# embedded-software-laboratory/p-dmpc

Measured on AMD Instinct MI355X. Metric: MPC steps/sec (whole node) + p50 per-step plan latency, N vehicles H=8, higher is better.
Workload: dtype f64

## Files before the change

include/pdmpc.h:

```cpp
#ifndef PDMPC_H
#define PDMPC_H

#include <stddef.h>
#include <stdint.h>

#ifdef __cplusplus
extern "C" {
#endif

#define PDMPC_HP_MAX 16
#define PDMPC_VMAX 8
#define PDMPC_JOINT_MAX 4

enum {
    PDMPC_OK = 0,
    PDMPC_EXHAUSTED = 1,
    PDMPC_ARENA_OVERFLOW = 2,
    PDMPC_ERR_INVALID = -1,
    PDMPC_ERR_NO_DEVICE = -2,
    PDMPC_ERR_HIP = -3,
    PDMPC_ERR_CAPACITY = -4,
    PDMPC_ERR_NO_MPA = -5
};

// ... 21 lines not shown
    double area[2][PDMPC_VMAX];
    double area_without_offset[2][PDMPC_VMAX];
    double area_large_offset[2][PDMPC_VMAX];
} pdmpc_maneuver;

typedef struct {
    int32_t n_trims;
    int32_t Hp;
    const uint8_t* transition;
    const int32_t* maneuver_index;
    int32_t n_maneuvers;
    const pdmpc_maneuver* maneuvers;
} pdmpc_mpa;

typedef struct {
    int32_t n_polygons;
    const int32_t* offset;
    const double* x;
    const double* y;
} pdmpc_polygon_set;

typedef struct {
    double x0, y0, yaw0;
    int32_t trim0;
    int32_t n_left;
    int32_t n_right;
    int32_t _pad;
    const double* ref_x;
    const double* ref_y;
    const double* v_ref;
    const double* left_x;
    const double* left_y;
    const double* right_x;
    const double* right_y;
    pdmpc_polygon_set obstacles;
    pdmpc_polygon_set dynamic_obstacles;
    pdmpc_polygon_set hdv_reachable_sets;
} pdmpc_vehicle_in;

typedef struct {
    int32_t status;
    int32_t n_expanded;
    int32_t n_popped;
    int32_t n_hp;
    int32_t tree_path[PDMPC_HP_MAX + 1];
    int32_t predicted_trims[PDMPC_HP_MAX];
    int32_t shape_cols[PDMPC_HP_MAX];
    int32_t _pad;
    double y_predicted[PDMPC_HP_MAX][3];
    double shapes[PDMPC_HP_MAX][2][PDMPC_VMAX];
    double path_nodes[PDMPC_HP_MAX + 1][8];
} pdmpc_vehicle_out;

typedef struct {
    int64_t n_vehicles;
    int64_t nodes_popped;
    int64_t nodes_generated;
    int64_t obstacle_columns;
    int64_t algorithmic_bytes;
    double kernel_ms;
    int64_t lds_bytes;
    int64_t lds_nodes;
    int64_t n_launches;
    int64_t queue_fallbacks;
    int64_t speculation_arrivals;
    int64_t edge_checks;
    int64_t segment_pair_tests;
    int64_t kernel;
    int64_t nodes_processed;
    int64_t rounds;
    int64_t shared_rounds;
    int64_t helper_checked;
    int64_t safe_replans;
    int64_t bad_status_plans;
} pdmpc_stats;


int pdmpc_create(const pdmpc_config* config, pdmpc_handle** out_handle);
int pdmpc_destroy(pdmpc_handle* handle);

int pdmpc_get_config(pdmpc_handle* handle, pdmpc_config* config, int32_t* mpa_uploaded);

int pdmpc_upload_mpa(pdmpc_handle* handle, const pdmpc_mpa* mpa);

int pdmpc_plan_batch(pdmpc_handle* handle, int32_t n_vehicles, const pdmpc_vehicle_in* in,
                     pdmpc_vehicle_out* out);

int pdmpc_set_arena_limit(pdmpc_handle* handle, int32_t max_nodes_limit);
int pdmpc_grow_arena(pdmpc_handle* handle, int32_t max_nodes);
int pdmpc_arena_nodes(pdmpc_handle* handle, int32_t* max_nodes, int64_t* regrows);

int pdmpc_plan_step(pdmpc_handle* handle, int32_t n_vehicles, const pdmpc_vehicle_in* in, const int32_t* pred_offset,
                    const int32_t* pred_index, const pdmpc_polygon_set* fallback_shapes, pdmpc_vehicle_out* out);

int pdmpc_plan_step_literal(pdmpc_handle* handle, int32_t n_vehicles, const pdmpc_vehicle_in* in, const int32_t* pred_offset, const int32_t* pred_index,
                            const pdmpc_polygon_set* fallback_shapes, pdmpc_vehicle_out* out);

int pdmpc_pack_batch(pdmpc_handle* handle, int32_t n_vehicles, const pdmpc_vehicle_in* in);
int pdmpc_plan_step_lean(pdmpc_handle* handle, int32_t n_vehicles, const pdmpc_vehicle_in* in, const int32_t* pred_offset, const int32_t* pred_index,
                         const pdmpc_polygon_set* fallback_shapes, int32_t* status, double* final_cost);
int pdmpc_fetch_records_at(pdmpc_handle* handle, int32_t count, const int32_t* vehicles, pdmpc_vehicle_out* out);
typedef struct {
    int32_t n_cells;
    int32_t n_graphs;
    int32_t n_picks;
    int32_t _pad;
    const int32_t* cell_offset;
    const int32_t* cell_slot;
    const int32_t* graph_offset;
    const int32_t* pick_graph;
    const int32_t* pick_offset;
    const int32_t* pick_slot;
} pdmpc_choice;
int pdmpc_choose_host(int32_t n, const int32_t* status, const double* final_cost, const pdmpc_choice* choice, int32_t* chosen, double* cell_cost);
int pdmpc_choose_resident(pdmpc_handle* handle, int32_t n, const pdmpc_choice* choice, int32_t* chosen, double* cell_cost, pdmpc_vehicle_out* picks);
int pdmpc_plan_step_chosen(pdmpc_handle* handle, int32_t n_vehicles, const pdmpc_vehicle_in* in, const int32_t* pred_offset, const int32_t* pred_index,
                           const pdmpc_polygon_set* fallback_shapes, const pdmpc_choice* choice, int32_t* chosen, double* cell_cost, pdmpc_vehicle_out* picks);
int pdmpc_choice_kernel_ms(pdmpc_handle* handle, double* ms);
int pdmpc_last_call_timing(pdmpc_handle* handle, double* us3);
int pdmpc_launch_packed(pdmpc_handle* handle);
int pdmpc_launch_range(pdmpc_handle* handle, int32_t first, int32_t count);
int pdmpc_fetch_results(pdmpc_handle* handle, int32_t n_vehicles, pdmpc_vehicle_out* out);
int pdmpc_synchronize(pdmpc_handle* handle);
int pdmpc_set_safe_launch(pdmpc_handle* handle, int32_t on);
int pdmpc_set_device_share(pdmpc_handle* handle, int32_t n_handles);
int pdmpc_begin_step(pdmpc_handle* handle);
int pdmpc_select_bank(pdmpc_handle* handle, int32_t bank);
int pdmpc_reset_stats(pdmpc_handle* handle);

int pdmpc_set_step_weights(pdmpc_handle* handle, int32_t n_vehicles, const double* weights);
int pdmpc_pack_step(pdmpc_handle* handle, int32_t n_vehicles, const pdmpc_vehicle_in* in,
                    const int32_t* pred_offset, const int32_t* pred_index,
                    const pdmpc_polygon_set* fallback_shapes);

int pdmpc_result_device_buffer(pdmpc_handle* handle, void** dev_ptr, size_t* nbytes);
int pdmpc_import_results(pdmpc_handle* handle, int32_t first, int32_t n, const void* dev_records);
int pdmpc_export_results(pdmpc_handle* handle, int32_t first, int32_t n, void* dev_records);

int pdmpc_export_results_async(pdmpc_handle* handle, int32_t first, int32_t n, void* dev_records);
int pdmpc_stream(pdmpc_handle* handle, void** hip_stream);

int pdmpc_get_last_stats(pdmpc_handle* handle, pdmpc_stats* stats);

int pdmpc_debug_pop_trace(pdmpc_handle* handle, int32_t vehicle, int32_t capacity, int32_t* ids, int32_t* n);
int pdmpc_debug_tree(pdmpc_handle* handle, int32_t vehicle, int32_t capacity, double* x, double* y,
                     double* yaw, double* g, double* h, int32_t* trim, int32_t* k, int32_t* parent,
                     int32_t* n);

int pdmpc_debug_edge_check(pdmpc_handle* handle, int32_t mode, int32_t n_cases, const int32_t* a_off, const double* a_x, const double* a_y,
                           const int32_t* b_off, const double* b_x, const double* b_y, int32_t* hit);

int pdmpc_debug_raw_tree(pdmpc_handle* handle, int32_t vehicle, int32_t capacity, double* x, double* y, double* yaw, double* g,
                         double* h, int32_t* trim, int32_t* k, int32_t* parent, double* key, uint8_t* validity, int32_t* n);

int pdmpc_debug_counters(pdmpc_handle* handle, uint64_t* out16);

int pdmpc_debug_progress(pdmpc_handle* handle, int32_t vehicle, uint32_t* words16);

int pdmpc_debug_heap_script(pdmpc_handle* handle, int32_t n, const int32_t* op, const int32_t* id, const double* key,
                            int32_t lds_entries, int32_t* popped, int32_t* n_popped, double* cycles_per_pop,
                            double* cycles_per_push);

int pdmpc_plan_batch_sampled(pdmpc_handle* handle, int32_t n_vehicles, const pdmpc_vehicle_in* in, const uint32_t* seeds,
                             pdmpc_vehicle_out* out);
int pdmpc_plan_step_sampled(pdmpc_handle* handle, int32_t n_vehicles, const pdmpc_vehicle_in* in, const int32_t* pred_offset,
                            const int32_t* pred_index, const pdmpc_polygon_set* fallback_shapes, const uint32_t* seeds,
// ... 181 lines not shown
```

p-dmpc_amd/csrc/api.cpp:

```cpp
#include <hip/hip_runtime.h>

#include <algorithm>
#include <cmath>
#include <cstdio>
#include <cstdlib>
#include <chrono>
#include <cstring>
#include <limits>
#include <map>
#include <mutex>
#include <string>
#include <utility>
#include <vector>

#include "../../include/pdmpc_geometry.h"
#include "handle.hpp"

namespace {

thread_local std::string g_err;

inline uint32_t align16(uint32_t v) { return (v + 15u) & ~15u; }

const size_t kLdsMax = 160 * 1024;

bool parse_tuning(const char* text, Tuning& T, std::string& err) {
    struct Key { const char* name; int* dst; };
    int spin = (int)T.spin_limit;
    const Key keys[] = {{"round0", &T.round0}, {"round", &T.round}, {"ramp", &T.ramp}, {"ready", &T.ready}, {"share_min", &T.share_min},
                        {"tile", &T.tile}, {"mid_min", &T.mid_min}, {"mid_fill", &T.mid_fill}, {"tentative", &T.tentative}, {"fast_arrival", &T.fast_arrival}, {"helpers_first", &T.helpers_first}, {"seat_nodes", &T.seat_nodes},
                        {"helpers", &T.helpers}, {"helpers_oversub", &T.helpers_oversub}, {"speculate", &T.speculate}, {"waves", &T.waves}, {"compact", &T.compact}, {"spin_limit", &spin},
                        {"force_tie", &T.force_tie}, {"reverse_dispatch", &T.reverse_dispatch}, {"debug_tail", &T.debug_tail}, {"debug_lds", &T.debug_lds},
                        {"debug_host", &T.debug_host}, {"debug_progress", &T.debug_progress}, {"generic", &T.generic}};
    std::string str(text ? text : "");
    size_t pos = 0;
    while (pos < str.size()) {
        size_t end = str.find(',', pos);
        if (end == std::string::npos) end = str.size();
        const std::string item = str.substr(pos, end - pos);
        pos = end + 1;
        if (item.empty()) continue;
        const size_t eq = item.find('=');
        if (eq == std::string::npos || eq == 0 || eq + 1 >= item.size()) {
            err = "PDMPC_TUNING: '" + item + "' is not key=value";
            return false;
        }
        const std::string name = item.substr(0, eq);
        char* tail = nullptr;
        const long v = strtol(item.c_str() + eq + 1, &tail, 10);
        if (!tail || *tail) {
            err = "PDMPC_TUNING: value of '" + name + "' is not an integer";
            return false;
        }
        bool found = false;
        for (const Key& k : keys)
            if (name == k.name) {
                *k.dst = (int)v;
                found = true;
            }
        if (!found) {
            err = "PDMPC_TUNING: unknown key '" + name + "'";
            return false;
        }
    }
    if (T.compact < -1 || T.compact > 1) {
        err = "PDMPC_TUNING: compact takes -1, 0 or 1";
        return false;
    }
    if (T.round0 >= 0) T.round0 = std::max(1, T.round0);
    if (T.round >= 0) T.round = std::max(1, T.round);
    if (T.ramp >= 0) T.ramp = std::max(1, T.ramp);
    T.ready = std::min(2048, std::max(256, T.ready)) & ~63;
    if (T.share_min >= 0) T.share_min = std::max(32, T.share_min);
    if (T.tile >= 0) T.tile = std::min(768, std::max(8, T.tile));
    T.mid_min = std::max(0, T.mid_min);
    T.mid_fill = std::max(256, T.mid_fill);
    if (T.waves >= 0) T.waves = std::min(PDMPC_MAX_WAVES, std::max(4, T.waves));
    T.spin_limit = (uint32_t)std::max(1024, spin);
    return true;
}
}

namespace {

std::mutex g_lds_mutex;
uint32_t g_lds_high_water[64][4][2];
const char* const kBulkKernelNames[4][2] = {{"pdmpc_bulk_kernel", "pdmpc_bulk_kernel_any"},
                                            {"pdmpc_bulk_kernel_wide", "pdmpc_bulk_kernel_wide_any"},
                                            {"pdmpc_bulk_kernel_sat", "pdmpc_bulk_kernel_sat_any"},
                                            {"pdmpc_bulk_kernel_compact", "pdmpc_bulk_kernel_compact_any"}};
template <class Layout>
uint32_t layout_mpa(const pdmpc_handle* h, uint32_t off, bool areas, Layout& L) {
    L.mask = off;
    off = align16(off + (uint32_t)h->mask_bytes);
    L.man_index = off;
    off = align16(off + (uint32_t)h->mi_bytes);
    L.pose = off;
    off = align16(off + (uint32_t)(h->n_man * sizeof(DevManPose)));
    L.area = off;
    if (areas) off = align16(off + (uint32_t)(h->n_man * 3 * PDMPC_VMAX * 16));
    return off;
}

bool layout_bulk(const pdmpc_handle* h, size_t budget, int n_waves, int areas, int soup_cap, LdsLayout& L, uint32_t& nv, uint32_t& nl, uint32_t ready_cap, bool compact) {
    const uint32_t lk_waves = compact ? PDMPC_LK_COMPACT_WAVES : PDMPC_MAX_WAVES, lk_ready = compact ? PDMPC_LK_COMPACT_READY_CAP : 2048u, lk_per = compact ? PDMPC_LK_COMPACT_BK_PER : PDMPC_BK_PER;
    if (ready_cap > lk_ready || (uint32_t)n_waves > lk_waves) return false;
    uint32_t off = layout_mpa(h, pdmpc_lk_fixed(lk_waves, lk_ready, lk_per, &L), areas, L);
    L.soup = off;
    off = align16(off + (uint32_t)std::max(soup_cap, 1) * 16);
    L.tree16 = L.bk_hist;
    const uint32_t min_nodes = 64 * (uint32_t)sizeof(NodeRec) + 1024;
    if ((size_t)off + min_nodes + 256 > budget) return false;
    const uint32_t rest = (uint32_t)(budget - off - 256);
    nv = std::min<uint32_t>(16384u, std::max<uint32_t>(compact ? 512u : 1024u, rest / 6));
    nv = std::min(nv, h->arena.max_nodes) & ~15u;
    nl = std::min((rest - nv) / (uint32_t)sizeof(NodeRec), h->arena.max_nodes);
    L.vstate = off;
    off += align16(nv);
    L.nodes = off;
    off += nl * (uint32_t)sizeof(NodeRec);
    L.total = align16(off);
    return L.total <= budget;
}

bool bulk_has_helpers(const Tuning& T, int n_cu, int n_launch) {
    if (!T.speculate || T.helpers == 0) return false;
    if (n_launch > n_cu) return T.helpers_oversub != 0;
    return n_launch <= n_cu - 2;
}

int compute_lds_bulk(const pdmpc_handle* h, int n_launch, int soup_cap, LaunchLayout& out) {
    const Tuning& T = h->tune;
    const int ready_want = bulk_has_helpers(T, h->n_cu, n_launch) ? T.ready : std::max(256, T.ready / 2);
    const int cap = h->cfg.checker == PDMPC_CHECK_SAT ? PDMPC_MAX_WAVES_SAT : PDMPC_MAX_WAVES;
    const bool want_compact = h->cfg.checker == PDMPC_CHECK_INTERX && h->n_words == 1 && (T.compact > 0 || (T.compact < 0 && n_launch > 2 * h->n_cu));
    uint32_t nv = 0, nl = 0;
    if (want_compact) {
        LdsLayout L{};
        const int waves = T.waves >= 0 ? std::min(T.waves, PDMPC_LK_COMPACT_WAVES) : PDMPC_LK_COMPACT_WAVES;
        const int ready = std::min(std::min(ready_want, 3 * PDMPC_WAVE * waves), (int)PDMPC_LK_COMPACT_READY_CAP);
        if (layout_bulk(h, kLdsMax / 2, waves, 0, soup_cap, L, nv, nl, (uint32_t)ready, true)) {
            out = {L, waves, (int)nl, (int)nv, 0, ready, true};
            return PDMPC_OK;
        }
    }
    const int waves = T.waves >= 0 ? std::min(T.waves, cap) : (n_launch > 2 * h->n_cu ? std::min(12, cap) : cap);
    for (int areas = 1; areas >= 0; --areas) {
        LdsLayout L{};
        const int ready = std::min(ready_want, 3 * PDMPC_WAVE * waves);
        if (!layout_bulk(h, kLdsMax, waves, areas, soup_cap, L, nv, nl, (uint32_t)ready, false)) continue;
        out = {L, waves, (int)nl, (int)nv, areas, ready, false};
        return PDMPC_OK;
    }
    char buf[256];
    snprintf(buf, sizeof buf, "obstacle soup (%d columns) + MPA tables do not fit into %zu B of LDS", soup_cap, kLdsMax);
    return fail(PDMPC_ERR_CAPACITY, buf);
}

int compute_lds_sampled(const pdmpc_handle* h, int soup_cap, int cand_cap, LaunchLayout& out) {
    static_assert(288u * 16u * 2u >= 624u * 4u, "the tree region holds the generator's state");
    for (int pass = 0; pass < 4; ++pass) {
        const int areas = pass == 0 || pass == 2;
        const size_t budget = pass < 2 ? kLdsMax / 2 : kLdsMax;
        LdsLayout L{};
        uint32_t off = layout_mpa(h, 0, areas, L);
        L.ref = off;
        off += 3 * PDMPC_HP_MAX * 8;
        L.shape = off;
        off += (2 * PDMPC_VMAX + 1) * 16;
        L.path = off;
        off += align16((PDMPC_HP_MAX + 2) * 4 + 2 * (PDMPC_HP_MAX + 1) * 4 + PDMPC_SH_WORDS * 4 + PDMPC_HP_MAX * 4);
        L.soup = off;
        off = align16(off + (uint32_t)std::max(soup_cap, 1) * 16);
        L.cand = off;
        off += align16((uint32_t)std::max(cand_cap, 1) * 4u);
        L.expand = off;
        off += (2 * PDMPC_HP_MAX * PDMPC_HP_MAX) * 8 + 16 * 16;
        L.tree16 = off;
        off += align16(288u * 18u * 2u);
        L.rand = off;
        off += align16((uint32_t)h->cfg.Hp * 250u * 8u);
        L.total = align16(off);
        if (L.total <= budget) {
            out = {L, 1, 0, 0, areas, h->tune.ready, false};
            return PDMPC_OK;
        }
    }
    return fail(PDMPC_ERR_CAPACITY, "obstacle soup + MPA tables do not fit into the LDS budget of the sampled optimizer");
}

int layout_joint(pdmpc_handle* h, int soup_cap, JointLds& L, uint32_t& heap_lds, int& areas_in_lds) {
    for (int pass = 0; pass < 4; ++pass) {
        const bool areas = pass == 0 || pass == 2;
        const size_t budget = pass < 2 ? 64 * 1024 : kLdsMax;
        uint32_t off = layout_mpa(h, 0, areas, L);
        L.ref = off;
        off += PDMPC_JOINT_MAX * 3 * PDMPC_HP_MAX * 8;
        L.shape = off;
        off += PDMPC_JOINT_MAX * 2 * PDMPC_VMAX * 16;
        L.ints = off;
        off = align16(off + PDMPC_JOINT_INTS * 4);
        L.succ = off;
        off = align16(off + (uint32_t)(PDMPC_JOINT_MAX * h->n_trims * 4));
        L.soup = off;
        off = align16(off + (uint32_t)std::max(soup_cap, 1) * 16);
        if (off + 256 * 12 > budget) continue;
        const uint32_t entries = std::min<uint32_t>(8192u, (uint32_t)((budget - off) / 12) & ~63u);
        L.heap_key = off;
        off += entries * 8;
        L.heap_id = off;
        off += entries * 4;
        L.total = align16(off);
        heap_lds = entries;
        areas_in_lds = areas ? 1 : 0;
        return PDMPC_OK;
    }
    return fail(PDMPC_ERR_CAPACITY, "the MPA tables and a joint problem's obstacle soups do not fit into LDS");
}
template <class Args>
void set_batch_args(const pdmpc_handle* h, const PackedStep& B, int areas_in_lds, Args& a) {
    a.succ_mask = h->d_mask.p;
    a.man_index = h->d_mi.p;
    a.man_pose = h->d_pose.p;
    a.man_area = h->d_area.p;
    a.n_trims = h->n_trims;
    a.n_words = h->n_words;
    a.n_man = h->n_man;
    a.Hp = h->cfg.Hp;
    a.areas_in_lds = areas_in_lds;
    a.dt = h->cfg.dt_seconds;
    a.veh = B.dev.veh;
    a.points = B.dev.pts;
    a.out = h->d_out.p;
    a.max_nodes = h->arena.max_nodes;
    a.tree_size = h->d_tree_size.p;
// ... 69 lines not shown
    a.bk_mid_fill = T.mid_fill;
    a.bk_tentative = T.tentative;
    a.bk_fast_arrival = T.fast_arrival;
    a.bk_seat_nodes = std::max(1, T.seat_nodes);
    a.bk_force_tie = T.force_tie;
    a.bk_post = h->d_bk_post.p;
    a.help_board = h->d_help_board.p;
    a.help_verdict = h->d_help_verdict.p;
    a.help_finished = h->d_help_finished.p;
    h->launch_serial += 1;
    if (h->launch_serial == 0) h->launch_serial = 1;
    a.launch_id = h->launch_serial;
    a.n_searches = count;
}

int prepare_boards(pdmpc_handle* h, int count, uint32_t& fin_base) {
    fin_base = 0;
    if (!h->boards_dirty) {
        fin_base = h->help_fin_total;
        h->help_fin_total += (uint32_t)count;
    } else {
        HIPCHK(hipMemsetAsync(h->d_help_board.p, 0, (size_t)h->max_vehicles * PDMPC_HB_WORDS * sizeof(unsigned long long), h->stream));
        HIPCHK(hipMemsetAsync(h->d_help_finished.p, 0, 16 * sizeof(uint32_t), h->stream));
        h->help_fin_total = (uint32_t)count;
        h->boards_dirty = false;
    }
    return PDMPC_OK;
}

int bulk_variant(const pdmpc_handle* h, const LaunchLayout& lay) {
    return lay.compact ? PDMPC_BULK_COMPACT : (h->cfg.checker == PDMPC_CHECK_SAT ? PDMPC_BULK_SAT : (h->n_words != 1 ? PDMPC_BULK_WIDE : PDMPC_BULK));
}
bool bulk_generic(const pdmpc_handle* h, const KernelArgs& a, const LaunchLayout& lay) { return h->tune.generic != 0 || !ProductSwitches::matches(a, bulk_variant(h, lay)); }

void print_bulk_layout(const pdmpc_handle* h, const KernelArgs& a, const LaunchLayout& lay) {
    const uint32_t near = (lay.compact ? PDMPC_LK_COMPACT_BK_PER : PDMPC_BK_PER) * (uint32_t)lay.n_waves * PDMPC_WAVE;
    const char* kernel = kBulkKernelNames[bulk_variant(h, lay)][bulk_generic(h, a, lay) ? 1 : 0];
    if (lay.compact)
        fprintf(stderr, "pdmpc LDS layout (compact): launch %d waves %d near %u ready %d nv %d nl %d total %u kernel %s\n", a.n_searches, lay.n_waves, near, lay.ready, lay.NV, lay.NL, lay.lds.total, kernel);
    else
        fprintf(stderr, "pdmpc LDS layout: launch %d waves %d areas %d near %u ready %d nv %d nl %d total %u kernel %s\n", a.n_searches, lay.n_waves, lay.areas_in_lds, near, lay.ready, lay.NV, lay.NL,
                lay.lds.total, kernel);
}

int dispatch(const pdmpc_handle* h, const KernelArgs& a, const LaunchLayout& lay, bool search, bool safe) {
    const int first = a.first, count = a.n_searches;
    const int variant = bulk_variant(h, lay), generic = bulk_generic(h, a, lay) ? 1 : 0;
    auto launch_search = [&](const KernelArgs* ka, int cnt) -> int {
        typedef int (*launcher_t)(const KernelArgs*, int, void*, uint32_t*);
        static const launcher_t launchers[4][2] = {{pdmpc_launch_bulk, pdmpc_launch_bulk_any},
                                                   {pdmpc_launch_bulk_wide, pdmpc_launch_bulk_wide_any},
                                                   {pdmpc_launch_bulk_sat, pdmpc_launch_bulk_sat_any},
                                                   {pdmpc_launch_bulk_compact, pdmpc_launch_bulk_compact_any}};
        std::lock_guard<std::mutex> lock(g_lds_mutex);
        return launchers[variant][generic](ka, cnt, (void*)h->stream, &g_lds_high_water[h->cfg.device & 63][variant][generic]);
    };
    auto in_slices = [&](int resident, auto&& launch) -> int {
        int lrc = 0;
        for (int done = 0; done < count && lrc == 0; done += resident) {
            KernelArgs part = a;
            part.first = first + done;
            part.n_searches = std::min(resident, count - done);
            lrc = launch(&part, part.n_searches);
        }
        return lrc;
    };
    if (!search) {
        const int resident = lay.lds.total <= kLdsMax / 2 ? 2 * h->n_cu : h->n_cu;
        return in_slices(safe ? resident : count, [&](const KernelArgs* ka, int cnt) { return pdmpc_launch_sampled(ka, cnt, (void*)h->stream); });
    }
    if (safe && count > h->n_cu) return in_slices(h->n_cu, launch_search);
    return launch_search(&a, count);
}

int launch_range(pdmpc_handle* h, int first, int count, bool safe) {
    if (!h) return fail(PDMPC_ERR_INVALID, "null handle");
    PackedStep& B = h->banks[h->bank];
    const bool search = !B.sampled;
    if (B.pack_failed) return fail(PDMPC_ERR_INVALID, "the last pack into this bank failed: nothing is packed");
    if (first < 0 || count < 0 || first + count > B.n_packed) return fail(PDMPC_ERR_INVALID, "launch range outside the packed batch");
    if (!B.perm.empty() && (first != 0 || count != B.n_packed)) return fail(PDMPC_ERR_INVALID, "range launches need a batch packed in level order (predecessors in lower slots)");
    if (count == 0) return PDMPC_OK;
    LaunchLayout lay;
    int rc = search ? compute_lds_bulk(h, count, B.soup_cap, lay) : compute_lds_sampled(h, B.soup_cap, B.cand_cap, lay);
    if (rc) return rc;
    KernelArgs a{};
    set_launch_args(h, B, lay, first, count, safe, a);
    launch_policy(h->tune, count, h->n_cu, h->device_share, safe, search, lay, B.host.veh + first, a);
    if (a.n_helpers > 0 && (rc = prepare_boards(h, count, a.help_fin_base))) return rc;
    if (search && h->tune.debug_lds) print_bulk_layout(h, a, lay);
    if ((rc = h->timer.begin(h->stream, search ? kLaunchSearch : kLaunchSampled))) return rc;
    const int lrc = dispatch(h, a, lay, search, safe);
    if (lrc != 0) {
        h->boards_dirty = true;
        char buf[256];
        snprintf(buf, sizeof buf, "kernel launch failed: %s (LDS %u B)", hipGetErrorString((hipError_t)lrc), lay.lds.total);
        return fail(PDMPC_ERR_HIP, buf);
    }
    if ((rc = h->timer.end(h->stream))) return rc;
    h->stats.lds_bytes = lay.lds.total;
    h->stats.lds_nodes = lay.NL;
    return PDMPC_OK;
}

int check_result_slots(const pdmpc_handle* h, int32_t first, int32_t n) {
    if (!h->banks[h->bank].perm.empty()) return fail(PDMPC_ERR_INVALID, "the packed batch was put into level order by the library: raw slots are not the caller's vehicles (pack it in level order to use the device-resident record path)");
    if (first < 0 || n < 0 || first + n > h->max_vehicles) return fail(PDMPC_ERR_INVALID, "slot range out of bounds");
    return PDMPC_OK;
}
}

extern "C" {

const char* pdmpc_last_error(void) { return g_err.c_str(); }
void pdmpc_set_last_error(const char* msg) { g_err = msg ? msg : ""; }
const char* pdmpc_version(void) { return "pdmpc-hip 0.1 (gfx950)"; }

int pdmpc_create(const pdmpc_config* config, pdmpc_handle** out_handle) {
    if (!config || !out_handle) return fail(PDMPC_ERR_INVALID, "null argument");
    if (config->Hp < 1 || config->Hp > PDMPC_HP_MAX) return fail(PDMPC_ERR_INVALID, "Hp must be in 1..PDMPC_HP_MAX");
    if (config->checker != PDMPC_CHECK_SAT && config->checker != PDMPC_CHECK_INTERX) return fail(PDMPC_ERR_INVALID, "unknown checker");
    int ndev = 0;
    if (hipGetDeviceCount(&ndev) != hipSuccess || ndev == 0)
        return fail(PDMPC_ERR_NO_DEVICE, "no HIP device visible: this backend has no CPU fallback");
    if (config->device < 0 || config->device >= ndev) return fail(PDMPC_ERR_NO_DEVICE, "device ordinal out of range");
    ON_DEVICE(config->device);
    hipDeviceProp_t prop;
    HIPCHK(hipGetDeviceProperties(&prop, config->device));
    if (std::string(prop.gcnArchName).find("gfx950") == std::string::npos)
        return fail(PDMPC_ERR_NO_DEVICE, std::string("device is ") + prop.gcnArchName + ", this library is built for gfx950 only");
    pdmpc_handle* h = new pdmpc_handle();
    h->cfg = *config;
    h->banks.resize(1);
    {
        std::string err;
        if (!parse_tuning(getenv("PDMPC_TUNING"), h->tune, err)) {
            delete h;
            return fail(PDMPC_ERR_INVALID, err);
        }
    }
    h->n_cu = prop.multiProcessorCount > 0 ? prop.multiProcessorCount : 256;
    const uint32_t want_nodes = config->max_nodes > 0 ? (uint32_t)config->max_nodes : 32768u;
    h->max_vehicles = config->max_vehicles > 0 ? config->max_vehicles : 256;
    if (hipStreamCreateWithFlags(&h->stream, hipStreamNonBlocking) != hipSuccess) {
        delete h;
        return fail(PDMPC_ERR_HIP, "hipStreamCreate failed");
    }
    int bad = h->arena.alloc(h->max_vehicles, want_nodes, h->cfg.Hp);
    bad |= h->d_out.ensure((size_t)h->max_vehicles) | h->d_flag.ensure((size_t)h->max_vehicles) | h->d_tree_size.ensure((size_t)h->max_vehicles) | h->d_tie_count.ensure(4) | h->d_work_count.ensure(16);
    bad |= h->d_help_board.ensure((size_t)h->max_vehicles * PDMPC_HB_WORDS) | h->d_help_verdict.ensure((size_t)h->max_vehicles * PDMPC_HELP_CAP) | h->d_help_finished.ensure(16);
    bad |= h->d_bk_post.ensure((size_t)h->max_vehicles * (size_t)h->tune.ready * 6);
    if (bad) {
        delete h;
        return fail(PDMPC_ERR_HIP, "hipMalloc failed for the per-vehicle arenas (lower max_nodes / max_vehicles)");
    }
    (void)hipMemsetAsync(h->d_flag.p, 0, h->d_flag.cap * sizeof(uint32_t), h->stream);
    (void)hipMemsetAsync(h->d_tree_size.p, 0, h->d_tree_size.cap * sizeof(int32_t), h->stream);
    (void)hipMemsetAsync(h->d_tie_count.p, 0, 4 * sizeof(int32_t), h->stream);
    (void)hipMemsetAsync(h->d_work_count.p, 0, 16 * sizeof(unsigned long long), h->stream);
    (void)hipMemsetAsync(h->d_out.p, 0, h->d_out.cap * sizeof(pdmpc_vehicle_out), h->stream);
    (void)hipStreamSynchronize(h->stream);
    *out_handle = h;
    return PDMPC_OK;
}

int pdmpc_destroy(pdmpc_handle* h) {
    if (!h) return PDMPC_OK;
    DeviceGuard device_guard__(h->cfg.device);
    delete h;
    return PDMPC_OK;
}

int pdmpc_upload_mpa(pdmpc_handle* h, const pdmpc_mpa* mpa) {
    if (!h || !mpa) return fail(PDMPC_ERR_INVALID, "null argument");
    if (mpa->n_trims < 1 || mpa->n_trims > 1023) return fail(PDMPC_ERR_INVALID, "n_trims must be in 1..1023");
    if (mpa->Hp < h->cfg.Hp) return fail(PDMPC_ERR_INVALID, "mpa.Hp smaller than config.Hp");
    if (!mpa->transition || !mpa->maneuver_index || (mpa->n_maneuvers > 0 && !mpa->maneuvers)) return fail(PDMPC_ERR_INVALID, "null table");
    ON_DEVICE(h->cfg.device);
    const int n = mpa->n_trims, Hp = h->cfg.Hp;
    const int nw = (n + 63) / 64;
    std::vector<uint64_t> mask((size_t)Hp * n * nw + 2, 0);
    for (int k = 0; k < Hp; ++k)
        for (int i = 0; i < n; ++i)
            for (int j = 0; j < n; ++j)
                if (mpa->transition[((size_t)k * n + i) * n + j]) {
                    const int mi = mpa->maneuver_index[i * n + j];
                    if (mi < 0 || mi >= mpa->n_maneuvers) return fail(PDMPC_ERR_INVALID, "transition allowed but maneuver missing");
                    mask[((size_t)k * n + i) * nw + j / 64] |= 1ull << (j % 64);
                }
    std::vector<int16_t> mi((size_t)n * n + 8, -1);
    for (int i = 0; i < n * n; ++i) mi[i] = (int16_t)mpa->maneuver_index[i];
    const int T = mpa->n_maneuvers;
    std::vector<DevManPose> pose((size_t)std::max(T, 1));
    std::vector<double> area((size_t)std::max(T, 1) * 3 * PDMPC_VMAX * 2, 0.0);
    for (int t = 0; t < T; ++t) {
        const pdmpc_maneuver& m = mpa->maneuvers[t];
        if (m.n_cols < 2 || m.n_cols > PDMPC_VMAX) return fail(PDMPC_ERR_INVALID, "maneuver area column count out of range");
        pose[t].dx = m.dx;
        pose[t].dy = m.dy;
        pose[t].dyaw = m.dyaw;
        pose[t].n_cols = m.n_cols;
        pose[t].pad = 0;
        const double(*src[3])[PDMPC_VMAX] = {m.area, m.area_without_offset, m.area_large_offset};
        for (int a = 0; a < 3; ++a)
            for (int v = 0; v < m.n_cols; ++v) {
                area[(((size_t)t * 3 + a) * PDMPC_VMAX + v) * 2 + 0] = src[a][0][v];
                area[(((size_t)t * 3 + a) * PDMPC_VMAX + v) * 2 + 1] = src[a][1][v];
            }
    }
    if (h->d_mask.ensure(mask.size()) || h->d_mi.ensure(mi.size()) || h->d_pose.ensure(pose.size()) || h->d_area.ensure(area.size()))
        return fail(PDMPC_ERR_HIP, "hipMalloc failed for the MPA tables");
    HIPCHK(hipMemcpy(h->d_mask.p, mask.data(), mask.size() * 8, hipMemcpyHostToDevice));
    HIPCHK(hipMemcpy(h->d_mi.p, mi.data(), mi.size() * 2, hipMemcpyHostToDevice));
    HIPCHK(hipMemcpy(h->d_pose.p, pose.data(), pose.size() * sizeof(DevManPose), hipMemcpyHostToDevice));
    HIPCHK(hipMemcpy(h->d_area.p, area.data(), area.size() * 8, hipMemcpyHostToDevice));
    h->n_trims = n;
    h->n_words = nw;
    h->n_man = T;
    h->mask_bytes = (size_t)Hp * n * nw * 8;
    h->mi_bytes = (size_t)n * n * 2;
    h->mpa_alg_bytes = (int64_t)8 * T * (3 + 6 * PDMPC_VMAX) + (int64_t)n * n * Hp / 8;
    h->has_mpa = true;
    return PDMPC_OK;
}

int pdmpc_pack_batch(pdmpc_handle* h, int32_t n, const pdmpc_vehicle_in* in) { return pdmpc_pack_step(h, n, in, nullptr, nullptr, nullptr); }

int pdmpc_pack_step(pdmpc_handle* h, int32_t n, const pdmpc_vehicle_in* in, const int32_t* pred_offset, const int32_t* pred_index,
                    const pdmpc_polygon_set* fallback_shapes) {
    if (!h) return fail(PDMPC_ERR_INVALID, "null handle");
    ON_DEVICE(h->cfg.device);
    if (pred_offset && !pred_index) return fail(PDMPC_ERR_INVALID, "pred_index missing");
    return pack_common(h, n, in, pred_offset, pred_index, fallback_shapes);
}

int pdmpc_set_step_weights(pdmpc_handle* h, int32_t n, const double* weights) {
    if (!h || n < 0 || (n > 0 && !weights)) return fail(PDMPC_ERR_INVALID, "pdmpc_set_step_weights: bad argument");
    h->next_weights.assign(weights, weights + n);
    return PDMPC_OK;
}

int pdmpc_set_step_seeds(pdmpc_handle* h, int32_t n, const uint32_t* seeds) {
    if (!h || n < 0 || (n > 0 && !seeds)) return fail(PDMPC_ERR_INVALID, "pdmpc_set_step_seeds: bad argument");
    h->next_seeds.assign(seeds, seeds + n);
    h->seeds_set = true;
    return PDMPC_OK;
}

int pdmpc_launch_packed(pdmpc_handle* h) {
    if (!h) return fail(PDMPC_ERR_INVALID, "null handle");
    ON_DEVICE(h->cfg.device);
    h->epoch += 1;
    return launch_range(h, 0, h->banks[h->bank].n_packed, h->safe_launches);
}

int pdmpc_set_device_share(pdmpc_handle* h, int32_t n_handles) {
    if (!h || n_handles < 1) return fail(PDMPC_ERR_INVALID, "pdmpc_set_device_share: bad argument");
    h->device_share = n_handles;
    return PDMPC_OK;
}

int pdmpc_set_safe_launch(pdmpc_handle* h, int32_t on) {
    if (!h) return fail(PDMPC_ERR_INVALID, "null handle");
    h->safe_launches = on != 0;
    return PDMPC_OK;
}

int pdmpc_begin_step(pdmpc_handle* h) {
    if (!h) return fail(PDMPC_ERR_INVALID, "null handle");
    h->epoch += 1;
    return PDMPC_OK;
}

int pdmpc_select_bank(pdmpc_handle* h, int32_t bank) {
    if (!h) return fail(PDMPC_ERR_INVALID, "null handle");
    if (bank < 0 || bank >= 4096) return fail(PDMPC_ERR_INVALID, "bank out of range");
    if ((size_t)bank >= h->banks.size()) h->banks.resize((size_t)bank + 1);
    h->bank = bank;
    return PDMPC_OK;
}

int pdmpc_reset_stats(pdmpc_handle* h) {
    if (!h) return fail(PDMPC_ERR_INVALID, "null handle");
    ON_DEVICE(h->cfg.device);
    HIPCHK(hipStreamSynchronize(h->stream));
    h->timer.reset();
    HIPCHK(hipMemsetAsync(h->d_tie_count.p, 0, 4 * sizeof(int32_t), h->stream));
    HIPCHK(hipMemsetAsync(h->d_work_count.p, 0, 16 * sizeof(unsigned long long), h->stream));
    return PDMPC_OK;
}

int pdmpc_launch_range(pdmpc_handle* h, int32_t first, int32_t count) {
// ... 923 lines not shown
```

p-dmpc_amd/csrc/bulk_search.hpp:

```cpp
#include <hip/hip_runtime.h>

#include "search_common.hpp"

#include "frontier_common.hpp"

#define BK_P2 3
#define BK_PER PDMPC_BK_PER
#define BK_FAST_PER 4

namespace {

typedef volatile LDS_AS unsigned long long lds_vu64;

__device__ __forceinline__ unsigned long long wg_scan_excl(unsigned long long v, lds_vu64* wsum, int lane, int wave, int n_waves, unsigned long long& total) {
    unsigned long long inc = v;
#pragma unroll
    for (int o = 1; o < PDMPC_WAVE; o <<= 1) {
        const unsigned long long t = __shfl_up(inc, o);
        inc += lane >= o ? t : 0ull;
    }
    if (lane == PDMPC_WAVE - 1) wsum[wave] = inc;
    __syncthreads();
    unsigned long long off = 0, tot = 0;
    for (int q = 0; q < n_waves; ++q) {
        const unsigned long long w = wsum[q];
        off += q < wave ? w : 0ull;
        tot += w;
    }
    total = tot;
    return off + inc - v;
}

__device__ __forceinline__ d2 node_piece(const Search& S, uint32_t i0, int q) {
    if (i0 < S.NL) return S.ln[4 * (size_t)i0 + q];
    return ((const d2*)(S.gn + i0))[q];
}
__device__ __forceinline__ void piece_link(d2 p3, uint32_t& parent, uint32_t& packed) {
    const uint64_t u = (uint64_t)__double_as_longlong(p3.y);
    parent = (uint32_t)(u & 0xffffffffull);
    packed = (uint32_t)(u >> 32);
}

struct BkCheck {
    const lds_d2* l_area;
    const d2* g_area;
    const lds_d2* l_soup;
    const lds_i32* l_soff;
    const lds_i32* l_hoff;
    const lds_i32* l_lit;
    int areas_in_lds, ll_base, ll_len, Hp;
};

#define VS_TENT 6u
#define BK_TENT_MIN FR_JOIN_MAX
#define BK_NTENT FR_SEL2_BIN
#define BK_ARRIVALS FR_SEL2_CUM
#define BK_DEPTH FR_RD_HEAD
#define BK_IDLE FR_RD_TAIL
#define BK_MID_N 10
#define BK_MID_MIN 12
#define BK_L_MID 14
#define BK_FD_LO 16
#define BK_FD_HI 17
#define BK_WAITRES 18
#define BK_TIEMODE 20
#define BK_RP_NEED 21
#define BK_RP_GOAL 22
#define BK_RP_NPOP 23
#define BK_RP_NREF 24
#define BK_PUBLISHED 19

__device__ __forceinline__ void bk_tentative_areas(const KernelArgs& A, const SpecCtx& P, unsigned long long who, int tid, int nthreads) {
    const double qnan = __longlong_as_double(0x7ff8000000000000LL);
    const int per = P.Hp * PDMPC_VMAX, n_pred = P.n_pred < 64 ? P.n_pred : 64;
    for (int idx = tid; idx < n_pred * per; idx += nthreads) {
        const int p = idx / per, rest = idx - p * per;
        if (!((who >> p) & 1ull)) continue;
        const DevVehicle* PV = A.veh + P.pred[p];
        if (PV->fb_off[0] < 0) continue;
        const int k = rest / PDMPC_VMAX, v = rest - k * PDMPC_VMAX;
        const int a = PV->fb_off[k], b = PV->fb_off[k + 1];
        const int cols = (b - a < PDMPC_VMAX) ? (b - a) : PDMPC_VMAX;
        d2 pt;
        pt.x = v < cols ? A.points[2 * (size_t)(a + (v < cols ? v : 0))] : qnan;
        pt.y = v < cols ? A.points[2 * (size_t)(a + (v < cols ? v : 0)) + 1] : qnan;
        P.l_soup[P.l_soff[k] + P.l_lit[k] + p * PDMPC_VMAX + v] = pt;
    }
}

struct BkTreeSrc {
    const Search* S;
    const lds_u32* ready;
    __device__ __forceinline__ void link(uint32_t r, uint32_t& parent, uint32_t& packed) const { piece_link(node_piece(*S, ready[r] - 1u, 3), parent, packed); }
    __device__ __forceinline__ void pose(uint32_t, uint32_t parent, double& px, double& py, double& cs, double& sn) const {
        const d2 pxy = node_piece(*S, parent - 1u, 0), pcs = node_piece(*S, parent - 1u, 2);
        px = pxy.x;
        py = pxy.y;
        cs = pcs.x;
        sn = pcs.y;
    }
};
struct BkPostSrc {
    const lds_d2* rec;
    __device__ __forceinline__ void link(uint32_t r, uint32_t& parent, uint32_t& packed) const { piece_link(d2{0.0, rec[3 * r + 2].x}, parent, packed); }
    __device__ __forceinline__ void pose(uint32_t r, uint32_t, double& px, double& py, double& cs, double& sn) const {
        const d2 pxy = rec[3 * r], pcs = rec[3 * r + 1];
        px = pxy.x;
        py = pxy.y;
        cs = pcs.x;
        sn = pcs.y;
    }
};

template <int CHECKER>
__device__ __forceinline__ void bk_item_counts(int M_k, int Hk, int ll_len, int& n0, int& n1, int& n2) {
    n0 = CHECKER == PDMPC_CHECK_INTERX ? (M_k > 1 ? M_k - 1 : 0) : M_k;
    n1 = CHECKER == PDMPC_CHECK_INTERX ? (Hk > 1 ? Hk - 1 : 0) : 0;
    n2 = ll_len > 1 ? ll_len - 1 : 0;
}
template <int CHECKER, class Src>
__device__ __forceinline__ void bk_check_items(const BkCheck& C, const Src& src, volatile lds_u32* r_flag, uint32_t r0, uint32_t R, int ls, uint32_t chmax, unsigned long long pend, int tid, int nthreads) {
    const uint32_t items = R * chmax;
    const int Sg = 1 << ls;
    for (uint32_t item = (uint32_t)tid; item < items; item += (uint32_t)nthreads) {
        const uint32_t c = item / R, r = r0 + (item - c * R);
        if (r_flag[r] & 1u) continue;
        uint32_t parent, packed;
        src.link(r, parent, packed);
        if (!parent) continue;
        const int k = NODE_K(packed), m = NODE_MAN(packed), ncols = NODE_COLS(packed);
        const int so = C.l_soff[k - 1], ho = C.l_hoff[k - 1];
        const int M_k = C.l_soff[k] - so, Hk = C.l_hoff[k] - ho;
        int n0, n1, n2;
        bk_item_counts<CHECKER>(M_k, Hk, C.ll_len, n0, n1, n2);
        const uint32_t c0 = (uint32_t)((n0 + Sg - 1) >> ls), c1 = (uint32_t)((n1 + Sg - 1) >> ls), c2 = (uint32_t)((n2 + Sg - 1) >> ls);
        int base, t0, left, which = 0;
        if (c < c0) {
            base = so;
            t0 = (int)(c << ls);
            left = n0 - t0;
        } else if (c < c0 + c1) {
            base = ho;
            t0 = (int)((c - c0) << ls);
            left = n1 - t0;
        } else if (c < c0 + c1 + c2) {
            base = C.ll_base;
            t0 = (int)((c - c0 - c1) << ls);
            left = n2 - t0;
            which = k == C.Hp ? 2 : 1;
        } else {
            continue;
        }
        const int tn = left < Sg ? left : Sg;
        double cc, ss, pX, pY;
        src.pose(r, parent, pX, pY, cc, ss);
        const size_t abase = ((size_t)m * 3 + (size_t)which) * PDMPC_VMAX;
        d2 pt[PDMPC_VMAX];
#pragma unroll
        for (int i = 0; i < PDMPC_VMAX; ++i) {
            const d2 a = C.areas_in_lds ? (d2)C.l_area[abase + i] : C.g_area[abase + i];
            pt[i].x = cc * a.x - ss * a.y + pX;
            pt[i].y = ss * a.x + cc * a.y + pY;
        }
        const lds_d2* q = C.l_soup + base + t0;
        if (CHECKER == PDMPC_CHECK_SAT) {
            uint32_t fnd = 0;
            if (which == 0) {
                const int lit = C.l_lit[k - 1];
                for (int t = 0; t < tn && !(fnd & 1u); ++t) {
                    const int j = t0 + t;
                    const bool start = !is_nan(q[t].x) && (j == 0 || is_nan(C.l_soup[base + j - 1].x) || (j >= lit && ((j - lit) & (PDMPC_VMAX - 1)) == 0));
                    if (start) {
                        int e = j + 1;
                        const int lim = j >= lit ? j + PDMPC_VMAX - ((j - lit) & (PDMPC_VMAX - 1)) : M_k;
                        while (e < lim && !is_nan(C.l_soup[base + e].x)) ++e;
                        if (sat_pair_lane(pt, ncols, C.l_soup + base + j, e - j)) {
                            const bool tent = j >= lit && ((pend >> ((j - lit) >> 3)) & 1ull) != 0ull;
                            fnd |= tent ? 2u : 1u;
                        }
                    }
                }
            } else {
                double min_x, max_x, min_y, max_y;
                sat_area_bbox(pt, ncols, min_x, max_x, min_y, max_y);
                for (int t = 0; t < tn && !fnd; ++t) fnd = sat_boundary_segment_lane(pt, ncols, min_x, max_x, min_y, max_y, q[t], q[t + 1]) ? 1u : 0u;
            }
            if (fnd) __hip_atomic_fetch_or((lds_u32*)&r_flag[r], fnd, __ATOMIC_RELAXED, __HIP_MEMORY_SCOPE_WORKGROUP);
            continue;
        }
        d2 q0 = q[0];
        const int rel0 = (which == 0 && base == so) ? t0 - C.l_lit[k - 1] : -(1 << 20);
        uint32_t found = 0;
        for (int t = 0; t < tn && !(found & 1u); ++t) {
            asm volatile("" : "+v"(pt[0].x), "+v"(pt[0].y), "+v"(pt[1].x), "+v"(pt[1].y), "+v"(pt[2].x), "+v"(pt[2].y), "+v"(pt[3].x), "+v"(pt[3].y), "+v"(pt[4].x), "+v"(pt[4].y),
                         "+v"(pt[5].x), "+v"(pt[5].y), "+v"(pt[6].x), "+v"(pt[6].y), "+v"(pt[7].x), "+v"(pt[7].y));
            const d2 q1 = q[t + 1];
            if (interx_segment_n<PDMPC_VMAX>(pt, ncols - 1, q0, q1)) {
                const int rel = rel0 + t;
                const bool tent = rel >= 0 && ((pend >> (rel >> 3)) & 1ull) != 0ull;
                found |= tent ? 2u : 1u;
            }
            q0 = q1;
        }
        if (found) __hip_atomic_fetch_or((lds_u32*)&r_flag[r], found, __ATOMIC_RELAXED, __HIP_MEMORY_SCOPE_WORKGROUP);
    }
}

__device__ __forceinline__ int bk_chunk_shift(const lds_u32* chm, uint32_t R, uint32_t nthreads) {
    int ls = 0;
    while (ls < 4 && R * chm[ls] > nthreads) ++ls;
    return ls;
}

__device__ __forceinline__ int nth_bit(uint64_t mask, int rk) {
    for (int b = 0; b < rk; ++b) mask &= mask - 1ull;
    return (int)__builtin_ctzll(mask);
}

template <int CHECKER>
__device__ __forceinline__ void bk_recheck_items(const Search& S, const VState& VS, const BkCheck& C, const SpecCtx& P, const uint32_t* vlist, const lds_u32* vcnt, uint32_t cap,
                                                 uint32_t items, unsigned long long arr, const lds_u64s* chg, volatile lds_u32* sh, int tid, int nthreads) {
    for (uint32_t item = (uint32_t)tid; item < items; item += (uint32_t)nthreads) {
        uint32_t v = item, n_k = 0;
        int ks = 1;
        for (; ks <= C.Hp; ++ks) {
            n_k = vcnt[ks - 1] < cap ? vcnt[ks - 1] : cap;
            const uint32_t m = n_k * (uint32_t)__builtin_popcountll(chg[ks - 1] & arr);
            if (v < m) break;
            v -= m;
        }
        const uint32_t a = v / n_k;
        const uint32_t i0 = vlist[(size_t)(ks - 1) * cap + (v - a * n_k)];
        if (vs_load(VS, i0) != VS_VALID) continue;
        uint32_t parent, packed;
        piece_link(node_piece(S, i0, 3), parent, packed);
        if (!parent) continue;
        const int k = NODE_K(packed), m = NODE_MAN(packed), ncols = NODE_COLS(packed);
        const unsigned long long due = chg[k - 1] & arr;
        if (a >= (uint32_t)__builtin_popcountll(due)) continue;
        const int p = nth_bit(due, (int)a);
        const d2 pxy = node_piece(S, parent - 1u, 0), pcs = node_piece(S, parent - 1u, 2);
        const double cc = pcs.x, ss = pcs.y, pX = pxy.x, pY = pxy.y;
        const size_t abase = (size_t)m * 3 * PDMPC_VMAX;
        d2 pt[PDMPC_VMAX];
#pragma unroll
        for (int i = 0; i < PDMPC_VMAX; ++i) {
            const d2 ar = C.areas_in_lds ? (d2)C.l_area[abase + i] : C.g_area[abase + i];
            pt[i].x = cc * ar.x - ss * ar.y + pX;
            pt[i].y = ss * ar.x + cc * ar.y + pY;
        }
        const lds_d2* poly = P.l_soup + P.l_soff[k - 1] + P.l_lit[k - 1] + p * PDMPC_VMAX;
        d2 q0 = poly[0];
        bool hit = false;
        if (CHECKER == PDMPC_CHECK_SAT) {
            int cols = 0;
            while (cols < PDMPC_VMAX && !is_nan(poly[cols].x)) ++cols;
            hit = cols > 0 && sat_pair_lane(pt, ncols, poly, cols);
        }
#pragma unroll 1
        for (int j = 0; CHECKER == PDMPC_CHECK_INTERX && j + 1 < PDMPC_VMAX; ++j) {
            asm volatile("" : "+v"(pt[0].x), "+v"(pt[0].y), "+v"(pt[1].x), "+v"(pt[1].y), "+v"(pt[2].x), "+v"(pt[2].y), "+v"(pt[3].x), "+v"(pt[3].y), "+v"(pt[4].x), "+v"(pt[4].y),
                         "+v"(pt[5].x), "+v"(pt[5].y), "+v"(pt[6].x), "+v"(pt[6].y), "+v"(pt[7].x), "+v"(pt[7].y));
            const d2 q1 = poly[j + 1];
            hit = hit || interx_segment_n<PDMPC_VMAX>(pt, ncols - 1, q0, q1);
            q0 = q1;
        }
        if (hit) {
            vs_store(VS, i0, VS_INVALID);
            atomicOr((uint32_t*)&sh[FR_FLAGS], FRF_INVALIDATED);
        }
    }
}

#define BK_NB 256
__device__ __forceinline__ uint32_t bk_bin(double key, double lo, double scale) {
    const double t = (key - lo) * scale;
    if (!(t > 0.0)) return 0u;
    return t < (double)(BK_NB - 1) ? (uint32_t)t : (uint32_t)(BK_NB - 1);
}
__device__ __forceinline__ void bk_select(const lds_u32* bins, uint32_t target, int lane, uint32_t& bin, uint32_t& cum) {
    uint32_t hq[4];
#pragma unroll
    for (int q = 0; q < 4; ++q) hq[q] = bins[4 * lane + q];
    const uint32_t loc = hq[0] + hq[1] + hq[2] + hq[3];
    uint32_t inc = loc;
#pragma unroll
    for (int o = 1; o < PDMPC_WAVE; o <<= 1) {
        const uint32_t v = (uint32_t)__shfl_up((int)inc, o);
        inc += lane >= o ? v : 0u;
    }
    const uint32_t total = lane_u(inc, PDMPC_WAVE - 1);
    const uint32_t want = target < total ? target : total;
    uint32_t c = inc - loc, b = 0, cu = 0;
    bool f = false;
#pragma unroll
    for (int q = 0; q < 4; ++q) {
        c += hq[q];
        const bool hit = !f && hq[q] != 0u && c >= want;
        b = hit ? (uint32_t)(4 * lane + q) : b;
        cu = hit ? c : cu;
        f = f || hit;
    }
    const unsigned long long m = __ballot(f);
    const int l = m ? (int)__builtin_ctzll(m) : 0;
    const uint32_t bb = lane_u(b, l), cc = lane_u(cu, l);
    bin = m ? bb : 0u;
    cum = m ? cc : 0u;
}

__device__ __forceinline__ void bk_post_store(d2* p, d2 v) {
    __hip_atomic_store((double*)p, (double)v.x, __ATOMIC_RELAXED, __HIP_MEMORY_SCOPE_AGENT);
    __hip_atomic_store((double*)p + 1, (double)v.y, __ATOMIC_RELAXED, __HIP_MEMORY_SCOPE_AGENT);
}
__device__ __forceinline__ d2 bk_post_load(const d2* p) {
    d2 v;
    v.x = __hip_atomic_load((const double*)p, __ATOMIC_RELAXED, __HIP_MEMORY_SCOPE_AGENT);
    v.y = __hip_atomic_load((const double*)p + 1, __ATOMIC_RELAXED, __HIP_MEMORY_SCOPE_AGENT);
    return v;
}
__device__ __forceinline__ void bk_area_store(double* p, double v) { __hip_atomic_store(p, v, __ATOMIC_RELAXED, __HIP_MEMORY_SCOPE_AGENT); }
__device__ __forceinline__ void bk_area_store_u32(int32_t* p, int v) { __hip_atomic_store(p, (int32_t)v, __ATOMIC_RELAXED, __HIP_MEMORY_SCOPE_AGENT); }
__device__ __forceinline__ double bk_area_load(const double* p) { return __hip_atomic_load(p, __ATOMIC_RELAXED, __HIP_MEMORY_SCOPE_AGENT); }
__device__ __forceinline__ int bk_area_load_i32(const int32_t* p) { return (int)__hip_atomic_load(p, __ATOMIC_RELAXED, __HIP_MEMORY_SCOPE_AGENT); }

__device__ __forceinline__ void bk_write_record(const KernelArgs& A, Ctx& X, uint32_t goal, int status, bool dep_timeout, uint32_t n_popped, uint32_t nnodes, bool path_ready,
                                                const lds_u32* ref_ids, bool again, bool counts_only, int lane) {
    const int Hp = X.Hp;
    const DevVehicle* __restrict__ V = X.V;
    pdmpc_vehicle_out* __restrict__ O = X.O;
    lds_u32* l_path = X.l_path;
    const Search& S = X.S;
    if (counts_only) {
        if (goal && ref_ids && lane <= Hp) O->tree_path[lane] = (int32_t)ref_ids[lane];
        if (lane == 0) {
// ... 38 lines not shown
            if (lane >= 1) {
                O->y_predicted[lane - 1][0] = r.x;
                O->y_predicted[lane - 1][1] = r.y;
                O->y_predicted[lane - 1][2] = r.yaw;
                O->predicted_trims[lane - 1] = (int32_t)NODE_TRIM(r.packed);
            }
        }
        for (int idx = lane; idx < Hp * PDMPC_VMAX; idx += PDMPC_WAVE) {
            const int i = idx / PDMPC_VMAX + 1;
            const int v = idx - (i - 1) * PDMPC_VMAX;
            const NodeRec pr = node_load(S, l_path[i - 1] - 1);
            const NodeRec cr = node_load(S, l_path[i] - 1);
            const int m = NODE_MAN(cr.packed);
            const int ncols = NODE_COLS(cr.packed);
            if (v == 0) {
                bk_area_store_u32(&O->shape_cols[i - 1], ncols);
                pcols[i - 1] = (uint32_t)ncols;
            }
            d2 sp = d2{0.0, 0.0};
            if (v < ncols) {
                const d2 a = X.C.g_area[(size_t)m * 3 * PDMPC_VMAX + v];
                sp.x = pr.cs * a.x - pr.sn * a.y + pr.x;
                sp.y = pr.sn * a.x + pr.cs * a.y + pr.y;
                bk_area_store(&O->shapes[i - 1][0][v], sp.x);
                bk_area_store(&O->shapes[i - 1][1][v], sp.y);
            }
            pshape[idx] = sp;
        }
    } else if (V->fb_off[0] >= 0) {
        for (int idx = lane; idx < Hp * PDMPC_VMAX; idx += PDMPC_WAVE) {
            const int k = idx / PDMPC_VMAX;
            const int v = idx - k * PDMPC_VMAX;
            const int a = V->fb_off[k], b = V->fb_off[k + 1];
            const int cols = (b - a < PDMPC_VMAX) ? (b - a) : PDMPC_VMAX;
            if (v == 0) bk_area_store_u32(&O->shape_cols[k], cols);
            if (v < cols) {
                bk_area_store(&O->shapes[k][0][v], A.points[2 * (size_t)(a + v)]);
                bk_area_store(&O->shapes[k][1][v], A.points[2 * (size_t)(a + v) + 1]);
            }
        }
    }
    if (lane == 0) {
        O->status = dep_timeout ? PDMPC_ERR_HIP : status;
        O->n_expanded = (int32_t)nnodes;
        O->n_popped = (int32_t)n_popped;
        O->n_hp = Hp;
    }
}

__device__ __forceinline__ void bk_publish_flag(const KernelArgs& A, int slot, int lane) {
    asm volatile("s_waitcnt vmcnt(0)" ::: "memory");
    wave_sync();
    if (lane == 0) {
        __hip_atomic_store(A.done_flag + slot, A.epoch, __ATOMIC_RELAXED, __HIP_MEMORY_SCOPE_AGENT);
    }
}
__device__ __forceinline__ void bk_publish(const KernelArgs& A, const Ctx& X, int status, bool dep_timeout) {
    if (X.lane == 0 && (dep_timeout || (status != PDMPC_OK && status != PDMPC_EXHAUSTED))) atomicAdd(A.work_count + 6, 1ull);
    bk_publish_flag(A, X.slot, X.lane);
}

__device__ __forceinline__ unsigned long long bk_poll_flags(const KernelArgs& A, const SpecCtx& P, unsigned long long want, int lane) {
    bool d = false;
    if ((want >> lane) & 1ull) d = __hip_atomic_load(A.done_flag + P.pred[lane], __ATOMIC_RELAXED, __HIP_MEMORY_SCOPE_AGENT) == A.epoch;
    const unsigned long long got = __ballot(d);
    return got;
}

__device__ __forceinline__ bool bk_poll_predecessors(const KernelArgs& A, const SpecCtx& P, volatile lds_u32* sh, unsigned long long skip, int lane) {
    const unsigned long long pend = sh_load64(sh, SH_PEND_LO) & ~skip;
    if (!pend) return false;
    const unsigned long long got = bk_poll_flags(A, P, pend, lane);
    if (!got) return false;
    if (lane == 0) {
        sh[SH_ARR_LO] = (uint32_t)got;
        sh[SH_ARR_HI] = (uint32_t)(got >> 32);
        __builtin_amdgcn_fence(__ATOMIC_RELEASE, "workgroup");
        atomicCAS((uint32_t*)&sh[SH_STATE], ST_RUN, ST_ARRIVED);
    }
    return true;
}

__device__ __forceinline__ void bk_incorporate_body(const pdmpc_vehicle_out* out, const int32_t* pred, lds_d2* l_soup, const lds_i32* l_soff, const lds_i32* l_lit, int Hp, unsigned long long arr, int tid,
                                                    int nthreads, lds_u64s* chg) {
    const double qnan = __longlong_as_double(0x7ff8000000000000LL);
    const int per = Hp * PDMPC_VMAX, n_arr = __builtin_popcountll(arr);
    for (int idx = tid; idx < n_arr * per; idx += nthreads) {
        const int a = idx / per, rest = idx - a * per;
        const int p = nth_bit(arr, a);
        const pdmpc_vehicle_out* PO = out + pred[p];
        const int k = rest / PDMPC_VMAX, v = rest - k * PDMPC_VMAX;
        const int cols = bk_area_load_i32(&PO->shape_cols[k]);
        const double sx = bk_area_load(&PO->shapes[k][0][v]), sy = bk_area_load(&PO->shapes[k][1][v]);
        d2 pt;
        pt.x = v < cols ? sx : qnan;
        pt.y = v < cols ? sy : qnan;
        lds_d2* slot = l_soup + l_soff[k] + l_lit[k] + p * PDMPC_VMAX + v;
        if (chg) {
            const d2 was = *slot;
            if (__double_as_longlong(was.x) != __double_as_longlong(pt.x) || __double_as_longlong(was.y) != __double_as_longlong(pt.y))
                __hip_atomic_fetch_or(chg + k, 1ull << p, __ATOMIC_RELAXED, __HIP_MEMORY_SCOPE_WORKGROUP);
        }
        *slot = pt;
    }
}
__device__ __forceinline__ void bk_incorporate(const pdmpc_vehicle_out* out, const int32_t* pred, lds_d2* l_soup, const lds_i32* l_soff, const lds_i32* l_lit, int Hp, unsigned long long arr, int tid,
                                               int nthreads, lds_u64s* chg) {
    bk_incorporate_body(out, pred, l_soup, l_soff, l_lit, Hp, arr, tid, nthreads, chg);
}

#define WC_DEAD 0x100u
#define WC_ONPATH 0x200u
#define WC_VALID 0x400u
__device__ int bk_classify_wave(const unsigned long long* glink, ulonglong2* walk, const VState& VS, const double* gkey, const lds_u32* gp_path, const lds_f64* gp_mp, bool have_goal,
                                bool check_alive, uint32_t best, uint32_t epoch, uint32_t a, double ka, volatile lds_u32* sh) {
    const uint32_t a0 = a ? a : 1u;
    const uint64_t ua = glink[a0 - 1u];
    const uint32_t p = (uint32_t)(ua & 0xffffffffull);
    const int k = NODE_K((uint32_t)(ua >> 32));
    const bool onp = have_goal && gp_path[k] == a0;
    const ulonglong2 c = walk[p ? p - 1u : 0u];
    const uint32_t ctag = (uint32_t)(c.y & 0xffffffffull), cinfo = (uint32_t)(c.y >> 32);
    const bool hit = p != 0u && ctag == best && (cinfo & (WC_VALID | 0xffff0000u)) == (WC_VALID | (epoch << 16));
    double M = -1.0;
    int dJ = k;
    bool dead = false;
    int st = (a == 0u || onp || hit) ? 1 : 0;
    uint32_t x = a0;
    while (__ballot(st == 0)) {
        const uint32_t i = x - 1u;
        const uint64_t u = glink[i];
        const int d = NODE_K((uint32_t)(u >> 32));
        const bool on_path = have_goal && gp_path[d] == x;
        const bool bad = !on_path && x != a0 && check_alive && vs_load(VS, i) != VS_VALID;
        const double kx = gkey[i];
        const uint32_t par = (uint32_t)(u & 0xffffffffull);
        const bool walking = st == 0;
        const bool stop = on_path || bad || par == 0u;
        dJ = (walking && on_path) ? d : dJ;
        dead = dead || (walking && bad);
        M = (walking && !on_path && !bad && kx > M) ? kx : M;
        st = (walking && stop) ? 1 : st;
        x = (walking && !stop) ? par : x;
    }
    if (hit && !onp) {
        const bool p_on = (cinfo & WC_ONPATH) != 0u;
        const double pM = __longlong_as_double((long long)c.x);
        const uint32_t vsp = check_alive && !p_on ? vs_load(VS, p - 1u) : (uint32_t)VS_VALID;
        dead = !p_on && ((cinfo & WC_DEAD) != 0u || vsp != VS_VALID);
        M = (!p_on && pM > ka) ? pM : ka;
        dJ = (int)(cinfo & 0xffu);
    }
    const double thr = gp_mp[dJ];
    int res = 1;
    if (a != 0u && !onp) {
        res = dead ? 4 : ((have_goal && M > thr) ? 3 : 1);
        if (!dead && have_goal && M == thr) atomicOr((uint32_t*)&sh[FR_FLAGS], FRF_TIE);
    }
    if (a != 0u && res == 1) {
        ulonglong2 w;
        w.x = (unsigned long long)__double_as_longlong(onp ? -1.0 : M);
        w.y = (unsigned long long)best | ((unsigned long long)((uint32_t)(onp ? k : dJ) | (onp ? WC_ONPATH : 0u) | WC_VALID | (epoch << 16)) << 32);
        walk[a0 - 1u] = w;
    }
    return res;
}

__device__ __forceinline__ void bk_wait_done(const uint32_t* done_flag, const int32_t* pred, const pdmpc_vehicle_out* out, uint32_t epoch, uint32_t slot, lds_d2* l_soup, const lds_i32* l_soff,
                                             const lds_i32* l_lit, lds_d2* pshape, volatile lds_u32* sh, int Hp, int n_pred, bool have_path, lds_vu64* tk_pub, unsigned long long first, uint32_t max_spins,
                                             bool sat, int lane) {
    const lds_u32* pcols = (const lds_u32*)(pshape + Hp * PDMPC_VMAX);
    lds_u64s* chg = (lds_u64s*)(pcols + PDMPC_HP_MAX);
    unsigned long long pend = sh_load64(sh, SH_PEND_LO), fd = sh_load64(sh, BK_FD_LO);
    unsigned long long got = first;
    uint32_t spins = 0, res = 0;
    for (;;) {
        if (!got && pend != 0ull) {
            bool d = false;
            if (lane < n_pred && ((pend >> lane) & 1ull)) d = __hip_atomic_load(done_flag + pred[lane], __ATOMIC_RELAXED, __HIP_MEMORY_SCOPE_AGENT) == epoch;
            got = __ballot(d);
            if (!got) {
                if (++spins >= max_spins) break;
                __builtin_amdgcn_s_sleep(1);
                continue;
            }
            bk_incorporate_body(out, pred, l_soup, l_soff, l_lit, Hp, got, lane, PDMPC_WAVE, chg);
            wave_sync();
            pend &= ~got;
            fd |= got;
        }
        const int n_got = __builtin_popcountll(got);
        const int per = Hp * (PDMPC_VMAX - 1), items = have_path ? n_got * per : 0;
        bool hit = false;
        for (int base = 0; base < items; base += PDMPC_WAVE) {
            const int item = base + lane;
            const bool in = item < items;
            const int it = in ? item : 0;
            const int a = it / per, rest = it - a * per;
            const int k0 = rest / (PDMPC_VMAX - 1), j = rest - k0 * (PDMPC_VMAX - 1);
            const int p = nth_bit(got, a);
            d2 pt[PDMPC_VMAX];
#pragma unroll
            for (int i = 0; i < PDMPC_VMAX; ++i) pt[i] = pshape[k0 * PDMPC_VMAX + i];
            const lds_d2* poly = l_soup + l_soff[k0] + l_lit[k0] + p * PDMPC_VMAX;
            bool h1;
            if (!((chg[k0] >> p) & 1ull)) {
                h1 = false;
            } else if (sat) {
                int cols = 0;
                while (cols < PDMPC_VMAX && !is_nan(poly[cols].x)) ++cols;
                h1 = j == 0 && cols > 0 && sat_pair_lane(pt, (int)pcols[k0], poly, cols);
            } else {
                h1 = interx_segment_n<PDMPC_VMAX>(pt, (int)pcols[k0] - 1, poly[j], poly[j + 1]);
            }
            hit = hit || (in && h1);
        }
        got = 0ull;
        if (__ballot(hit)) {
            res = 1;
            break;
        }
        if (pend == 0ull) {
            res = 2;
            asm volatile("s_waitcnt vmcnt(0)" ::: "memory");
            wave_sync();
            if (lane == 0) {
                __hip_atomic_store((uint32_t*)done_flag + slot, epoch, __ATOMIC_RELAXED, __HIP_MEMORY_SCOPE_AGENT);
                if (tk_pub) *tk_pub = __builtin_amdgcn_s_memrealtime();
            }
            break;
        }
        if (max_spins == 0u) break;
    }
    if (lane == 0) {
        sh[SH_PEND_LO] = (uint32_t)pend;
        sh[SH_PEND_HI] = (uint32_t)(pend >> 32);
        sh[BK_FD_LO] = (uint32_t)fd;
        sh[BK_FD_HI] = (uint32_t)(fd >> 32);
        sh[BK_WAITRES] = res;
        if (res == 2u) sh[BK_PUBLISHED] = 1u;
        sh[BK_IDLE] = sh[BK_IDLE] + spins + 1u;
    }
}

__device__ __forceinline__ void bk_offer_goals_lanes(const Frontier& F, const Search& S, const VState& VS, bool cand, uint32_t id, int lane) {
    double m = 0.0;
    bool alive = cand;
    if (cand) {
        uint32_t nd = id;
        for (;;) {
            const double k = F.gkey[nd - 1];
            m = k > m ? k : m;
            if (nd != id && vs_load(VS, nd - 1) != VS_VALID) alive = false;
            const uint32_t par = node_parent(S, nd - 1);
            if (!par) break;
            nd = par;
        }
    }
    const unsigned long long bal = __ballot(alive);
    if (bal) {
        const uint32_t base = sh_add_uniform(F.sh, FR_GOAL_N, (uint32_t)__builtin_popcountll(bal), lane);
        if (alive) {
            node_store_cs(S, id - 1u, m, 0.0);
            const uint32_t pos = base + lane_rank(bal, lane);
            if (pos < 1024u) F.goal_list[pos] = id;
        }
    }
}

__device__ __noinline__ void bk_far_select(const Frontier& F, uint32_t fill, int lane) {
    fr_select2(F, fill, fill, FR_SEL_BIN, FR_SEL_BIN, lane);
}

template <int NW>
__device__ __forceinline__ void bk_replay(const KernelArgs& A, Ctx& X, const Frontier& F, const ExpandEnv& EE, lds_f64* heap_key, lds_u32* heap_id, uint32_t hl, uint32_t* pops, uint32_t* node2ref,
                                          const uint32_t* child0, lds_u32* ref_ids, int lane) {
    volatile lds_u32* sh = F.sh;
    const VState& VS = X.VS;
    const int Hp = X.Hp, n = EE.n, nw = NW > 0 ? NW : EE.nw;
    Search H = X.S;
    H.lkey = heap_key;
    H.lid = heap_id;
    H.HL = hl & ~1u;
    H.gkey = F.far_key;
    H.gid = F.far_id;
    H.heap_len = 0;
    H.lane = lane;
    H.pl = make_pop_lane(lane);
    heap_push(H, 0u, 0.0);
    if (lane == 0) node2ref[0] = 1u;
    uint32_t n_ref = 1, n_pop = 0, goal = 0, need = 0;
    bool bug = false;
    for (;;) {
        if (H.heap_len == 0u) break;
        double k0;
        uint32_t b;
        heap_load<true>(H, 0u, true, k0, b);
        b = uni_u(b);
        heap_pop(H);
        if (lane == 0) pops[n_pop] = b;
        n_pop += 1u;
        const uint32_t v = uni_u(vs_load(VS, b));
        if (v == VS_UNKNOWN || v == VS_TENT) {
            need = b + 1u;
            break;
        }
        if (v != VS_VALID) continue;
        const uint64_t u = F.glink[b];
        const uint32_t packed = uni_u((uint32_t)(u >> 32));
        const int k = NODE_K(packed);
        if (k == Hp) {
            goal = b + 1u;
            break;
        }
        const lds_mask64* mrow = EE.l_mask + ((size_t)k * n + (NODE_TRIM(packed) - 1)) * nw;
        uint32_t cnt = 0;
        for (int w = 0; w < nw; ++w) cnt += (uint32_t)__builtin_popcountll(mrow[w]);
        cnt = uni_u(cnt);
        if (cnt == 0u) continue;
        const uint32_t c0 = uni_u(__hip_atomic_load(child0 + b, __ATOMIC_RELAXED, __HIP_MEMORY_SCOPE_AGENT));
        if (c0 == 0u) {
            bug = true;
// ... 18 lines not shown
        for (int i = Hp; i >= 0; --i) {
            X.l_path[i] = nd;
            ref_ids[i] = __hip_atomic_load(node2ref + (nd - 1u), __ATOMIC_RELAXED, __HIP_MEMORY_SCOPE_AGENT);
            nd = (uint32_t)(F.glink[nd - 1u] & 0xffffffffull);
        }
    }
    if (lane == 0) {
        sh[BK_RP_NEED] = need;
        sh[BK_RP_GOAL] = goal;
        sh[BK_RP_NPOP] = n_pop;
        sh[BK_RP_NREF] = n_ref;
        if (bug) sh[FR_FLAGS] = sh[FR_FLAGS] | FRF_BUG;
        if (!need && !bug) atomicAdd(X.P.counters + 0, 1);
    }
}

template <int NW, int CHECKER, class SW>
__device__ __forceinline__ bool bulk_search(const KernelArgs& A, Ctx& X, lds_u32* ref_ids) {
    const int tid = X.tid, lane = X.lane, wave = X.wave, slot = X.slot, Hp = X.Hp;
    volatile lds_u32* sh = X.l_shared;
    Search& S = X.S;
    const VState& VS = X.VS;
    const SpecCtx& P = X.P;
    const DevVehicle* __restrict__ V = X.V;
    const int n_waves = (int)(blockDim.x >> 6), bd = (int)blockDim.x;
    const double inf = __longlong_as_double(0x7FF0000000000000LL);
    const size_t voff = (size_t)slot * A.max_nodes;
    const int n = X.n, nw = NW > 0 ? NW : X.nw;
    const uint32_t OC = (uint32_t)(BK_PER * bd), RC = (uint32_t)A.bk_ready_cap;
    const uint32_t VCAP = 1024u;

    lds_f64* near_key = (lds_f64*)(X.lsm + PDMPC_LK_NEAR_KEY);
    lds_u32* near_id = (lds_u32*)(X.lsm + PDMPC_LK_NEAR_ID);
    lds_u32* ready = (lds_u32*)(X.lsm + PDMPC_LK_READY);
    volatile lds_u32* r_flag = (volatile lds_u32*)(ready + RC);
    lds_u32* hist = (lds_u32*)(X.lsm + PDMPC_LK_HIST);
    lds_u32* vlist = hist + 1024;
    lds_u32* voffs = hist + 2048;
    lds_u32* gp_path = (lds_u32*)(X.lsm + PDMPC_LK_MISC);
    lds_f64* gp_mp = (lds_f64*)(gp_path + 32);
    lds_vu64* wsum64 = (lds_vu64*)(gp_mp + 32);
    volatile lds_u32* wsum = (volatile lds_u32*)(wsum64 + 32);
    lds_u32* chm = (lds_u32*)(wsum + 32);
    lds_u32* bins = gp_path + 256;

    Frontier F;
    F.sh = sh;
    F.ready = ready;
    F.hist = hist;
    F.goal_list = hist;
    F.near_key = A.arena.pb_key + voff;
    F.near_id = A.arena.pb_d + voff;
    F.far_key = A.arena.far_key + voff;
    F.far_id = A.arena.far_id + voff;
    F.gkey = S.gkey;
    F.glink = A.arena.link + voff;
    F.n_waves = n_waves;

    ExpandEnv EE;
    EE.l_mask = X.l_mask;
    EE.l_mi = X.l_mi;
    EE.l_pose = X.l_pose;
    EE.l_rx = X.l_rx;
    EE.l_ry = X.l_ry;
    EE.l_dcum = X.l_dcum;
    EE.l_term = nullptr;
    EE.l_chxy = nullptr;
    EE.Hp = Hp;
    EE.n = X.n;
    EE.nw = X.nw;
    EE.lane = lane;

    BkCheck CK;
    CK.l_area = X.C.l_area;
    CK.g_area = X.C.g_area;
    CK.l_soup = X.C.l_soup;
    CK.l_soff = X.C.l_soff;
    CK.l_hoff = X.C.l_hoff;
    CK.l_lit = P.l_lit;
    CK.areas_in_lds = SW::areas_in_lds(A);
    CK.ll_base = X.C.ll_base;
    CK.ll_len = X.C.ll_len;
    CK.Hp = Hp;

    if (tid == 0) {
        NodeRec r;
        r.x = V->x0;
        r.y = V->y0;
        r.yaw = V->yaw0;
        r.g = 0.0;
        r.cs = 0.0;
        r.sn = 0.0;
        r.h = 0.0;
        r.parent = 0;
        r.packed = (uint32_t)V->trim0;
        node_store(S, 0, r);
        F.gkey[0] = 0.0;
        F.glink[0] = (unsigned long long)r.parent | ((unsigned long long)r.packed << 32);
        ((ulonglong2*)A.arena.walk + voff)[0].y = 0ull;
        (A.arena.child0 + voff)[0] = 0u;
        vs_store(VS, 0, VS_UNKNOWN);
        for (int w = 26; w < SH_WORDS; ++w) sh[w] = 0;
        sh[FR_NNODES] = 1;
        sh_st_d(sh, FR_NEAR_MIN, inf);
        sh_st_d(sh, FR_FAR_MIN, inf);
        sh_st_d(sh, FR_L_FAR, inf);
        sh_st_d(sh, BK_TENT_MIN, inf);
        sh[BK_MID_N] = 0;
        sh[BK_MID_N + 1] = 0;
        sh_st_d(sh, BK_MID_MIN, inf);
        sh_st_d(sh, BK_L_MID, -1.0);
        sh[SH_NNODES] = 1;
        sh[BK_TIEMODE] = SW::force_tie(A) ? 1u : 0u;
        ready[0] = 1u;
        r_flag[0] = 0u;
    }
    if (tid < BK_NB) bins[tid] = 0u;
    if (A.n_helpers > 0 && tid >= 64 && tid < 64 + PDMPC_HB_SEATS_MAX) {
        unsigned long long* bd0 = A.help_board + (size_t)slot * PDMPC_HB_WORDS;
        const int k = tid - 64;
        __hip_atomic_store(bd0 + PDMPC_HB_ASSIGN + k, 0ull, __ATOMIC_RELAXED, __HIP_MEMORY_SCOPE_AGENT);
        __hip_atomic_store(bd0 + PDMPC_HB_DONE + k, 0ull, __ATOMIC_RELAXED, __HIP_MEMORY_SCOPE_AGENT);
        if (k == 0) {
            __hip_atomic_store(bd0 + PDMPC_HB_WANT, 0ull, __ATOMIC_RELAXED, __HIP_MEMORY_SCOPE_AGENT);
            __hip_atomic_store(bd0 + PDMPC_HB_SEATS, (unsigned long long)A.launch_id << 32, __ATOMIC_RELAXED, __HIP_MEMORY_SCOPE_AGENT);
        }
        asm volatile("s_waitcnt vmcnt(0)" ::: "memory");
    }
    if (SW::tentative(A)) bk_tentative_areas(A, P, sh_load64(sh, SH_PEND_LO), tid, (int)blockDim.x);
    if (tid >= 64 && tid < 72) {
        const int ls = tid - 64;
        uint32_t mx = 0;
        for (int k = 1; k <= Hp; ++k) {
            const int M_k = CK.l_soff[k] - CK.l_soff[k - 1], Hk = CK.l_hoff[k] - CK.l_hoff[k - 1];
            int n0, n1, n2;
            bk_item_counts<CHECKER>(M_k, Hk, CK.ll_len, n0, n1, n2);
            const int Sg = 1 << ls;
            const uint32_t ch = (uint32_t)(((n0 + Sg - 1) >> ls) + ((n1 + Sg - 1) >> ls) + ((n2 + Sg - 1) >> ls));
            mx = ch > mx ? ch : mx;
        }
        chm[ls] = mx;
    }
    __syncthreads();

    int status = PDMPC_OK;
    bool dep_timeout = X.dep_timeout;
    uint32_t goal = 0;
    uint32_t Rn = 1;
    uint32_t depth_seen = 0xffffffffu;
    bool heavy = false;
    uint32_t t_checks = 0, t_pairs = 0;
    lds_vu64* tk = (lds_vu64*)(gp_path + 200);
    enum { TK_MARK, TK_START, tk_work, tk_arrival, tk_select, tk_wait, tk_p1, tk_p2, tk_p3, tk_pb, tk_refill, tk_pub };
    const bool ticking = SW::debug_tail(A) != 0 && tid == 0;
    if (ticking) {
        for (int i = 2; i < 12; ++i) tk[i] = 0ull;
        tk[TK_MARK] = tk[TK_START] = __builtin_amdgcn_s_memrealtime();
    }
    lds_u64s* chg = (lds_u64s*)((lds_u32*)((lds_d2*)(X.lsm + PDMPC_LK_PSHAPE) + Hp * PDMPC_VMAX) + PDMPC_HP_MAX);
    lds_u32* vcnt = (lds_u32*)(chg + PDMPC_HP_MAX);
#define BK_VLIST(k) (A.arena.vlist + ((size_t)slot * (size_t)(Hp + 1) + (size_t)((k) - 1)) * A.max_nodes)
#define BK_PLIST BK_VLIST(Hp + 1)
    if (tid < PDMPC_HP_MAX) {
        chg[tid] = 0ull;
        vcnt[tid] = 0u;
    }
    lds_vu64* tk2 = (lds_vu64*)(gp_path + 242);
    if (ticking)
        for (int i = 0; i < 7; ++i) tk2[i] = 0ull;
#define BK_TICK2(i)                                                        \
    if (ticking && SW::debug_tail(A) != 3) {                                                         \
        const unsigned long long now__ = __builtin_amdgcn_s_memrealtime(); \
        tk2[i] += now__ - tk2[6];                                          \
        tk2[6] = now__;                                                    \
    }
#define BK_MARK2 \
    if (ticking && SW::debug_tail(A) != 3) tk2[6] = __builtin_amdgcn_s_memrealtime();
    const bool ticking3 = ticking && SW::debug_tail(A) == 3;
#define BK_TICK3(i)                                                        \
    if (ticking3) {                                                        \
        const unsigned long long now__ = __builtin_amdgcn_s_memrealtime(); \
        tk2[i] += now__ - tk2[6];                                          \
        tk2[6] = now__;                                                    \
    }
#define BK_MARK3 \
    if (ticking3) tk2[6] = __builtin_amdgcn_s_memrealtime();
#define BK_TICK(acc)                                                       \
    if (ticking) {                                                         \
        const unsigned long long now__ = __builtin_amdgcn_s_memrealtime(); \
        tk[acc] += now__ - tk[TK_MARK];                                    \
        tk[TK_MARK] = now__;                                               \
    }
    double far_mn = inf, far_mx = 0.0, near_mn = inf, near_mx = 0.0, mid_mn = inf;
    double* const mid_key = A.arena.mid_key + voff;
    uint32_t* const mid_id = A.arena.mid_id + voff;
    double l_mid = -1.0;
    auto load_l_mid = [&]() {
        const unsigned long long v = (unsigned long long)__double_as_longlong(sh_ld_d(sh, BK_L_MID));
        const uint32_t lo32 = (uint32_t)__builtin_amdgcn_readfirstlane((int)(uint32_t)v), hi32 = (uint32_t)__builtin_amdgcn_readfirstlane((int)(uint32_t)(v >> 32));
        l_mid = __longlong_as_double((long long)(((unsigned long long)hi32 << 32) | lo32));
    };
    auto to_far = [&](bool take, double k, uint32_t i) {
        const unsigned long long b = __ballot(take);
        if (b && l_mid < 0.0) {
            const uint32_t base = sh_add_uniform(sh, FR_FAR_N, (uint32_t)__builtin_popcountll(b), lane);
            if (take) {
                const uint32_t pos = base + lane_rank(b, lane);
                F.far_key[pos] = k;
                F.far_id[pos] = i;
                far_mn = k < far_mn ? k : far_mn;
                far_mx = k > far_mx ? k : far_mx;
            }
        } else if (b) {
            const bool tm = k <= l_mid;
            const unsigned long long bm = __ballot(take && tm), bf = b & ~bm;
            lds_u32* p = lane == 0 ? (lds_u32*)(sh + FR_FAR_N) : (lane == 1 ? (lds_u32*)(sh + BK_MID_N) : (lds_u32*)(sh + FR_SCRATCH + lane));
            const uint32_t old = __hip_atomic_fetch_add(p, lane == 0 ? (uint32_t)__builtin_popcountll(bf) : (lane == 1 ? (uint32_t)__builtin_popcountll(bm) : 0u), __ATOMIC_RELAXED,
                                                        __HIP_MEMORY_SCOPE_WORKGROUP);
            const uint32_t base_f = (uint32_t)__builtin_amdgcn_readlane((int)old, 0), base_m = (uint32_t)__builtin_amdgcn_readlane((int)old, 1);
            if (take) {
                const uint32_t pos = tm ? base_m + lane_rank(bm, lane) : base_f + lane_rank(bf, lane);
                (tm ? mid_key : F.far_key)[pos] = k;
                (tm ? mid_id : F.far_id)[pos] = i;
                mid_mn = (tm && k < mid_mn) ? k : mid_mn;
                far_mn = (!tm && k < far_mn) ? k : far_mn;
                far_mx = (!tm && k > far_mx) ? k : far_mx;
            }
        }
    };
    auto flush_far = [&]() {
        sh_minmax_wave(sh, FR_FAR_MIN, FR_FAR_MAX, far_mn, far_mx, lane);
        far_mn = inf;
        far_mx = 0.0;
        if (__ballot(mid_mn < inf)) {
            double m = mid_mn;
#pragma unroll
            for (int o = PDMPC_WAVE / 2; o > 0; o >>= 1) {
                const double a = __shfl_xor(m, o);
                m = a < m ? a : m;
            }
            if (lane == 0) sh_min_d(sh, BK_MID_MIN, m);
            mid_mn = inf;
        }
    };
    auto to_near = [&](bool take, double k, uint32_t i) {
        const unsigned long long b = __ballot(take);
        if (b) {
            const uint32_t base = sh_add_uniform(sh, FR_NEAR_N, (uint32_t)__builtin_popcountll(b), lane);
            if (take) {
                const uint32_t pos = base + lane_rank(b, lane);
                near_key[pos] = k;
                near_id[pos] = i;
                near_mn = k < near_mn ? k : near_mn;
                near_mx = k > near_mx ? k : near_mx;
            }
        }
    };
    auto flush_near = [&]() {
        sh_minmax_wave(sh, FR_NEAR_MIN, FR_NEAR_MAX, near_mn, near_mx, lane);
        near_mn = inf;
        near_mx = 0.0;
    };
    auto bk_wait = [&]() -> bool {
        if (wave == 0) {
            uint32_t spins = 0;
            while (!bk_poll_predecessors(A, P, sh, 0ull, lane) && ++spins < 4096u) __builtin_amdgcn_s_sleep(1);
            if (lane == 0) sh[BK_IDLE] = sh[BK_IDLE] + spins + 1u;
        }
        __syncthreads();
        return sh[BK_IDLE] > A.spin_limit;
    };
    PhaseB R;
    R.n_popped = 0;
    R.n_expanded = 0;
    bool pb_valid = false;
    bool rec_valid = false, rec_written = false;
    bool vs_copied = false;
    bool tie_replayed = false;
    bool verify_req = false;
    unsigned long long* board = A.help_board + (size_t)slot * PDMPC_HB_WORDS;
    uint32_t help_seq = 0;
    bool wanted = false;

    const int tid_k = tid, lane_k = lane;
    for (;;) {
        int tid_o = tid_k, lane_o = lane_k;
        asm volatile("" : "+v"(tid_o), "+v"(lane_o));
        int tid = tid_o, lane = lane_o;
#define BK_OPAQUE_TID                                      \
    {                                                      \
        int t__ = tid_k, l__ = lane_k;                     \
        asm volatile("" : "+v"(t__), "+v"(l__));           \
        tid = t__;                                         \
        lane = l__;                                        \
    }
        if (Rn) {
            pb_valid = false;
            rec_valid = false;
            vs_copied = false;
            BK_MARK3
            const BkTreeSrc tsrc{&S, ready};
            const unsigned long long pend_now = SW::tentative(A) ? sh_load64(sh, SH_PEND_LO) : 0ull;
            bool share = A.n_helpers > 0 && Rn >= (uint32_t)A.bk_share_min && P.n_pred <= 64;
            uint32_t own_n = Rn, seats = 0, per_h = 0;
            if (share) {
                if (tid == 0) {
                    __hip_atomic_store(board + PDMPC_HB_WEIGHT, (unsigned long long)(sh[FR_PROCESSED] + Rn), __ATOMIC_RELAXED, __HIP_MEMORY_SCOPE_AGENT);
                    if (!wanted) __hip_atomic_store(board + PDMPC_HB_WANT, (unsigned long long)A.launch_id, __ATOMIC_RELAXED, __HIP_MEMORY_SCOPE_AGENT);
                    const unsigned long long sw = __hip_atomic_load(board + PDMPC_HB_SEATS, __ATOMIC_RELAXED, __HIP_MEMORY_SCOPE_AGENT);
                    uint32_t k = (uint32_t)(sw >> 32) == A.launch_id ? (uint32_t)(sw & 0xffffffffull) : 0u;
                    sh[FR_HELP_CLOSED] = k < (uint32_t)PDMPC_HB_SEATS_MAX ? k : (uint32_t)PDMPC_HB_SEATS_MAX;
                }
                wanted = true;
                __syncthreads();
                seats = sh[FR_HELP_CLOSED];
                share = seats != 0u;
            }
            if (share) {
                per_h = (Rn + seats) / (seats + 1u);
                {
                    const uint32_t cap = (uint32_t)A.bk_tile;
                    per_h = per_h < cap ? per_h : cap;
                }
                const uint32_t helped = per_h * seats < Rn ? per_h * seats : Rn;
                own_n = Rn - helped;
                ++help_seq;
                d2* post = (d2*)A.bk_post + (size_t)slot * RC * 3u;
                for (uint32_t r = own_n + (uint32_t)tid; r < Rn; r += (uint32_t)bd) {
                    uint32_t parent, packed;
                    const d2 p3 = node_piece(S, ready[r] - 1u, 3);
                    piece_link(p3, parent, packed);
                    bk_post_store(post + 3 * r, node_piece(S, parent - 1u, 0));
                    bk_post_store(post + 3 * r + 1, node_piece(S, parent - 1u, 2));
                    bk_post_store(post + 3 * r + 2, d2{p3.y, 0.0});
                }
                asm volatile("s_waitcnt vmcnt(0)" ::: "memory");
                __syncthreads();
                if (wave == 0) {
                    if (lane == 0) {
                        const unsigned long long all = P.n_pred >= 64 ? ~0ull : ((1ull << P.n_pred) - 1ull);
                        __hip_atomic_store(board + PDMPC_HB_N, (unsigned long long)Rn, __ATOMIC_RELAXED, __HIP_MEMORY_SCOPE_AGENT);
                        __hip_atomic_store(board + PDMPC_HB_MASK, all & ~sh_load64(sh, SH_PEND_LO), __ATOMIC_RELAXED, __HIP_MEMORY_SCOPE_AGENT);
                    }
                    asm volatile("s_waitcnt vmcnt(0)" ::: "memory");
                    wave_sync();
                    if ((uint32_t)lane < seats) {
                        const uint32_t first = own_n + (uint32_t)lane * per_h;
                        const uint32_t cnt = first >= Rn ? 0u : (Rn - first < per_h ? Rn - first : per_h);
                        __hip_atomic_store(board + PDMPC_HB_ASSIGN + lane, ((unsigned long long)help_seq << 40) | ((unsigned long long)first << 20) | (unsigned long long)cnt, __ATOMIC_RELAXED,
                                           __HIP_MEMORY_SCOPE_AGENT);
                    }
                }
            }
            {
                BK_TICK3(0)
                const uint32_t Rr = own_n;
                const int ls = bk_chunk_shift(chm, Rr ? Rr : 1u, (uint32_t)bd);
                bk_check_items<CHECKER>(CK, tsrc, r_flag, 0u, Rr, ls, chm[ls], pend_now, tid, bd);
                BK_TICK3(1)
                for (uint32_t r = (uint32_t)(bd - 1 - tid); r < Rn; r += (uint32_t)bd) {
                    const uint32_t i0 = ready[r] - 1u;
                    uint32_t parent, packed;
                    piece_link(node_piece(S, i0, 3), parent, packed);
                    if (NODE_K(packed) < Hp) {
                        const d2 p1 = node_piece(S, i0, 1);
                        double sn, cs;
                        pdmpc_sincos(p1.x, &sn, &cs);
                        node_store_cs(S, i0, cs, sn);
                    }
                }
                BK_TICK3(2)
            }
            if (share) {
                if (wave == 0) {
                    uint32_t spins = 0;
                    bool bad = false;
                    for (;;) {
                        bool pending_h = false;
                        if ((uint32_t)lane < seats) pending_h = (uint32_t)__hip_atomic_load(board + PDMPC_HB_DONE + lane, __ATOMIC_RELAXED, __HIP_MEMORY_SCOPE_AGENT) != help_seq;
                        if (!__ballot(pending_h)) break;
                        __builtin_amdgcn_s_sleep(1);
                        if (++spins > A.spin_limit) {
                            bad = true;
// ... 164 lines not shown
                        double expH = 0.0;
                        for (int it = 1; it <= steps_to_go; ++it) {
                            const double ddx = ch.x - EE.l_rx[k_exp - 1 + it], ddy = ch.y - EE.l_ry[k_exp - 1 + it];
                            const double nrm = sqrt(ddx * ddx + ddy * ddy);
                            const double df = nrm - EE.l_dcum[(k_exp - 1) * PDMPC_HP_MAX + (it - 1)];
                            const double m0 = (df > 0) ? df : 0.0;
                            expH = expH + m0 * m0;
                        }
                        ch.h = expH;
                        f = ch.g * 1 + expH * 1;
                        ci = nn_base + voffs[gi] + rank;
                        node_store(S, ci, ch);
                        vs_store(VS, ci, 0);
                        F.gkey[ci] = f;
                        F.glink[ci] = (unsigned long long)ch.parent | ((unsigned long long)ch.packed << 32);
                        ((ulonglong2*)A.arena.walk + voff)[ci].y = 0ull;
                        (A.arena.child0 + voff)[ci] = 0u;
                        if (rank == 0u) (A.arena.child0 + voff)[i0] = ci + 1u;
                    }
                    to_near(active && !(f > l_far), f, ci + 1u);
                    to_far(active && f > l_far, f, ci + 1u);
                }
            }
            if (tid == 0) {
                sh[FR_NNODES] = nn_base + (overflow ? 0u : NC);
                sh[FR_PROCESSED] = sh[FR_PROCESSED] + Rn;
                if (SW::debug_tail(A) == 1 && sh[FR_ROUNDS] < 32u) X.O->path_nodes[PDMPC_HP_MAX - 7 + (int)(sh[FR_ROUNDS] >> 3)][sh[FR_ROUNDS] & 7u] = (double)Rn;
                sh[FR_ROUNDS] = sh[FR_ROUNDS] + 1u;
                if (overflow) sh[FR_FLAGS] = sh[FR_FLAGS] | FRF_OVERFLOW;
            }
            Rn = 0;
            BK_TICK(tk_p3)
        }
        BK_OPAQUE_TID
        flush_near();
        flush_far();
        asm volatile("s_waitcnt vmcnt(0)" ::: "memory");
        __syncthreads();
        if (sh[FR_GOAL_N] > 1024u) {
            __syncthreads();
            if (tid == 0) sh[FR_GOAL_N] = 1024u;
            __syncthreads();
        }
        fr_resolve_goals(F, S, tid, lane, wave);
        if (sh[FR_FLAGS] & FRF_GOALS_LOST) {
            __syncthreads();
            if (tid == 0) {
                sh[FR_BEST_ID] = 0;
                sh[FR_PATH_FOR] = 0;
                sh[FR_FLAGS] = sh[FR_FLAGS] & ~FRF_GOALS_LOST;
            }
            __syncthreads();
            uint32_t nn = sh[FR_NNODES];
            nn = nn < S.max_nodes ? nn : S.max_nodes;
            for (uint32_t base = 0; base < nn; base += (uint32_t)bd) {
                const uint32_t b = base + (uint32_t)wave * PDMPC_WAVE;
                const uint32_t i0 = b + (uint32_t)lane;
                const bool in = i0 < nn;
                const uint32_t j0 = in ? i0 : 0u;
                const bool cand = in && vs_load(VS, j0) == VS_VALID && NODE_K(((const uint32_t*)(S.gn + j0))[15]) == Hp;
                bk_offer_goals_lanes(F, S, VS, cand, j0 + 1u, lane);
                __syncthreads();
                fr_resolve_goals(F, S, tid, lane, wave);
            }
        }
        BK_TICK(tk_work)

        uint32_t flags = sh[FR_FLAGS];
        if (flags & FRF_OVERFLOW) {
            status = PDMPC_ARENA_OVERFLOW;
            break;
        }
        if ((flags & FRF_BUG) || sh[FR_ROUNDS] > A.spin_limit) {
            dep_timeout = true;
            status = PDMPC_EXHAUSTED;
            break;
        }
        BK_MARK2
        if (sh_load64(sh, SH_PEND_LO) != 0ull) {
            if (wave == 0 && sh[SH_STATE] != ST_ARRIVED) (void)bk_poll_predecessors(A, P, sh, 0ull, lane);
            __syncthreads();
            if (sh[SH_STATE] == ST_ARRIVED) {
                const unsigned long long arr = sh_load64(sh, SH_ARR_LO);
                bk_incorporate(P.out, P.pred, P.l_soup, P.l_soff, P.l_lit, Hp, arr, tid, bd, chg);
                __syncthreads();
                if (tid == 0) {
                    const unsigned long long pend = sh_load64(sh, SH_PEND_LO) & ~arr, fd = sh_load64(sh, BK_FD_LO) | arr;
                    sh[SH_PEND_LO] = (uint32_t)pend;
                    sh[SH_PEND_HI] = (uint32_t)(pend >> 32);
                    sh[BK_FD_LO] = (uint32_t)fd;
                    sh[BK_FD_HI] = (uint32_t)(fd >> 32);
                    sh[SH_ARR_LO] = 0;
                    sh[SH_ARR_HI] = 0;
                    sh[SH_STATE] = ST_RUN;
                    if (ticking) {
                        X.O->path_nodes[PDMPC_HP_MAX - 2][6] = (double)sh[FR_ROUNDS];
                        X.O->path_nodes[PDMPC_HP_MAX - 2][7] = (double)__builtin_amdgcn_s_memrealtime();
                    }
                }
                __syncthreads();
                verify_req = true;
            }
        }
        BK_TICK2(0)
        if (verify_req) {
            verify_req = false;
            const unsigned long long arr = sh_load64(sh, BK_FD_LO);
            uint32_t nn = sh[FR_NNODES];
            nn = nn < S.max_nodes ? nn : S.max_nodes;
            uint32_t items = 0;
            for (int k = 0; k < Hp; ++k)
                items += (vcnt[k] < A.max_nodes ? vcnt[k] : A.max_nodes) * (uint32_t)__builtin_popcountll(chg[k] & arr);
            if (ticking) {
                unsigned long long due = 0;
                for (int k = 0; k < Hp; ++k) due += (unsigned long long)__builtin_popcountll(chg[k] & arr);
                atomicAdd(A.work_count + 14, due);
                atomicAdd(A.work_count + 15, (unsigned long long)(Hp * __builtin_popcountll(arr)));
            }
            BK_TICK2(5)
            bk_recheck_items<CHECKER>(S, VS, CK, P, BK_VLIST(1), vcnt, A.max_nodes, items, arr, chg, sh, tid, bd);
            __syncthreads();
            BK_TICK2(1)
            flags = sh[FR_FLAGS];
            bool best_alive = false;
            if ((flags & FRF_INVALIDATED) && sh[FR_BEST_ID] != 0u) {
                const uint32_t g = sh[FR_BEST_ID];
                double b1;
                best_alive = vs_load(VS, g - 1u) == VS_VALID && fr_goal_path(S, VS, F.gkey, g, b1);
            }
            const bool lost_best = (flags & FRF_INVALIDATED) && !best_alive;
            const bool reopen = lost_best && sh[FR_DROPPED] != 0u;
            const uint32_t n_parked = sh[BK_NTENT];
            if (n_parked) {
                const bool fits = sh[FR_NEAR_N] + n_parked <= OC;
                const double l_far = sh_ld_d(sh, FR_L_FAR);
                const uint32_t n_list = n_parked < A.max_nodes ? n_parked : A.max_nodes;
                for (uint32_t base = 0; base < n_list; base += (uint32_t)bd) {
                    const uint32_t e = base + (uint32_t)tid;
                    const uint32_t i0 = e < n_list ? BK_PLIST[e] : 0u;
                    const bool tent = e < n_list && vs_load(VS, i0) == VS_TENT;
                    const double k = tent ? F.gkey[i0] : 0.0;
                    if (tent) vs_store(VS, i0, VS_UNKNOWN);
                    const bool push = tent && !reopen;
                    to_near(push && fits && !(k > l_far), k, i0 + 1u);
                    to_far(push && !(fits && !(k > l_far)), k, i0 + 1u);
                }
            }
            BK_TICK2(2)
            if (flags & FRF_INVALIDATED) {
                pb_valid = false;
                rec_valid = false;
            }
            vs_copied = false;
            __syncthreads();
            if (tid == 0) {
                sh[BK_ARRIVALS] = sh[BK_ARRIVALS] + 1u;
                sh[BK_FD_LO] = 0;
                sh[BK_FD_HI] = 0;
                for (int k = 0; k < Hp; ++k) chg[k] = 0ull;
                sh[BK_NTENT] = 0;
                sh_st_d(sh, BK_TENT_MIN, inf);
                if (flags & FRF_INVALIDATED) {
                    sh[FR_EVER_INVAL] = 1;
                    if (lost_best) {
                        sh[FR_BEST_ID] = 0;
                        sh[FR_PATH_FOR] = 0;
                    }
                    sh[FR_FLAGS] = flags & ~FRF_INVALIDATED;
                }
// ... 575 lines not shown
            b += __shfl_xor(b, o);
        }
        if (lane_r == 0) {
            atomicAdd(A.work_count + 0, a);
            atomicAdd(A.work_count + 1, b);
        }
    }
    if (tid_r == 0) {
        atomicAdd(P.counters + 2, (int)sh[BK_ARRIVALS]);
        atomicAdd(A.work_count + 2, (unsigned long long)sh[FR_PROCESSED]);
        atomicAdd(A.work_count + 3, (unsigned long long)sh[FR_ROUNDS]);
        A.tree_size[slot] = (int32_t)(nnodes_raw | 0x40000000u | (tie_replayed ? 0x20000000u : 0u));
    }
    if (tid_r == 0 && SW::debug_tail(A)) {
        double* dbg = X.O->path_nodes[PDMPC_HP_MAX];
        dbg[0] = (double)sh[FR_ROUNDS];
        dbg[1] = (double)sh[FR_PROCESSED];
        dbg[2] = (double)nnodes_raw;
        dbg[3] = (double)sh[FR_NEAR_N];
        dbg[4] = (double)(sh[FR_FAR_N] + sh[BK_MID_N]);
        dbg[5] = (double)sh[FR_FLAGS];
        dbg[6] = (double)sh[BK_ARRIVALS];
        dbg[7] = (double)(__builtin_amdgcn_s_memrealtime() - tk[TK_START]);
        for (int i = 0; i < 6; ++i) X.O->path_nodes[PDMPC_HP_MAX - 3][i] = (double)tk2[i];
        if (A.n_helpers > 0) {
            const unsigned long long sw = __hip_atomic_load(board + PDMPC_HB_SEATS, __ATOMIC_RELAXED, __HIP_MEMORY_SCOPE_AGENT);
            X.O->path_nodes[PDMPC_HP_MAX - 3][7] = (double)(sw & 0xffffffffull);
        }
        X.O->path_nodes[PDMPC_HP_MAX - 2][0] = (double)(tk[TK_START] - X.rt_kernel_start);
        X.O->path_nodes[PDMPC_HP_MAX - 2][1] = (double)tk[tk_p1];
        X.O->path_nodes[PDMPC_HP_MAX - 2][2] = (double)tk[tk_p2];
        X.O->path_nodes[PDMPC_HP_MAX - 2][3] = (double)tk[tk_p3];
        X.O->path_nodes[PDMPC_HP_MAX - 2][4] = (double)tk[tk_pb];
        X.O->path_nodes[PDMPC_HP_MAX - 2][5] = (double)tk[tk_refill];
        X.O->path_nodes[PDMPC_HP_MAX - 1][0] = (double)(tk[tk_work] + tk[tk_p1] + tk[tk_p2] + tk[tk_p3]);
        X.O->path_nodes[PDMPC_HP_MAX - 1][1] = (double)tk[tk_arrival];
        X.O->path_nodes[PDMPC_HP_MAX - 1][2] = (double)tk[tk_select];
        X.O->path_nodes[PDMPC_HP_MAX - 1][3] = (double)tk[tk_wait];
        X.O->path_nodes[PDMPC_HP_MAX - 1][4] = (double)(tk[TK_MARK] - tk[TK_START]);
        X.O->path_nodes[PDMPC_HP_MAX - 1][5] = (double)tk[tk_pub];
        X.O->path_nodes[PDMPC_HP_MAX - 1][6] = (double)__builtin_amdgcn_s_memrealtime();
        X.O->path_nodes[PDMPC_HP_MAX - 1][7] = (double)X.rt_kernel_start;
    }
    X.status = status;
    X.n_popped = (int)R.n_popped;
    X.path_ready = pb_ran && goal != 0u;
    X.goal = goal;
    X.nnodes = R.n_expanded;
    X.dep_timeout = dep_timeout;
    X.rec_valid = rec_valid && !dep_timeout;
    X.rec_written = rec_written;
    X.published = sh[BK_PUBLISHED] != 0u;
    return false;
}


template <int CHECKER, class SW>
__device__ __forceinline__ void bulk_helper_body(const KernelArgs& A) {
    extern __shared__ __attribute__((aligned(16))) unsigned char smem[];
    LDS_AS unsigned char* lsm = (LDS_AS unsigned char*)smem;
    const int tid = threadIdx.x, lane = tid & (PDMPC_WAVE - 1), wave = uni_i(tid >> 6), bd = (int)blockDim.x;
    const int Hp = A.Hp, n_s = A.n_searches;
    const uint32_t CAP = (uint32_t)A.bk_tile;
    lds_u32* l_path = (lds_u32*)(lsm + PDMPC_LK_PATH);
    lds_i32* l_soff = (lds_i32*)(l_path + PDMPC_HP_MAX + 2);
    lds_i32* l_hoff = l_soff + PDMPC_HP_MAX + 1;
    volatile lds_u32* hs = (volatile lds_u32*)(l_hoff + PDMPC_HP_MAX + 1);
    lds_i32* l_lit = (lds_i32*)(hs + SH_WORDS);
    lds_d2* l_soup = (lds_d2*)(lsm + A.lds.soup);
    lds_d2* t_rec = (lds_d2*)(lsm + PDMPC_LK_NEAR_KEY);
    volatile lds_u32* t_flag = (volatile lds_u32*)(lsm + PDMPC_LK_READY);
    lds_u32* chm = (lds_u32*)(lsm + PDMPC_LK_MISC) + 192;
    BkCheck CK;
    CK.l_area = (const lds_d2*)(lsm + A.lds.area);
    CK.g_area = (const d2*)A.man_area;
    CK.l_soup = l_soup;
    CK.l_soff = l_soff;
    CK.l_hoff = l_hoff;
    CK.l_lit = l_lit;
    CK.areas_in_lds = SW::areas_in_lds(A);
    CK.ll_base = 0;
    CK.ll_len = 0;
    CK.Hp = Hp;
    if (SW::areas_in_lds(A)) stage16(lsm + A.lds.area, A.man_area, A.n_man * 3 * PDMPC_VMAX, tid);
    if (tid < SH_WORDS) hs[tid] = 0;
    __syncthreads();
    int my_slot = -1, my_seat = -1;
    uint32_t last_seq = 0;
    unsigned long long cur_mask = 0;
    const int pref = (int)blockIdx.x % n_s;
    SpecCtx P;
    P.sh = hs;
    P.l_soup = l_soup;
    P.l_soff = l_soff;
    P.l_lit = l_lit;
    P.out = A.out;
    P.pred = A.pred;
    P.counters = A.tie_count;
    P.n_pred = 0;
    P.Hp = Hp;
    uint32_t idle = 0;
    const bool hticking = SW::debug_tail(A) != 0 && tid == 0;
    unsigned long long hk_mark = hticking ? __builtin_amdgcn_s_memrealtime() : 0ull, hk[5] = {0, 0, 0, 0, 0}, hk_tiles = 0;
    const unsigned long long hk_start = hk_mark;
#define HK_TICK(i)                                                        \
    if (hticking) {                                                       \
        const unsigned long long n__ = __builtin_amdgcn_s_memrealtime(); \
        hk[i] += n__ - hk_mark;                                           \
        hk_mark = n__;                                                    \
    }
    for (;;) {
        if (my_slot < 0) {
            if (wave == 0) {
                float best_score = -1.0f;
                int best_rel = -1;
                for (int base = 0; base < n_s; base += PDMPC_WAVE) {
                    const int k = base + lane;
                    const int s_rel = k < n_s ? (pref + k) % n_s : 0;
                    const unsigned long long* b = A.help_board + (size_t)(A.first + s_rel) * PDMPC_HB_WORDS;
                    const unsigned long long want = __hip_atomic_load(b + PDMPC_HB_WANT, __ATOMIC_RELAXED, __HIP_MEMORY_SCOPE_AGENT);
                    const unsigned long long sw = __hip_atomic_load(b + PDMPC_HB_SEATS, __ATOMIC_RELAXED, __HIP_MEMORY_SCOPE_AGENT);
                    const unsigned long long wt = __hip_atomic_load(b + PDMPC_HB_WEIGHT, __ATOMIC_RELAXED, __HIP_MEMORY_SCOPE_AGENT);
                    const uint32_t cnt = (uint32_t)(sw >> 32) == A.launch_id ? (uint32_t)(sw & 0xffffffffull) : 0u;
                    uint32_t allowed = 1u + (uint32_t)((wt * (unsigned long long)A.n_helpers) / ((unsigned long long)n_s * (unsigned long long)A.bk_seat_nodes));
                    if (idle >= 8u) allowed = (uint32_t)PDMPC_HB_SEATS_MAX;
                    allowed = allowed < (uint32_t)PDMPC_HB_SEATS_MAX ? allowed : (uint32_t)PDMPC_HB_SEATS_MAX;
                    const bool cand = k < n_s && want == (unsigned long long)A.launch_id && cnt < allowed;
                    const float score = cand ? (float)(wt + 1ull) / (float)(cnt + 1u) : -1.0f;
                    float c = score;
#pragma unroll
                    for (int o = PDMPC_WAVE / 2; o > 0; o >>= 1) {
                        const float v = __shfl_xor(c, o);
                        c = v > c ? v : c;
                    }
                    const unsigned long long m = __ballot(cand && score == c);
                    if (m && c > best_score) {
                        best_score = c;
                        best_rel = (pref + base + (int)__builtin_ctzll(m)) % n_s;
                    }
                }
                uint32_t got = 0xffffffffu;
                if (best_rel >= 0) {
                    unsigned long long old = 0;
                    if (lane == 0)
                        old = __hip_atomic_fetch_add(A.help_board + (size_t)(A.first + best_rel) * PDMPC_HB_WORDS + PDMPC_HB_SEATS, 1ull, __ATOMIC_RELAXED, __HIP_MEMORY_SCOPE_AGENT);
                    const uint32_t lo32 = uni_u((uint32_t)old), hi32 = uni_u((uint32_t)(old >> 32));
                    if (hi32 == A.launch_id && lo32 < (uint32_t)PDMPC_HB_SEATS_MAX) got = lo32;
                }
                uint32_t cmd = 0;
                if (got != 0xffffffffu) {
                    cmd = 1;
                } else {
                    const uint32_t fin = __hip_atomic_load(A.help_finished, __ATOMIC_RELAXED, __HIP_MEMORY_SCOPE_AGENT);
                    if (fin - A.help_fin_base >= (uint32_t)n_s) cmd = 2;
                }
                if (lane == 0) {
                    hs[HS_SLOT] = (uint32_t)(A.first + (best_rel >= 0 ? best_rel : 0));
                    hs[HS_FIRST] = got;
                    hs[HS_CMD] = cmd;
                }
            }
            __syncthreads();
            const uint32_t cmd = hs[HS_CMD];
            if (cmd == 2u) break;
            if (cmd == 0u) {
                __builtin_amdgcn_s_sleep(127);
                __builtin_amdgcn_s_sleep(127);
                if (++idle > (A.spin_limit >> 4)) break;
                __syncthreads();
                continue;
            }
            my_slot = (int)hs[HS_SLOT];
            my_seat = (int)hs[HS_FIRST];
            last_seq = 0;
            idle = 0;
            const DevVehicle* __restrict__ V = A.veh + my_slot;
            const int pred_cols = V->n_pred * PDMPC_VMAX;
            int off = 0;
            for (int k = 0; k < Hp; ++k) {
                const int a = V->lit_off[k], b = V->lit_off[k + 1];
                if (tid == 0) {
                    l_soff[k] = off;
                    l_lit[k] = b - a;
                }
                stage16(l_soup + off, (const d2*)A.points + a, b - a, tid);
                off += (b - a) + pred_cols;
            }
            if (tid == 0) l_soff[Hp] = off;
            for (int k = 0; k < Hp; ++k) {
                const int a = V->hdv_off[k], b = V->hdv_off[k + 1];
                if (tid == 0) l_hoff[k] = off;
                stage16(l_soup + off, (const d2*)A.points + a, b - a, tid);
                off += (b - a);
            }
            if (tid == 0) l_hoff[Hp] = off;
            stage16(l_soup + off, (const d2*)A.points + V->ll_off, V->ll_len, tid);
            CK.ll_base = off;
            CK.ll_len = V->ll_len;
            __syncthreads();
            const d2 nanpt = d2{__longlong_as_double(0x7ff8000000000000LL), __longlong_as_double(0x7ff8000000000000LL)};
            for (int idx = tid; idx < Hp * pred_cols; idx += bd) {
                const int k = idx / pred_cols;
                l_soup[l_soff[k] + l_lit[k] + (idx - k * pred_cols)] = nanpt;
            }
            __syncthreads();
            P.pred = A.pred + V->pred_off;
            P.n_pred = V->n_pred;
            if (SW::tentative(A)) bk_tentative_areas(A, P, V->n_pred >= 64 ? ~0ull : ((1ull << V->n_pred) - 1ull), tid, bd);
            cur_mask = 0;
            __syncthreads();
            if (tid < 8) {
                const int ls = tid;
                uint32_t mx = 0;
                for (int k = 1; k <= Hp; ++k) {
                    const int M_k = l_soff[k] - l_soff[k - 1], Hk = l_hoff[k] - l_hoff[k - 1];
                    int n0, n1, n2;
                    bk_item_counts<CHECKER>(M_k, Hk, CK.ll_len, n0, n1, n2);
                    const int Sg = 1 << ls;
                    const uint32_t ch = (uint32_t)(((n0 + Sg - 1) >> ls) + ((n1 + Sg - 1) >> ls) + ((n2 + Sg - 1) >> ls));
                    mx = ch > mx ? ch : mx;
                }
                chm[ls] = mx;
            }
            __syncthreads();
            if (hticking) hk_mark = __builtin_amdgcn_s_memrealtime();
            continue;
        }
        unsigned long long* board = A.help_board + (size_t)my_slot * PDMPC_HB_WORDS;
        if (wave == 0) {
            const unsigned long long w = __hip_atomic_load(board + PDMPC_HB_ASSIGN + my_seat, __ATOMIC_RELAXED, __HIP_MEMORY_SCOPE_AGENT);
            const uint32_t seq = (uint32_t)(w >> 40);
            uint32_t cmd = 0;
            if (seq != last_seq && seq != 0u) {
                cmd = 1;
                const unsigned long long mask = __hip_atomic_load(board + PDMPC_HB_MASK, __ATOMIC_RELAXED, __HIP_MEMORY_SCOPE_AGENT);
                if (lane == 0) {
                    hs[HS_FIRST] = (uint32_t)((w >> 20) & 0xfffffull);
                    hs[HS_COUNT] = (uint32_t)(w & 0xfffffull);
                    hs[HS_TICKET] = seq;
                    hs[HS_MASK_LO] = (uint32_t)mask;
                    hs[HS_MASK_HI] = (uint32_t)(mask >> 32);
                }
            } else if ((idle & 15u) == 15u) {
                const unsigned long long want = __hip_atomic_load(board + PDMPC_HB_WANT, __ATOMIC_RELAXED, __HIP_MEMORY_SCOPE_AGENT);
                if (want != (unsigned long long)A.launch_id) cmd = 3;
            }
            if (lane == 0) hs[HS_CMD] = cmd;
        }
        __syncthreads();
        const uint32_t cmd = hs[HS_CMD];
        if (cmd == 3u) {
            my_slot = -1;
            my_seat = -1;
            idle = 0;
            __syncthreads();
            continue;
        }
        if (cmd == 0u) {
            if (idle < 256u)
                __builtin_amdgcn_s_sleep(1);
            else
                __builtin_amdgcn_s_sleep(16);
            if (++idle > A.spin_limit) break;
            __syncthreads();
            continue;
        }
        idle = 0;
        HK_TICK(0)
        const uint32_t first = hs[HS_FIRST], Rt = hs[HS_COUNT] < CAP ? hs[HS_COUNT] : CAP, seq = hs[HS_TICKET];
        const unsigned long long mask = ((unsigned long long)hs[HS_MASK_HI] << 32) | hs[HS_MASK_LO];
        last_seq = seq;
        if (mask != cur_mask) {
            bk_incorporate(P.out, P.pred, P.l_soup, P.l_soff, P.l_lit, Hp, mask & ~cur_mask, tid, bd, nullptr);
            cur_mask = mask;
        }
        HK_TICK(1)
        {
            const d2* post = (const d2*)A.bk_post + ((size_t)my_slot * (size_t)A.bk_ready_cap + first) * 3u;
            for (uint32_t i = (uint32_t)tid; i < Rt * 3u; i += (uint32_t)bd) t_rec[i] = bk_post_load(post + i);
            for (uint32_t i = (uint32_t)tid; i < Rt; i += (uint32_t)bd) t_flag[i] = 0u;
        }
        __syncthreads();
        HK_TICK(2)
        if (Rt) {
            const BkPostSrc psrc{t_rec};
            const int ls = bk_chunk_shift(chm, Rt, (uint32_t)bd);
            const unsigned long long pend = SW::tentative(A) ? (P.n_pred >= 64 ? ~0ull : ((1ull << P.n_pred) - 1ull)) & ~mask : 0ull;
            bk_check_items<CHECKER>(CK, psrc, t_flag, 0u, Rt, ls, chm[ls], pend, tid, bd);
        }
        __syncthreads();
        HK_TICK(3)
        {
            uint32_t* verdict = A.help_verdict + (size_t)my_slot * PDMPC_HELP_CAP + first;
            for (uint32_t i = (uint32_t)tid; i < Rt; i += (uint32_t)bd) {
                const uint32_t fl = t_flag[i];
                __hip_atomic_store(verdict + i, (fl & 1u) ? 2u : ((fl & 2u) ? 3u : 1u), __ATOMIC_RELAXED, __HIP_MEMORY_SCOPE_AGENT);
            }
        }
        asm volatile("s_waitcnt vmcnt(0)" ::: "memory");
        __syncthreads();
        if (tid == 0) {
            __hip_atomic_store(board + PDMPC_HB_DONE + my_seat, (unsigned long long)seq, __ATOMIC_RELAXED, __HIP_MEMORY_SCOPE_AGENT);
            hs[HS_CMD] = 0;
        }
        __syncthreads();
        HK_TICK(4)
        hk_tiles += 1;
    }
    if (hticking) {
        atomicAdd(A.work_count + 7, __builtin_amdgcn_s_memrealtime() - hk_start);
        for (int i = 0; i < 5; ++i) atomicAdd(A.work_count + 8 + i, hk[i]);
        atomicAdd(A.work_count + 13, hk_tiles);
    }
#undef HK_TICK
}

template <int NW, int CHECKER, class SW>
__device__ __forceinline__ void bulk_body(const KernelArgs& A) {
    if ((int)blockIdx.x < A.bk_helpers_first || (int)blockIdx.x >= A.bk_helpers_first + A.n_searches) {
        bulk_helper_body<CHECKER, SW>(A);
        return;
    }
    extern __shared__ __attribute__((aligned(16))) unsigned char smem[];
    Ctx X;
    const unsigned long long rt0 = __builtin_amdgcn_s_memrealtime();
    search_prologue<SW>(A, X, (LDS_AS unsigned char*)smem);
    X.rt_kernel_start = rt0;
    const int wave = X.wave;
    lds_u32* ref_ids = (lds_u32*)(X.lsm + PDMPC_LK_MISC) + 224;
    const bool tie = bulk_search<NW, CHECKER, SW>(A, X, ref_ids);
    (void)tie;
    __syncthreads();
    if (wave != 0) return;
    {
        int l__ = X.lane;
        asm volatile("" : "+v"(l__));
        X.lane = l__;
    }
    if (!X.rec_valid) bk_write_record(A, X, X.goal, X.status, X.dep_timeout, (uint32_t)X.n_popped, X.nnodes, X.path_ready, ref_ids, X.rec_written, X.published, X.lane);
    bk_publish(A, X, X.status, X.dep_timeout);
    if (X.lane == 0 && A.n_helpers > 0) {
        __hip_atomic_store(A.help_board + (size_t)X.slot * PDMPC_HB_WORDS + PDMPC_HB_WANT, 0ull, __ATOMIC_RELAXED, __HIP_MEMORY_SCOPE_AGENT);
        atomicAdd(A.help_finished, 1u);
    }
}

}

#ifndef PDMPC_BULK_KERNEL_ATTR
#define PDMPC_BULK_KERNEL_ATTR
#endif
#define PDMPC_BULK_INSTANCE(NAME, LAUNCHER, NW, CHECKER, MAXWAVES, SW)                                                                   \
    extern "C" __global__ __launch_bounds__(PDMPC_WAVE * (MAXWAVES)) PDMPC_BULK_KERNEL_ATTR void NAME(const KernelArgs A) { bulk_body<NW, CHECKER, SW>(A); } \
    extern "C" int LAUNCHER(const KernelArgs* args, int count, void* stream, uint32_t* lds_high_water) {                                \
        if (count <= 0) return 0;                                                                                                        \
        typedef void (*kernel_t)(const KernelArgs);                                                                                      \
        kernel_t fn = NAME;                                                                                                              \
// ... 14 lines not shown
```

p-dmpc_amd/csrc/handle.hpp:

```cpp
#pragma once
#include <hip/hip_runtime.h>

#include <algorithm>
#include <cstdio>
#include <cstring>
#include <string>
#include <utility>
#include <vector>

#include "../../include/pdmpc.h"
#include "pdmpc_device.h"

extern "C" void pdmpc_set_last_error(const char* msg);

inline int fail(int code, const std::string& msg) {
    pdmpc_set_last_error(msg.c_str());
    return code;
}

#define HIPCHK(expr)                                                                                 \
    do {                                                                                             \
        hipError_t e__ = (expr);                                                                     \
        if (e__ != hipSuccess) {                                                                     \
            char buf__[512];                                                                         \
// ... 62 lines not shown
    ~PinnedBuf() { release(); }
    int ensure(size_t n) { return ensure_keep(n, 0); }
    int ensure_keep(size_t n, size_t keep) {
        if (n <= cap) return 0;
        size_t want = std::max(n, (size_t)64);
        want += want / 2;
        T* q = nullptr;
        hipError_t e = hipHostMalloc((void**)&q, want * sizeof(T), hipHostMallocDefault);
        if (e != hipSuccess) return (int)e;
        if (p && keep) std::memcpy(q, p, std::min(keep, cap) * sizeof(T));
        if (p) (void)hipHostFree(p);
        p = q;
        cap = want;
        return 0;
    }
    void release() {
        if (p) (void)hipHostFree(p);
        p = nullptr;
        cap = 0;
    }
};

struct Arenas {
    uint32_t max_nodes = 0;
    DevBuf<NodeRec> nodes;
    DevBuf<double> key, far_key, mid_key, pb_key, walk;
    DevBuf<unsigned long long> link;
    DevBuf<uint32_t> far_id, mid_id, pb_d, child0, vlist;
    DevBuf<uint8_t> vstate;
    template <class Self, class F>
    static void each(Self& a, int Hp, F&& f) {
        f(a.nodes, 1);
        f(a.key, 1);
        f(a.link, 1);
        f(a.vstate, 1);
        f(a.far_key, 1);
        f(a.far_id, 1);
        f(a.mid_key, 1);
        f(a.mid_id, 1);
        f(a.pb_key, 1);
        f(a.pb_d, 1);
        f(a.walk, 2);
        f(a.child0, 1);
        f(a.vlist, Hp + 1);
    }
    size_t bytes_per_node(int Hp) const {
        size_t sum = 0;
        each(*this, Hp, [&](const auto& b, int per) { sum += (size_t)per * sizeof *b.p; });
        return sum;
    }
    int alloc(int max_vehicles, uint32_t n, int Hp) {
        n = (n + 1u) & ~1u;
        const size_t tot = (size_t)max_vehicles * n;
        each(*this, Hp, [](auto& b, int) { b.release(); });
        max_nodes = 0;
        int bad = 0;
        each(*this, Hp, [&](auto& b, int per) { bad |= b.ensure_exact(tot * (size_t)per); });
        if (bad) return bad;
        max_nodes = n;
        return 0;
    }
    NodeArena view() const {
        return {nodes.p, key.p, link.p, vstate.p, far_key.p, far_id.p, mid_key.p, mid_id.p, pb_key.p, pb_d.p, walk.p, child0.p, vlist.p};
    }
};

enum LaunchKind : int32_t { kLaunchSearch = 2, kLaunchSampled = 3, kLaunchJoint = 4 };

struct BlobRegions {
    DevVehicle* veh = nullptr;
    int32_t* pred = nullptr;
    double* pts = nullptr;
};

struct PackedStep {
    PinnedBuf<unsigned char> h_blob;
    DevBuf<unsigned char> d_blob;
    BlobRegions host, dev;
    uint64_t staged_serial = ~0ull;
    int n_packed = 0;
    bool pack_failed = false;
    bool sampled = false;
    int soup_cap = 0;
    int cand_cap = 0;
    std::vector<int64_t> lit_cols;
    std::vector<int32_t> perm;
    std::vector<int32_t> inv;
};

struct SoupKey {
    const void* p[13];
    int32_t c[6];
};

struct SoupTable {
    std::vector<SoupKey> keys;
    std::vector<int32_t> slot;
    std::vector<int32_t> table;
    static uint64_t hash(const SoupKey& k) {
        static_assert(sizeof(SoupKey) % 8 == 0, "SoupKey is hashed by 64-bit words");
        uint64_t hsh = 1469598103934665603ull;
        const uint64_t* w = (const uint64_t*)&k;
        for (size_t q = 0; q < sizeof(SoupKey) / 8; ++q) hsh = (hsh ^ w[q]) * 1099511628211ull;
        return hsh ^ (hsh >> 29);
    }
    void reset(int n) {
        size_t size = 64;
        while (size < (size_t)n * 2) size *= 2;
        keys.clear();
        slot.clear();
        table.assign(size, 0);
    }
    int find(const SoupKey& k, size_t& at) const {
        for (at = (size_t)hash(k) & (table.size() - 1); table[at] != 0; at = (at + 1) & (table.size() - 1)) {
            const int q = table[at] - 1;
            if (std::memcmp(&keys[(size_t)q], &k, sizeof k) == 0) return slot[(size_t)q];
        }
        return -1;
    }
    void insert(const SoupKey& k, int packed_in, size_t at) {
        keys.push_back(k);
        slot.push_back(packed_in);
        table[at] = (int32_t)keys.size();
    }
};

struct Tuning {
    int round0 = -1;
    int round = -1;
    int ramp = -1;
    int ready = 2048;
    int share_min = -1;
    int tile = -1;
    int mid_min = 24576;
    int mid_fill = 12288;
    int tentative = 1;
    int fast_arrival = 1;
    int helpers = -1;
    int helpers_oversub = -1;
    int seat_nodes = 256;
    int helpers_first = -1;
    int speculate = 1;
    int compact = -1;
    int waves = -1;
    uint32_t spin_limit = 1u << 22;
    int force_tie = 0;
    int reverse_dispatch = 0;
    int debug_tail = 0;
    int debug_lds = 0;
    int debug_host = 0;
    int debug_progress = 0;
    int generic = 0;
};

struct LaunchLayout {
    LdsLayout lds{};
    int n_waves = 0;
    int NL = 0, NV = 0;
    int areas_in_lds = 0;
    int ready = 0;
    bool compact = false;
};

struct LaunchTimer {
    static constexpr size_t kMaxPairs = 4096;
    std::vector<std::pair<hipEvent_t, hipEvent_t>> events;
// ... 193 lines not shown
```

p-dmpc_amd/csrc/pack.cpp:

```cpp
#include <hip/hip_runtime.h>

#include <algorithm>
#include <cstring>
#include <limits>
#include <numeric>
#include <string>
#include <utility>
#include <vector>

#include "coupling_order.hpp"
#include "handle.hpp"

namespace {

int check_set(const pdmpc_polygon_set& s, const char* what) {
    if (s.n_polygons < 0) return fail(PDMPC_ERR_INVALID, std::string(what) + ": negative polygon count");
    if (s.n_polygons > 0 && (!s.offset || !s.x || !s.y)) return fail(PDMPC_ERR_INVALID, std::string(what) + ": null pointer");
    for (int i = 0; i < s.n_polygons; ++i)
        if (s.offset[i + 1] < s.offset[i]) return fail(PDMPC_ERR_INVALID, std::string(what) + ": offsets not monotone");
    return PDMPC_OK;
}

size_t set_points(const pdmpc_polygon_set& s) {
    return s.n_polygons > 0 ? (size_t)(s.offset[s.n_polygons] - s.offset[0]) + (size_t)s.n_polygons : 0;
}

int slot_order(const pdmpc_handle* h, int n, const int32_t* pred_offset, const int32_t* pred_index, const std::vector<double>& weights, PackedStep& B) {
    B.perm.clear();
    B.inv.clear();
    if (!pred_offset) return PDMPC_OK;
    const bool by_priority = (int)weights.size() == n && n > 1;
    bool ordered = true;
    for (int i = 0; i < n && ordered; ++i)
        for (int q = pred_offset[i]; q < pred_offset[i + 1]; ++q) {
            const int ps = pred_index[q];
            if (ps < 0 || ps >= h->max_vehicles) return fail(PDMPC_ERR_INVALID, "predecessor slot out of range");
            if (ps < n && ps >= i) ordered = false;
        }
    if (ordered && !by_priority) return PDMPC_OK;
    CouplingOrder order;
    const CouplingOrder::Status st = order.build(n, pred_offset, pred_index, by_priority ? weights.data() : nullptr);
    if (st == CouplingOrder::kSelfEdge) return fail(PDMPC_ERR_INVALID, "a vehicle is its own predecessor");
    if (st == CouplingOrder::kCycle) return fail(PDMPC_ERR_INVALID, "the sequential coupling graph has a cycle");
    B.perm.resize((size_t)n);
    std::iota(B.perm.begin(), B.perm.end(), 0);
    order.sort(B.perm);
    bool identity = true;
    for (int i = 0; i < n && identity; ++i) identity = B.perm[(size_t)i] == i;
    if (identity) {
        B.perm.clear();
    } else {
        B.inv.resize((size_t)n);
        for (int sl = 0; sl < n; ++sl) B.inv[(size_t)B.perm[(size_t)sl]] = sl;
    }
    return PDMPC_OK;
}

struct Packer {
    pdmpc_handle* h;
    PackedStep& B;
    const int n;
    const pdmpc_vehicle_in* in;
    const int32_t *pred_offset, *pred_index;
    const pdmpc_polygon_set* fallback;
    const std::vector<uint32_t>* seeds;
    size_t veh_bytes = 0, pts_base = 0;
    BlobRegions host;
    size_t n_pred_out = 0, n_pts = 0;
    int soup_cap = 0, cand_cap = 0;

    BlobRegions regions(unsigned char* blob) const { return {(DevVehicle*)blob, (int32_t*)(blob + veh_bytes), (double*)(blob + pts_base)}; }
    int vehicle_of(int slot) const { return B.perm.empty() ? slot : B.perm[(size_t)slot]; }
    void put(double x, double y) {
        host.pts[2 * n_pts] = x;
        host.pts[2 * n_pts + 1] = y;
        ++n_pts;
    }
    void append_poly(const pdmpc_polygon_set& s, int p, bool sep) {
        const double qnan = std::numeric_limits<double>::quiet_NaN();
        for (int q = s.offset[p]; q < s.offset[p + 1]; ++q) put(s.x[q], s.y[q]);
        if (sep) put(qnan, qnan);
    }

    int reserve(size_t points) {
        if (B.h_blob.ensure_keep(pts_base + (n_pts + points) * 16, pts_base + n_pts * 16)) return fail(PDMPC_ERR_HIP, "hipHostMalloc failed");
        host = regions(B.h_blob.p);
        return PDMPC_OK;
    }

    int open() {
        size_t total_pred = 0;
        if (pred_offset)
            for (int vi = 0; vi < n; ++vi) total_pred += (size_t)std::max(0, pred_offset[vi + 1] - pred_offset[vi]);
        veh_bytes = ((size_t)std::max(n, 1) * sizeof(DevVehicle) + 15) & ~(size_t)15;
        const size_t pred_bytes = ((total_pred + 1) * sizeof(int32_t) + 15) & ~(size_t)15;
        pts_base = veh_bytes + pred_bytes;
        B.host = BlobRegions{};
        if (int rc = reserve(256)) return rc;
        B.lit_cols.assign((size_t)n, 0);
        return PDMPC_OK;
    }

    static SoupKey soup_key(const pdmpc_vehicle_in& v, const pdmpc_polygon_set* fbv) {
        SoupKey key;
        std::memset(&key, 0, sizeof key);
        const void* ptrs[13] = {v.obstacles.offset, v.obstacles.x, v.obstacles.y, v.dynamic_obstacles.offset, v.dynamic_obstacles.x, v.dynamic_obstacles.y, v.hdv_reachable_sets.offset,
                                v.hdv_reachable_sets.x, v.left_x, v.right_x, fbv ? fbv->offset : nullptr, fbv ? fbv->x : nullptr, fbv ? fbv->y : nullptr};
        for (int q = 0; q < 13; ++q) key.p[q] = ptrs[q];
        key.c[0] = v.obstacles.n_polygons;
        key.c[1] = v.dynamic_obstacles.n_polygons;
        key.c[2] = v.hdv_reachable_sets.n_polygons;
        key.c[3] = v.n_left;
        key.c[4] = v.n_right;
        key.c[5] = fbv ? fbv->n_polygons : 0;
        return key;
    }

    int check_soups(const pdmpc_vehicle_in& v, const pdmpc_polygon_set* fbv) const {
        const int Hp = h->cfg.Hp;
        int rc;
        if ((rc = check_set(v.obstacles, "obstacles"))) return rc;
        if ((rc = check_set(v.dynamic_obstacles, "dynamic_obstacles"))) return rc;
        if ((rc = check_set(v.hdv_reachable_sets, "hdv_reachable_sets"))) return rc;
        if (v.dynamic_obstacles.n_polygons % Hp) return fail(PDMPC_ERR_INVALID, "dynamic_obstacles must hold n_d * Hp polygons");
        if (v.hdv_reachable_sets.n_polygons % Hp) return fail(PDMPC_ERR_INVALID, "hdv_reachable_sets must hold n_h * Hp polygons");
        if (v.n_left < 0 || v.n_right < 0 || v.n_left == 1 || v.n_right == 1) return fail(PDMPC_ERR_INVALID, "lanelet boundary needs 0 or >= 2 points per side");
        if (fbv) {
            if (fbv->n_polygons != Hp) return fail(PDMPC_ERR_INVALID, "fallback_shapes must hold Hp polygons per vehicle");
            if ((rc = check_set(*fbv, "fallback_shapes"))) return rc;
        }
        return PDMPC_OK;
    }

    int write_head(int vi, DevVehicle& d) {
        const pdmpc_vehicle_in& v = in[vi];
        std::memset(&d, 0, sizeof d);
        d.x0 = v.x0;
        d.y0 = v.y0;
        d.yaw0 = v.yaw0;
        d.trim0 = v.trim0;
        d.seed = seeds ? (*seeds)[(size_t)vi] : 0u;
        for (int k = 0; k < h->cfg.Hp; ++k) {
            d.ref_x[k] = v.ref_x[k];
            d.ref_y[k] = v.ref_y[k];
            d.v_ref[k] = v.v_ref[k];
        }
        const int n_pred = pred_offset ? pred_offset[vi + 1] - pred_offset[vi] : 0;
        d.n_pred = n_pred;
        d.pred_off = (int32_t)n_pred_out;
        for (int q = 0; q < n_pred; ++q) {
            const int ps = pred_index[pred_offset[vi] + q];
            if (ps < 0 || ps >= h->max_vehicles) return fail(PDMPC_ERR_INVALID, "predecessor slot out of range");
            host.pred[n_pred_out++] = !B.perm.empty() && ps < n ? B.inv[(size_t)ps] : ps;
        }
        return PDMPC_OK;
    }

    void share_soups(int slot, int seen_slot, DevVehicle& d) {
        const DevVehicle& f = host.veh[(size_t)seen_slot];
        std::memcpy(d.lit_off, f.lit_off, sizeof d.lit_off);
        std::memcpy(d.hdv_off, f.hdv_off, sizeof d.hdv_off);
        std::memcpy(d.fb_off, f.fb_off, sizeof d.fb_off);
        d.ll_off = f.ll_off;
        d.ll_len = f.ll_len;
        B.lit_cols[(size_t)slot] = B.lit_cols[(size_t)seen_slot];
    }

    int append_soups(int slot, const pdmpc_vehicle_in& v, const pdmpc_polygon_set* fbv, DevVehicle& d) {
        const int Hp = h->cfg.Hp;
        const double qnan = std::numeric_limits<double>::quiet_NaN();
        const int n_dyn = v.dynamic_obstacles.n_polygons / Hp;
        const int n_hdv = v.hdv_reachable_sets.n_polygons / Hp;
        for (int k = 0; k < Hp; ++k) {
            d.lit_off[k] = (int32_t)n_pts;
            for (int p = 0; p < v.obstacles.n_polygons; ++p) append_poly(v.obstacles, p, true);
            for (int r = 0; r < n_dyn; ++r) append_poly(v.dynamic_obstacles, r * Hp + k, true);
        }
        d.lit_off[Hp] = (int32_t)n_pts;
        for (int k = 0; k < Hp; ++k) {
            d.hdv_off[k] = (int32_t)n_pts;
            for (int r = 0; r < n_hdv; ++r) append_poly(v.hdv_reachable_sets, r * Hp + k, true);
        }
        d.hdv_off[Hp] = (int32_t)n_pts;
        d.ll_off = (int32_t)n_pts;
        for (int q = 0; q < v.n_left; ++q) put(v.left_x[q], v.left_y[q]);
        put(qnan, qnan);
        for (int q = 0; q < v.n_right; ++q) put(v.right_x[q], v.right_y[q]);
        put(qnan, qnan);
        d.ll_len = (int32_t)n_pts - d.ll_off;
        B.lit_cols[(size_t)slot] = (d.lit_off[Hp] - d.lit_off[0]) + d.ll_len;
        if (fbv) {
            for (int k = 0; k < Hp; ++k) {
                d.fb_off[k] = (int32_t)n_pts;
                if (fbv->offset[k + 1] - fbv->offset[k] > PDMPC_VMAX) return fail(PDMPC_ERR_INVALID, "fallback area has more than PDMPC_VMAX columns");
                append_poly(*fbv, k, false);
            }
            d.fb_off[Hp] = (int32_t)n_pts;
        } else {
            for (int k = 0; k <= Hp; ++k) d.fb_off[k] = -1;
        }
        return PDMPC_OK;
    }

    int pack_vehicle(int slot) {
        const int Hp = h->cfg.Hp;
        const int vi = vehicle_of(slot);
        const pdmpc_vehicle_in& v = in[vi];
        if (!v.ref_x || !v.ref_y || !v.v_ref) return fail(PDMPC_ERR_INVALID, "reference trajectory missing");
        if (v.trim0 < 1 || v.trim0 > h->n_trims) return fail(PDMPC_ERR_INVALID, "trim0 out of range");
        const pdmpc_polygon_set* fbv = fallback && fallback[vi].n_polygons > 0 ? &fallback[vi] : nullptr;
        const SoupKey key = soup_key(v, fbv);
        size_t at = 0;
        const int seen_slot = h->soups.find(key, at);
        const pdmpc_vehicle_in* first_in = seen_slot >= 0 ? &in[vehicle_of(seen_slot)] : nullptr;
        const bool shared = first_in && v.left_y == first_in->left_y && v.right_y == first_in->right_y && v.hdv_reachable_sets.y == first_in->hdv_reachable_sets.y;
        int rc;
        if (!shared) {
            if ((rc = check_soups(v, fbv))) return rc;
            const size_t most = (size_t)Hp * set_points(v.obstacles) + set_points(v.dynamic_obstacles) + set_points(v.hdv_reachable_sets) + (size_t)v.n_left + (size_t)v.n_right + 2 +
                                (fbv ? set_points(*fbv) : 0) + 2;
            if ((rc = reserve(most))) return rc;
        }
        DevVehicle& d = host.veh[(size_t)slot];
        if ((rc = write_head(vi, d))) return rc;
        if (shared) {
            share_soups(slot, seen_slot, d);
        } else {
            if (seen_slot < 0) h->soups.insert(key, slot, at);
            if ((rc = append_soups(slot, v, fbv, d))) return rc;
        }
        const int need = (d.lit_off[Hp] - d.lit_off[0]) + Hp * d.n_pred * PDMPC_VMAX + (d.hdv_off[Hp] - d.hdv_off[0]) + d.ll_len;
        soup_cap = std::max(soup_cap, need);
        for (int k = 0; k < Hp; ++k) cand_cap = std::max(cand_cap, (d.lit_off[k + 1] - d.lit_off[k]) + d.n_pred * PDMPC_VMAX + (d.hdv_off[k + 1] - d.hdv_off[k]) + d.ll_len);
        return PDMPC_OK;
    }

    int close() {
        const double qnan = std::numeric_limits<double>::quiet_NaN();
        put(qnan, qnan);
        host.pred[n_pred_out++] = 0;
        B.soup_cap = soup_cap + 2;
        B.cand_cap = (cand_cap + 4 + 3) & ~3;
        const size_t pts_bytes = (n_pts * 16 + 15) & ~(size_t)15;
        const size_t total = pts_base + pts_bytes;
        if (B.d_blob.ensure(total)) return fail(PDMPC_ERR_HIP, "hipMalloc failed for the batch blob");
        B.host = host;
        B.dev = regions(B.d_blob.p);
        HIPCHK(hipMemcpyAsync(B.d_blob.p, B.h_blob.p, total, hipMemcpyHostToDevice, h->stream));
        B.staged_serial = h->sync_serial;
        B.n_packed = n;
        B.pack_failed = false;
        return PDMPC_OK;
    }
};

}

int pack_common(pdmpc_handle* h, int n, const pdmpc_vehicle_in* in, const int32_t* pred_offset, const int32_t* pred_index, const pdmpc_polygon_set* fallback) {
    if (!h) return fail(PDMPC_ERR_INVALID, "null handle");
    const std::vector<double> weights = std::move(h->next_weights);
    h->next_weights.clear();
    const bool sampled = h->seeds_set;
    const std::vector<uint32_t> seeds = std::move(h->next_seeds);
    h->next_seeds.clear();
    h->seeds_set = false;
    if (!h->has_mpa) return fail(PDMPC_ERR_NO_MPA, "pdmpc_upload_mpa has not been called");
    if (n < 0 || (n > 0 && !in)) return fail(PDMPC_ERR_INVALID, "bad vehicle array");
    if (n > h->max_vehicles) return fail(PDMPC_ERR_CAPACITY, "batch larger than config.max_vehicles");
    PackedStep& B = h->banks[h->bank];
    if (B.staged_serial == h->sync_serial) HIPCHK(sync_stream(h));
    B.n_packed = 0;
    B.pack_failed = true;
    B.sampled = sampled;
    if (sampled && (int)seeds.size() != n) return fail(PDMPC_ERR_INVALID, "pdmpc_set_step_seeds: the seeds are not one per vehicle of the packed step");
    Packer P{h, B, n, in, pred_offset, pred_index, fallback, sampled ? &seeds : nullptr};
    int rc;
    if ((rc = P.open())) return rc;
    if ((rc = slot_order(h, n, pred_offset, pred_index, weights, B))) return rc;
    h->soups.reset(n);
    for (int slot = 0; slot < n; ++slot)
        if ((rc = P.pack_vehicle(slot))) return rc;
    if ((rc = P.close())) return rc;
    h->timer.reset();
    std::memset(&h->stats, 0, sizeof h->stats);
    return PDMPC_OK;
}
```

p-dmpc_amd/csrc/pdmpc_device.h:

```cpp
#ifndef PDMPC_DEVICE_H
#define PDMPC_DEVICE_H

#include <stdint.h>

#include "../../include/pdmpc.h"

#define PDMPC_WAVE 64
#define PDMPC_MAX_WAVES 16
#define PDMPC_MAX_WAVES_SAT 12
#define PDMPC_MAX_THREADS (PDMPC_WAVE * PDMPC_MAX_WAVES)
#define PDMPC_SH_WORDS 128

struct DevManPose {
    double dx, dy, dyaw;
    int32_t n_cols;
    int32_t pad;
};

struct DevVehicle {
    double x0, y0, yaw0;
    double ref_x[PDMPC_HP_MAX];
    double ref_y[PDMPC_HP_MAX];
    double v_ref[PDMPC_HP_MAX];
    int32_t trim0;
    int32_t n_pred;
    int32_t pred_off;
    int32_t ll_off, ll_len;
    int32_t lit_off[PDMPC_HP_MAX + 1];
    int32_t hdv_off[PDMPC_HP_MAX + 1];
    int32_t fb_off[PDMPC_HP_MAX + 1];
    uint32_t seed;
};

struct NodeRec {
    double x, y, yaw, g;
    double cs, sn;
    double h;
    uint32_t parent;
    uint32_t packed;
};
#define NODE_TRIM(p) ((int)((p) & 1023u))
#define NODE_K(p) ((int)(((p) >> 10) & 31u))
#define NODE_MAN(p) ((int)(((p) >> 15) & 4095u))
#define NODE_COLS(p) ((int)(((p) >> 27) & 15u))

struct LdsLayout {
    uint32_t mask, man_index, pose, area;
    uint32_t ref;
    uint32_t shape;
    uint32_t path;
    uint32_t soup;
    uint32_t cand;
    uint32_t vstate;
    uint32_t expand;
    uint32_t tree16;
    uint32_t rand;
    uint32_t nodes;
    uint32_t total;
    uint32_t bk_near_key, bk_near_id;
    uint32_t bk_ready;
    uint32_t bk_hist;
    uint32_t bk_misc;
    uint32_t bk_pshape;
};

#define PDMPC_LK_ALIGN16(x) (((x) + 15u) & ~15u)
#ifndef PDMPC_LK_WAVES
#define PDMPC_LK_WAVES PDMPC_MAX_WAVES
#endif
#ifndef PDMPC_LK_READY_CAP
#define PDMPC_LK_READY_CAP 2048u
#endif
#define PDMPC_LK_COMPACT_WAVES 8
#define PDMPC_LK_COMPACT_READY_CAP 512u
#define PDMPC_LK_COMPACT_BK_PER 2
#define PDMPC_LKX_THREADS(W) ((uint32_t)(W) * PDMPC_WAVE)
#define PDMPC_LKX_REF 0u
#define PDMPC_LKX_SHAPE (PDMPC_LKX_REF + 3u * PDMPC_HP_MAX * 8u)
#define PDMPC_LKX_PATH(W) (PDMPC_LKX_SHAPE + (uint32_t)(W) * (2u * PDMPC_VMAX + 1u) * 16u)
#define PDMPC_LKX_CAND(W) (PDMPC_LKX_PATH(W) + PDMPC_LK_ALIGN16((PDMPC_HP_MAX + 2u) * 4u + 2u * (PDMPC_HP_MAX + 1u) * 4u + PDMPC_SH_WORDS * 4u + PDMPC_HP_MAX * 4u))
#define PDMPC_LKX_EXPAND(W) (PDMPC_LKX_CAND(W) + PDMPC_LK_ALIGN16(12u * PDMPC_LKX_THREADS(W)))
#define PDMPC_LKX_NEAR_KEY(W) (PDMPC_LKX_EXPAND(W) + (2u * PDMPC_HP_MAX * PDMPC_HP_MAX) * 8u + 16u * 16u)
#define PDMPC_LKX_NEAR_ID(W, P) (PDMPC_LKX_NEAR_KEY(W) + PDMPC_LK_ALIGN16((uint32_t)(P) * PDMPC_LKX_THREADS(W) * 8u))
#define PDMPC_LKX_READY(W, P) (PDMPC_LKX_NEAR_ID(W, P) + PDMPC_LK_ALIGN16((uint32_t)(P) * PDMPC_LKX_THREADS(W) * 4u))
#define PDMPC_LKX_HIST(W, RC, P) (PDMPC_LKX_READY(W, P) + (uint32_t)(RC) * 8u)
#define PDMPC_LKX_MISC(W, RC, P) (PDMPC_LKX_HIST(W, RC, P) + 3072u * 4u)
#define PDMPC_LKX_PSHAPE(W, RC, P) (PDMPC_LKX_MISC(W, RC, P) + 2048u)
#define PDMPC_LKX_FIXED_END(W, RC, P) (PDMPC_LKX_PSHAPE(W, RC, P) + PDMPC_LK_ALIGN16(PDMPC_HP_MAX * PDMPC_VMAX * 16u + PDMPC_HP_MAX * 4u + PDMPC_HP_MAX * 8u + PDMPC_HP_MAX * 4u))
#ifndef PDMPC_BK_PER
#define PDMPC_BK_PER 4
#endif
#define PDMPC_LK_THREADS PDMPC_LKX_THREADS(PDMPC_LK_WAVES)
#define PDMPC_LK_REF PDMPC_LKX_REF
#define PDMPC_LK_SHAPE PDMPC_LKX_SHAPE
#define PDMPC_LK_PATH PDMPC_LKX_PATH(PDMPC_LK_WAVES)
#define PDMPC_LK_CAND PDMPC_LKX_CAND(PDMPC_LK_WAVES)
#define PDMPC_LK_EXPAND PDMPC_LKX_EXPAND(PDMPC_LK_WAVES)
#define PDMPC_LK_NEAR_KEY PDMPC_LKX_NEAR_KEY(PDMPC_LK_WAVES)
#define PDMPC_LK_NEAR_ID PDMPC_LKX_NEAR_ID(PDMPC_LK_WAVES, PDMPC_BK_PER)
#define PDMPC_LK_READY PDMPC_LKX_READY(PDMPC_LK_WAVES, PDMPC_BK_PER)
#define PDMPC_LK_HIST PDMPC_LKX_HIST(PDMPC_LK_WAVES, PDMPC_LK_READY_CAP, PDMPC_BK_PER)
#define PDMPC_LK_MISC PDMPC_LKX_MISC(PDMPC_LK_WAVES, PDMPC_LK_READY_CAP, PDMPC_BK_PER)
#define PDMPC_LK_PSHAPE PDMPC_LKX_PSHAPE(PDMPC_LK_WAVES, PDMPC_LK_READY_CAP, PDMPC_BK_PER)
#define PDMPC_LK_FIXED_END PDMPC_LKX_FIXED_END(PDMPC_LK_WAVES, PDMPC_LK_READY_CAP, PDMPC_BK_PER)

struct NodeArena {
    NodeRec* nodes;
    double* key;
    unsigned long long* link;
    uint8_t* vstate;
    double* far_key;
    uint32_t* far_id;
    double* mid_key;
    uint32_t* mid_id;
    double* pb_key;
    uint32_t* pb_d;
    double* walk;
    uint32_t* child0;
    uint32_t* vlist;
};

static inline uint32_t pdmpc_lk_fixed(uint32_t W, uint32_t RC, uint32_t P, LdsLayout* L) {
    L->ref = PDMPC_LKX_REF;
    L->shape = PDMPC_LKX_SHAPE;
    L->path = PDMPC_LKX_PATH(W);
    L->cand = PDMPC_LKX_CAND(W);
    L->expand = PDMPC_LKX_EXPAND(W);
    L->bk_near_key = PDMPC_LKX_NEAR_KEY(W);
    L->bk_near_id = PDMPC_LKX_NEAR_ID(W, P);
    L->bk_ready = PDMPC_LKX_READY(W, P);
    L->bk_hist = PDMPC_LKX_HIST(W, RC, P);
    L->bk_misc = PDMPC_LKX_MISC(W, RC, P);
    L->bk_pshape = PDMPC_LKX_PSHAPE(W, RC, P);
    return PDMPC_LKX_FIXED_END(W, RC, P);
}

#define PDMPC_HELP_CAP 2048
#define PDMPC_HB_SEATS_MAX 64
#define PDMPC_HB_N 1
#define PDMPC_HB_MASK 2
#define PDMPC_HB_SEATS 3
#define PDMPC_HB_WANT 4
#define PDMPC_HB_WEIGHT 5
#define PDMPC_HB_ASSIGN 8
#define PDMPC_HB_DONE 72
#define PDMPC_HB_WORDS 136

struct KernelArgs {
    const uint64_t* succ_mask;
    const int16_t* man_index;
    const DevManPose* man_pose;
    const double* man_area;
    int32_t n_trims, n_words, n_man, Hp;
    int32_t checker;
    int32_t areas_in_lds;
    double dt;
    const DevVehicle* veh;
    const double* points;
    const int32_t* pred;
    pdmpc_vehicle_out* out;
    uint32_t* done_flag;
    uint32_t epoch;
    int32_t first;
    NodeArena arena;
    uint32_t max_nodes;
    int32_t* tree_size;
    LdsLayout lds;
    int32_t NL, NV, soup_cap, cand_cap;
    int32_t n_waves;
    unsigned long long* work_count;
    int32_t* tie_count;
    uint32_t* progress;
    int32_t debug_tail;
    int32_t n_searches;
    int32_t n_helpers;
    unsigned long long* help_board;
    uint32_t* help_verdict;
    uint32_t* help_finished;
    uint32_t help_fin_base;
    uint32_t launch_id;
    int32_t bk_ready_cap;
    int32_t bk_round0;
    int32_t bk_round;
    int32_t bk_ramp;
    int32_t bk_helpers_first;
    int32_t bk_seat_nodes;
    int32_t bk_tentative;
    int32_t bk_tile;
    int32_t bk_mid_min;
    int32_t bk_mid_fill;
    int32_t bk_share_min;
    int32_t bk_force_tie;
    int32_t bk_fast_arrival;
    double* bk_post;
    int32_t speculate;
    uint32_t spin_limit;
    int32_t reverse_dispatch;
};

enum { PDMPC_BULK = 0, PDMPC_BULK_WIDE = 1, PDMPC_BULK_SAT = 2, PDMPC_BULK_COMPACT = 3 };
struct ProductSwitches {
    static constexpr int32_t debug_tail = 0, bk_force_tie = 0, reverse_dispatch = 0, bk_tentative = 1, bk_fast_arrival = 1, speculate = 1;
    static constexpr int32_t areas_in_lds(int kernel) { return kernel == PDMPC_BULK || kernel == PDMPC_BULK_SAT ? 1 : 0; }
    static bool matches(const KernelArgs& a, int kernel) {
        return a.debug_tail == debug_tail && a.bk_force_tie == bk_force_tie && a.reverse_dispatch == reverse_dispatch && a.bk_tentative == bk_tentative &&
               a.bk_fast_arrival == bk_fast_arrival && a.speculate == speculate && a.areas_in_lds == areas_in_lds(kernel);
    }
};

struct JointLds {
    uint32_t mask, man_index, pose, area;
    uint32_t ref;
    uint32_t shape;
    uint32_t ints;
    uint32_t succ;
    uint32_t soup;
// ... 190 lines not shown
```

p-dmpc_amd/pdmpc/prototypes.py:

```python
import ctypes as C

from . import abi

P = C.POINTER
INT, STR = C.c_int, C.c_char_p
OBJ = C.c_void_p
VOIDP = C.c_void_p
I32, I64, U32, F64 = C.c_int32, C.c_int64, C.c_uint32, C.c_double
DP, IP, BP, UP = abi.c_double_p, abi.c_int32_p, abi.c_uint8_p, abi.c_uint32_p
CONFIG, MPA, POLYS, VIN, VOUT, CHOICE = P(abi.Config), P(abi.Mpa), P(abi.PolygonSet), P(abi.VehicleIn), P(abi.VehicleOut), P(abi.ChoiceStruct)

STEP = [I32, VIN, IP, IP, POLYS]
STEP_OUT = [P(I32), P(VIN), P(IP), P(IP), P(POLYS)]
POSES = [DP, DP, DP, DP, IP]
TABLE = [I32, I32, POLYS]
COUPLED = [BP, DP]
BOUND = POSES + [POLYS, I32, I32, IP, DP, DP, BP]
FCA = [I32, I32, DP, DP, DP, DP, I32, IP, POLYS, POLYS, F64, F64, F64, IP, IP]
FCA_GROUPED = [I32, P(abi.FcaGroup), I32, DP, DP, DP, DP, IP, IP]
CHOSEN = [CHOICE, IP, DP]
UNIQUE = [I32, BP, I64, P(I64), UP, IP]

PROTOTYPES = {
    "pdmpc_create": (INT, [CONFIG, P(OBJ)]),
    "pdmpc_destroy": (INT, [OBJ]),
    "pdmpc_get_config": (INT, [OBJ, CONFIG, P(I32)]),
    "pdmpc_upload_mpa": (INT, [OBJ, MPA]),
    "pdmpc_plan_batch": (INT, [OBJ, I32, VIN, VOUT]),
    "pdmpc_set_arena_limit": (INT, [OBJ, I32]),
    "pdmpc_grow_arena": (INT, [OBJ, I32]),
    "pdmpc_arena_nodes": (INT, [OBJ, P(I32), P(I64)]),
    "pdmpc_plan_step": (INT, [OBJ] + STEP + [VOUT]),
    "pdmpc_plan_step_literal": (INT, [OBJ] + STEP + [VOUT]),
    "pdmpc_pack_batch": (INT, [OBJ, I32, VIN]),
    "pdmpc_plan_step_lean": (INT, [OBJ] + STEP + [IP, DP]),
    "pdmpc_fetch_records_at": (INT, [OBJ, I32, IP, VOUT]),
    "pdmpc_choose_host": (INT, [I32, IP, DP] + CHOSEN),
    "pdmpc_choose_resident": (INT, [OBJ, I32] + CHOSEN + [VOUT]),
    "pdmpc_plan_step_chosen": (INT, [OBJ] + STEP + CHOSEN + [VOUT]),
    "pdmpc_choice_kernel_ms": (INT, [OBJ, DP]),
    "pdmpc_last_call_timing": (INT, [OBJ, DP]),
    "pdmpc_launch_packed": (INT, [OBJ]),
    "pdmpc_launch_range": (INT, [OBJ, I32, I32]),
    "pdmpc_fetch_results": (INT, [OBJ, I32, VOUT]),
    "pdmpc_synchronize": (INT, [OBJ]),
    "pdmpc_set_safe_launch": (INT, [OBJ, I32]),
    "pdmpc_set_device_share": (INT, [OBJ, I32]),
    "pdmpc_begin_step": (INT, [OBJ]),
    "pdmpc_select_bank": (INT, [OBJ, I32]),
    "pdmpc_reset_stats": (INT, [OBJ]),
    "pdmpc_set_step_weights": (INT, [OBJ, I32, DP]),
    "pdmpc_pack_step": (INT, [OBJ] + STEP),
    "pdmpc_result_device_buffer": (INT, [OBJ, P(VOIDP), P(C.c_size_t)]),
    "pdmpc_import_results": (INT, [OBJ, I32, I32, VOIDP]),
    "pdmpc_export_results": (INT, [OBJ, I32, I32, VOIDP]),
    "pdmpc_export_results_async": (INT, [OBJ, I32, I32, VOIDP]),
    "pdmpc_stream": (INT, [OBJ, P(VOIDP)]),
    "pdmpc_get_last_stats": (INT, [OBJ, P(abi.Stats)]),
    "pdmpc_debug_pop_trace": (INT, [OBJ, I32, I32, IP, IP]),
    "pdmpc_debug_tree": (INT, [OBJ, I32, I32] + [DP] * 5 + [IP] * 4),
    "pdmpc_debug_edge_check": (INT, [OBJ, I32, I32, IP, DP, DP, IP, DP, DP, IP]),
    "pdmpc_debug_raw_tree": (INT, [OBJ, I32, I32] + [DP] * 5 + [IP] * 3 + [DP, BP, IP]),
    "pdmpc_debug_counters": (INT, [OBJ, P(C.c_uint64)]),
    "pdmpc_debug_progress": (INT, [OBJ, I32, UP]),
    "pdmpc_debug_heap_script": (INT, [OBJ, I32, IP, IP, DP, I32, IP, IP, DP, DP]),
    "pdmpc_plan_batch_sampled": (INT, [OBJ, I32, VIN, UP, VOUT]),
    "pdmpc_plan_step_sampled": (INT, [OBJ] + STEP + [UP, VOUT]),
    "pdmpc_set_step_seeds": (INT, [OBJ, I32, UP]),
    "pdmpc_debug_random_numbers": (INT, [OBJ, I32, UP, I32, DP]),
    "pdmpc_plan_joint": (INT, [OBJ, I32, IP, VIN, VOUT]),
    "pdmpc_unique_priorities": (INT, [OBJ] + UNIQUE),
    "pdmpc_unique_priorities_host": (INT, UNIQUE),
    "pdmpc_local_reachable_sets": (INT, [MPA, I32, IP, DP, DP]),
    "pdmpc_upload_reachable_sets": (INT, [OBJ] + TABLE),
    "pdmpc_reachable_set_coupling": (INT, [OBJ, I32] + POSES + COUPLED),
    "pdmpc_reachable_set_coupling_host": (INT, TABLE + [I32] + POSES + COUPLED),
    "pdmpc_reachable_set_coupling_kernel_ms": (INT, [OBJ, DP]),
    "pdmpc_bound_reachable_sets": (INT, [OBJ, I32] + BOUND),
    "pdmpc_bound_reachable_sets_host": (INT, TABLE + [I32] + BOUND),
    "pdmpc_bounded_set_coupling": (INT, [OBJ] + COUPLED),
    "pdmpc_polygon_set_coupling_host": (INT, [POLYS, I32] + COUPLED),
    "pdmpc_bounded_reachable_kernel_ms": (INT, [OBJ, DP]),
    "pdmpc_reachable_set_coupling_grouped": (INT, [OBJ, I32, IP] + POSES + COUPLED),
    "pdmpc_bounded_set_coupling_grouped": (INT, [OBJ, I32, IP] + COUPLED),
    "pdmpc_reachable_set_coupling_grouped_host": (INT, TABLE + [I32, IP] + POSES + COUPLED),
    "pdmpc_polygon_set_coupling_grouped_host": (INT, [POLYS, I32, IP] + COUPLED),
    "pdmpc_fca_collisions": (INT, [OBJ] + FCA),
    "pdmpc_fca_collisions_host": (INT, FCA),
    "pdmpc_fca_kernel_ms": (INT, [OBJ, DP]),
    "pdmpc_fca_collisions_grouped": (INT, [OBJ] + FCA_GROUPED),
    "pdmpc_fca_collisions_grouped_host": (INT, FCA_GROUPED),
    "pdmpc_controller_create": (INT, [OBJ, P(abi.ControllerConfig), P(abi.ScenarioStruct), P(OBJ)]),
    "pdmpc_controller_destroy": (INT, [OBJ]),
    "pdmpc_controller_step": (INT, [OBJ]),
    "pdmpc_controller_run": (INT, [OBJ, I32, DP]),
    "pdmpc_controller_build_step": (INT, [OBJ]),
    "pdmpc_controller_apply": (INT, [OBJ, VOUT]),
    "pdmpc_controller_problem": (INT, [OBJ] + STEP_OUT + [P(IP), P(IP)]),
    "pdmpc_controller_state": (INT, [OBJ] + [DP] * 5 + [IP, P(I32)]),
    "pdmpc_controller_records": (VOUT, [OBJ]),
    "pdmpc_exploration_permutations": (INT, [I32, I32, U32, IP]),
    "pdmpc_controller_explore_build": (INT, [OBJ, I32, U32]),
    "pdmpc_controller_explore_problem": (INT, [OBJ] + STEP_OUT + [P(IP)] * 3),
    "pdmpc_controller_explore_choose": (INT, [OBJ, VOUT, IP, P(I32), DP]),
    "pdmpc_controller_explore_step": (INT, [OBJ, I32]),
    "pdmpc_controller_explore_run": (INT, [OBJ, I32, I32, DP]),
    "pdmpc_controller_explore_follow_own": (INT, [OBJ, I32]),
    "pdmpc_controller_explore_result": (INT, [OBJ, IP, P(I32), P(DP), P(VOUT)]),
    "pdmpc_controller_optimal_build": (INT, [OBJ, I32]),
    "pdmpc_controller_optimal_choose": (INT, [OBJ, VOUT, IP, DP]),
# ... 52 lines not shown
```

Before: 1512.

## Prune obstacle segments outside per-step reachability boxes before collision checks

Derives a conservative reach radius per prediction step from the MPA (largest maneuver displacement plus largest area extent) and builds an axis-aligned box around each vehicle root. At vehicle start and whenever predecessor shapes arrive, the kernel filters soup, HDV and lanelet segments against these boxes into LDS index lists. Item counts and chunk tables are then computed from the filtered lists, so the intersection checker visits only segments that could be reached. This costs extra LDS, rebuild passes and barriers on each arrival, and a tight fallback layout with fewer node slots when space runs short.

```diff
diff --git a/include/pdmpc.h b/include/pdmpc.h
--- a/include/pdmpc.h
+++ b/include/pdmpc.h
@@ -127,6 +127,9 @@
 int pdmpc_get_config(pdmpc_handle* handle, pdmpc_config* config, int32_t* mpa_uploaded);
 
 int pdmpc_upload_mpa(pdmpc_handle* handle, const pdmpc_mpa* mpa);
+int pdmpc_mpa_reach_host(const pdmpc_mpa* mpa, double* dmax, double* amax);
+int pdmpc_reach_lists_host(int32_t Hp, double dmax, double amax, double root_x, double root_y, const double* x, const double* y, const int32_t* step_first,
+                           const int32_t* step_count, int32_t* list_offset, int32_t* list);
 
 int pdmpc_plan_batch(pdmpc_handle* handle, int32_t n_vehicles, const pdmpc_vehicle_in* in,
                      pdmpc_vehicle_out* out);
diff --git a/include/pdmpc_reach.h b/include/pdmpc_reach.h
--- /dev/null
+++ b/include/pdmpc_reach.h
@@ -0,0 +1,34 @@
+#ifndef PDMPC_REACH_H
+#define PDMPC_REACH_H
+
+#include <math.h>
+
+#include "pdmpc_math.h"
+
+#define PDMPC_REACH_FINITE 0x1p64
+#define PDMPC_REACH_MARGIN 0x1p-20
+
+PDMPC_HD static inline double pdmpc_reach_radius(double dmax, double amax, int k) {
+    const double r = (double)(k - 1) * dmax + amax;
+    return r + r * 0x1p-50;
+}
+
+PDMPC_HD static inline void pdmpc_reach_box(double dmax, double amax, int k, double root_x, double root_y, double* box) {
+    const double R = pdmpc_reach_radius(dmax, amax, k);
+    const double rho = R + PDMPC_REACH_MARGIN * (1.0 + fabs(root_x) + fabs(root_y) + R);
+    box[0] = root_x - rho;
+    box[1] = root_x + rho;
+    box[2] = root_y - rho;
+    box[3] = root_y + rho;
+}
+
+PDMPC_HD static inline int pdmpc_reach_in(double x0, double y0, double x1, double y1, double x_lo, double x_hi, double y_lo, double y_hi) {
+    if (x0 != x0 || y0 != y0 || x1 != x1 || y1 != y1) return 0;
+    const int bounded = fabs(x0) <= PDMPC_REACH_FINITE && fabs(y0) <= PDMPC_REACH_FINITE && fabs(x1) <= PDMPC_REACH_FINITE && fabs(y1) <= PDMPC_REACH_FINITE;
+    if (!bounded) return 1;
+    const double max_x = x0 > x1 ? x0 : x1, min_x = x0 < x1 ? x0 : x1;
+    const double max_y = y0 > y1 ? y0 : y1, min_y = y0 < y1 ? y0 : y1;
+    return !(max_x < x_lo || min_x > x_hi || max_y < y_lo || min_y > y_hi);
+}
+
+#endif
diff --git a/p-dmpc_amd/csrc/api.cpp b/p-dmpc_amd/csrc/api.cpp
--- a/p-dmpc_amd/csrc/api.cpp
+++ b/p-dmpc_amd/csrc/api.cpp
@@ -14,6 +14,7 @@
 #include <vector>
 
 #include "../../include/pdmpc_geometry.h"
+#include "../../include/pdmpc_reach.h"
 #include "handle.hpp"
 
 namespace {
@@ -102,14 +103,17 @@
     return off;
 }
 
-bool layout_bulk(const pdmpc_handle* h, size_t budget, int n_waves, int areas, int soup_cap, LdsLayout& L, uint32_t& nv, uint32_t& nl, uint32_t ready_cap, bool compact) {
+bool layout_bulk(const pdmpc_handle* h, size_t budget, int n_waves, int areas, int soup_cap, int ll_cap, LdsLayout& L, uint32_t& nv, uint32_t& nl, uint32_t ready_cap, bool compact, bool tight = false) {
     const uint32_t lk_waves = compact ? PDMPC_LK_COMPACT_WAVES : PDMPC_MAX_WAVES, lk_ready = compact ? PDMPC_LK_COMPACT_READY_CAP : 2048u, lk_per = compact ? PDMPC_LK_COMPACT_BK_PER : PDMPC_BK_PER;
     if (ready_cap > lk_ready || (uint32_t)n_waves > lk_waves) return false;
-    uint32_t off = layout_mpa(h, pdmpc_lk_fixed(lk_waves, lk_ready, lk_per, &L), areas, L);
+    L.reach = pdmpc_lk_fixed(lk_waves, lk_ready, lk_per, &L);
+    L.reach_shared = tight ? 1u : 0u;
+    const uint32_t list_entries = h->cfg.checker == PDMPC_CHECK_INTERX ? (uint32_t)(std::max(soup_cap, 1) + (tight ? 0 : (h->cfg.Hp - 1) * std::max(ll_cap, 0))) : 0u;
+    uint32_t off = layout_mpa(h, align16(L.reach + list_entries * 2), areas, L);
     L.soup = off;
     off = align16(off + (uint32_t)std::max(soup_cap, 1) * 16);
     L.tree16 = L.bk_hist;
-    const uint32_t min_nodes = 64 * (uint32_t)sizeof(NodeRec) + 1024;
+    const uint32_t min_nodes = (tight ? 16u : 64u) * (uint32_t)sizeof(NodeRec) + 1024;
     if ((size_t)off + min_nodes + 256 > budget) return false;
     const uint32_t rest = (uint32_t)(budget - off - 256);
     nv = std::min<uint32_t>(16384u, std::max<uint32_t>(compact ? 512u : 1024u, rest / 6));
@@ -129,7 +133,7 @@
     return n_launch <= n_cu - 2;
 }
 
-int compute_lds_bulk(const pdmpc_handle* h, int n_launch, int soup_cap, LaunchLayout& out) {
+int compute_lds_bulk(const pdmpc_handle* h, int n_launch, int soup_cap, int ll_cap, LaunchLayout& out) {
     const Tuning& T = h->tune;
     const int ready_want = bulk_has_helpers(T, h->n_cu, n_launch) ? T.ready : std::max(256, T.ready / 2);
     const int cap = h->cfg.checker == PDMPC_CHECK_SAT ? PDMPC_MAX_WAVES_SAT : PDMPC_MAX_WAVES;
@@ -139,7 +143,7 @@
         LdsLayout L{};
         const int waves = T.waves >= 0 ? std::min(T.waves, PDMPC_LK_COMPACT_WAVES) : PDMPC_LK_COMPACT_WAVES;
         const int ready = std::min(std::min(ready_want, 3 * PDMPC_WAVE * waves), (int)PDMPC_LK_COMPACT_READY_CAP);
-        if (layout_bulk(h, kLdsMax / 2, waves, 0, soup_cap, L, nv, nl, (uint32_t)ready, true)) {
+        if (layout_bulk(h, kLdsMax / 2, waves, 0, soup_cap, ll_cap, L, nv, nl, (uint32_t)ready, true)) {
             out = {L, waves, (int)nl, (int)nv, 0, ready, true};
             return PDMPC_OK;
         }
@@ -148,9 +152,17 @@
     for (int areas = 1; areas >= 0; --areas) {
         LdsLayout L{};
         const int ready = std::min(ready_want, 3 * PDMPC_WAVE * waves);
-        if (!layout_bulk(h, kLdsMax, waves, areas, soup_cap, L, nv, nl, (uint32_t)ready, false)) continue;
+        if (!layout_bulk(h, kLdsMax, waves, areas, soup_cap, ll_cap, L, nv, nl, (uint32_t)ready, false)) continue;
         out = {L, waves, (int)nl, (int)nv, areas, ready, false};
         return PDMPC_OK;
+    }
+    {
+        LdsLayout L{};
+        const int ready = std::min(ready_want, 3 * PDMPC_WAVE * waves);
+        if (layout_bulk(h, kLdsMax, waves, 0, soup_cap, ll_cap, L, nv, nl, (uint32_t)ready, false, true)) {
+            out = {L, waves, (int)nl, (int)nv, 0, ready, false};
+            return PDMPC_OK;
+        }
     }
     char buf[256];
     snprintf(buf, sizeof buf, "obstacle soup (%d columns) + MPA tables do not fit into %zu B of LDS", soup_cap, kLdsMax);
@@ -386,7 +398,7 @@
     if (!B.perm.empty() && (first != 0 || count != B.n_packed)) return fail(PDMPC_ERR_INVALID, "range launches need a batch packed in level order (predecessors in lower slots)");
     if (count == 0) return PDMPC_OK;
     LaunchLayout lay;
-    int rc = search ? compute_lds_bulk(h, count, B.soup_cap, lay) : compute_lds_sampled(h, B.soup_cap, B.cand_cap, lay);
+    int rc = search ? compute_lds_bulk(h, count, B.soup_cap, B.ll_cap, lay) : compute_lds_sampled(h, B.soup_cap, B.cand_cap, lay);
     if (rc) return rc;
     KernelArgs a{};
     set_launch_args(h, B, lay, first, count, safe, a);
@@ -475,6 +487,41 @@
     return PDMPC_OK;
 }
 
+static void mpa_reach(const pdmpc_mpa* mpa, double& dmax, double& amax) {
+    dmax = 0.0;
+    amax = 0.0;
+    for (int t = 0; t < mpa->n_maneuvers; ++t) {
+        const pdmpc_maneuver& m = mpa->maneuvers[t];
+        dmax = std::max(dmax, hypot(m.dx, m.dy));
+        const double(*src[3])[PDMPC_VMAX] = {m.area, m.area_without_offset, m.area_large_offset};
+        for (int a = 0; a < 3; ++a)
+            for (int v = 0; v < m.n_cols && v < PDMPC_VMAX; ++v) amax = std::max(amax, hypot(src[a][0][v], src[a][1][v]));
+    }
+}
+
+int pdmpc_mpa_reach_host(const pdmpc_mpa* mpa, double* dmax, double* amax) {
+    if (!mpa || !dmax || !amax || (mpa->n_maneuvers > 0 && !mpa->maneuvers)) return fail(PDMPC_ERR_INVALID, "pdmpc_mpa_reach_host: null argument");
+    mpa_reach(mpa, *dmax, *amax);
+    return PDMPC_OK;
+}
+
+int pdmpc_reach_lists_host(int32_t Hp, double dmax, double amax, double root_x, double root_y, const double* x, const double* y, const int32_t* step_first,
+                           const int32_t* step_count, int32_t* list_offset, int32_t* list) {
+    if (Hp < 1 || Hp > PDMPC_HP_MAX || !step_first || !step_count || !list_offset) return fail(PDMPC_ERR_INVALID, "pdmpc_reach_lists_host: bad argument");
+    int32_t n = 0;
+    for (int k = 1; k <= Hp; ++k) {
+        const int32_t a = step_first[k - 1], c = step_count[k - 1];
+        if (a < 0 || c < 0 || (c > 1 && (!x || !y || !list))) return fail(PDMPC_ERR_INVALID, "pdmpc_reach_lists_host: bad step ranges");
+        double box[4];
+        pdmpc_reach_box(dmax, amax, k, root_x, root_y, box);
+        list_offset[k - 1] = n;
+        for (int32_t j = 0; j + 1 < c; ++j)
+            if (pdmpc_reach_in(x[a + j], y[a + j], x[a + j + 1], y[a + j + 1], box[0], box[1], box[2], box[3])) list[n++] = j;
+    }
+    list_offset[Hp] = n;
+    return PDMPC_OK;
+}
+
 int pdmpc_upload_mpa(pdmpc_handle* h, const pdmpc_mpa* mpa) {
     if (!h || !mpa) return fail(PDMPC_ERR_INVALID, "null argument");
     if (mpa->n_trims < 1 || mpa->n_trims > 1023) return fail(PDMPC_ERR_INVALID, "n_trims must be in 1..1023");
@@ -496,7 +543,7 @@
     for (int i = 0; i < n * n; ++i) mi[i] = (int16_t)mpa->maneuver_index[i];
     const int T = mpa->n_maneuvers;
     std::vector<DevManPose> pose((size_t)std::max(T, 1));
-    std::vector<double> area((size_t)std::max(T, 1) * 3 * PDMPC_VMAX * 2, 0.0);
+    std::vector<double> area((size_t)std::max(T, 1) * 3 * PDMPC_VMAX * 2 + 2, 0.0);
     for (int t = 0; t < T; ++t) {
         const pdmpc_maneuver& m = mpa->maneuvers[t];
         if (m.n_cols < 2 || m.n_cols > PDMPC_VMAX) return fail(PDMPC_ERR_INVALID, "maneuver area column count out of range");
@@ -512,6 +559,7 @@
                 area[(((size_t)t * 3 + a) * PDMPC_VMAX + v) * 2 + 1] = src[a][1][v];
             }
     }
+    mpa_reach(mpa, area[(size_t)T * 3 * PDMPC_VMAX * 2], area[(size_t)T * 3 * PDMPC_VMAX * 2 + 1]);
     if (h->d_mask.ensure(mask.size()) || h->d_mi.ensure(mi.size()) || h->d_pose.ensure(pose.size()) || h->d_area.ensure(area.size()))
         return fail(PDMPC_ERR_HIP, "hipMalloc failed for the MPA tables");
     HIPCHK(hipMemcpy(h->d_mask.p, mask.data(), mask.size() * 8, hipMemcpyHostToDevice));
diff --git a/p-dmpc_amd/csrc/bulk_search.hpp b/p-dmpc_amd/csrc/bulk_search.hpp
--- a/p-dmpc_amd/csrc/bulk_search.hpp
+++ b/p-dmpc_amd/csrc/bulk_search.hpp
@@ -3,6 +3,8 @@
 #include "search_common.hpp"
 
 #include "frontier_common.hpp"
+
+#include "../../include/pdmpc_reach.h"
 
 #define BK_P2 3
 #define BK_PER PDMPC_BK_PER
@@ -11,6 +13,7 @@
 namespace {
 
 typedef volatile LDS_AS unsigned long long lds_vu64;
+typedef LDS_AS uint16_t lds_u16;
 
 __device__ __forceinline__ unsigned long long wg_scan_excl(unsigned long long v, lds_vu64* wsum, int lane, int wave, int n_waves, unsigned long long& total) {
     unsigned long long inc = v;
@@ -50,6 +53,92 @@
     const lds_i32* l_lit;
     int areas_in_lds, ll_base, ll_len, Hp;
 };
+
+#define BK_RLIST(lsm) ((lds_u16*)((lsm) + PDMPC_LK_FIXED_END))
+__device__ __forceinline__ LDS_AS unsigned char* bk_lds_base() {
+    extern __shared__ __attribute__((aligned(16))) unsigned char smem[];
+    return (LDS_AS unsigned char*)smem;
+}
+#define BK_RBOX(lsm) ((lds_f64*)((lsm) + PDMPC_LK_REACH))
+#define BK_RCNT(lsm) ((lds_u32*)((lsm) + PDMPC_LK_REACH + PDMPC_LK_REACH_CNT))
+#define BK_RSTALE(lsm) ((volatile lds_u32*)((lsm) + PDMPC_LK_REACH + PDMPC_LK_REACH_STALE))
+#define BK_RSC(lsm) ((lds_i32*)((lsm) + PDMPC_LK_REACH + PDMPC_LK_REACH_SC))
+__device__ __forceinline__ void bk_reach_scalars(const BkCheck& C, LDS_AS unsigned char* lsm, bool shared_boundary_list) {
+    lds_i32* sc = BK_RSC(lsm);
+    sc[0] = (int32_t)((LDS_AS unsigned char*)C.l_soup - lsm);
+    sc[1] = (int32_t)((LDS_AS unsigned char*)C.l_area - lsm);
+    sc[2] = C.Hp;
+    sc[3] = C.ll_base;
+    sc[4] = C.ll_len;
+    sc[5] = shared_boundary_list ? 0 : C.ll_len;
+}
+struct BkItemCtx {
+    const BkCheck& C;
+    int interx;
+    __device__ __forceinline__ int word(int i) const { return BK_RSC(bk_lds_base())[i]; }
+    __device__ __forceinline__ const lds_d2* l_soup() const { return interx ? (const lds_d2*)(bk_lds_base() + word(0)) : C.l_soup; }
+    __device__ __forceinline__ const lds_d2* l_area() const { return interx ? (const lds_d2*)(bk_lds_base() + word(1)) : C.l_area; }
+    __device__ __forceinline__ int Hp() const { return interx ? word(2) : C.Hp; }
+    __device__ __forceinline__ int ll_base() const { return interx ? word(3) : C.ll_base; }
+    __device__ __forceinline__ int ll_len() const { return interx ? word(4) : C.ll_len; }
+    __device__ __forceinline__ int ll_stride() const { return interx ? word(5) : C.ll_len; }
+};
+template <int CHECKER>
+__device__ __forceinline__ BkItemCtx bk_item_ctx(const BkCheck& C) {
+    return BkItemCtx{C, CHECKER == PDMPC_CHECK_INTERX ? 1 : 0};
+}
+__device__ __forceinline__ void bk_reach_boxes(const KernelArgs& A, const DevVehicle* V, LDS_AS unsigned char* lsm, int tid) {
+    if (tid < A.Hp) {
+        const double* reach = A.man_area + (size_t)A.n_man * 3 * PDMPC_VMAX * 2;
+        double box[4];
+        pdmpc_reach_box(reach[0], reach[1], tid + 1, V->x0, V->y0, box);
+        lds_f64* rb = BK_RBOX(lsm) + 4 * tid;
+        rb[0] = box[0];
+        rb[1] = box[1];
+        rb[2] = box[2];
+        rb[3] = box[3];
+    }
+}
+template <int SOUPS>
+__device__ __forceinline__ void bk_reach_build(const BkCheck& C, LDS_AS unsigned char* lsm, int lane, int wave, int n_waves) {
+    const lds_f64* rbox = BK_RBOX(lsm);
+    lds_u32* rcnt = BK_RCNT(lsm);
+    for (int u = wave; u < (SOUPS == 1 ? 1 : 3) * C.Hp; u += n_waves) {
+        const int k = SOUPS == 1 ? u : u / 3, s = SOUPS == 1 ? 0 : u - 3 * k;
+        int base, n, at, kb = k;
+        if (s == 0) {
+            base = C.l_soff[k];
+            n = C.l_soff[k + 1] - base - 1;
+            at = base;
+        } else if (s == 1) {
+            base = C.l_hoff[k];
+            n = C.l_hoff[k + 1] - base - 1;
+            at = base;
+        } else {
+            const int stride = BK_RSC(lsm)[5];
+            base = C.ll_base;
+            n = C.ll_len - 1;
+            at = base + k * stride;
+            kb = stride ? k : C.Hp - 1;
+        }
+        const double x_lo = rbox[4 * kb], x_hi = rbox[4 * kb + 1], y_lo = rbox[4 * kb + 2], y_hi = rbox[4 * kb + 3];
+        const lds_d2* q = C.l_soup + base;
+        lds_u16* lst = BK_RLIST(lsm) + at;
+        uint32_t cnt = 0;
+        for (int j0 = 0; j0 < n; j0 += PDMPC_WAVE) {
+            const int j = j0 + lane;
+            bool in = false;
+            if (j < n) {
+                const d2 q0 = q[j], q1 = q[j + 1];
+                in = pdmpc_reach_in(q0.x, q0.y, q1.x, q1.y, x_lo, x_hi, y_lo, y_hi) != 0;
+            }
+            const unsigned long long m = __ballot(in);
+            if (in) lst[cnt + __builtin_amdgcn_mbcnt_hi((uint32_t)(m >> 32), __builtin_amdgcn_mbcnt_lo((uint32_t)m, 0u))] = (uint16_t)j;
+            cnt += (uint32_t)__builtin_popcountll(m);
+        }
+        if (lane == 0) rcnt[s * PDMPC_HP_MAX + k] = cnt;
+    }
+}
 
 #define VS_TENT 6u
 #define BK_TENT_MIN FR_JOIN_MAX
@@ -118,8 +207,33 @@
     n1 = CHECKER == PDMPC_CHECK_INTERX ? (Hk > 1 ? Hk - 1 : 0) : 0;
     n2 = ll_len > 1 ? ll_len - 1 : 0;
 }
+template <int CHECKER>
+__device__ __forceinline__ void bk_reach_counts(const BkCheck& C, const lds_u32* rcnt, int k, int& n0, int& n1, int& n2) {
+    if (CHECKER == PDMPC_CHECK_INTERX) {
+        n0 = (int)rcnt[k - 1];
+        n1 = (int)rcnt[PDMPC_HP_MAX + k - 1];
+        n2 = (int)rcnt[2 * PDMPC_HP_MAX + k - 1];
+    } else {
+        bk_item_counts<CHECKER>(C.l_soff[k] - C.l_soff[k - 1], C.l_hoff[k] - C.l_hoff[k - 1], C.ll_len, n0, n1, n2);
+    }
+}
+template <int CHECKER>
+__device__ __forceinline__ void bk_chunk_table(const BkCheck& C, const lds_u32* rcnt, lds_u32* chm, int t) {
+    if (t < 0 || t >= 8) return;
+    const int ls = t, Sg = 1 << ls;
+    uint32_t mx = 0;
+    for (int k = 1; k <= C.Hp; ++k) {
+        int n0, n1, n2;
+        bk_reach_counts<CHECKER>(C, rcnt, k, n0, n1, n2);
+        const uint32_t ch = (uint32_t)(((n0 + Sg - 1) >> ls) + ((n1 + Sg - 1) >> ls) + ((n2 + Sg - 1) >> ls));
+        mx = ch > mx ? ch : mx;
+    }
+    chm[ls] = mx;
+}
 template <int CHECKER, class Src>
 __device__ __forceinline__ void bk_check_items(const BkCheck& C, const Src& src, volatile lds_u32* r_flag, uint32_t r0, uint32_t R, int ls, uint32_t chmax, unsigned long long pend, int tid, int nthreads) {
+    const lds_u32* rcnt = BK_RCNT(bk_lds_base());
+    const lds_u16* rlist = BK_RLIST(bk_lds_base());
     const uint32_t items = R * chmax;
     const int Sg = 1 << ls;
     for (uint32_t item = (uint32_t)tid; item < items; item += (uint32_t)nthreads) {
@@ -128,13 +242,14 @@
         uint32_t parent, packed;
         src.link(r, parent, packed);
         if (!parent) continue;
+        const BkItemCtx I = bk_item_ctx<CHECKER>(C);
         const int k = NODE_K(packed), m = NODE_MAN(packed), ncols = NODE_COLS(packed);
         const int so = C.l_soff[k - 1], ho = C.l_hoff[k - 1];
-        const int M_k = C.l_soff[k] - so, Hk = C.l_hoff[k] - ho;
+        const int M_k = C.l_soff[k] - so;
         int n0, n1, n2;
-        bk_item_counts<CHECKER>(M_k, Hk, C.ll_len, n0, n1, n2);
+        bk_reach_counts<CHECKER>(C, rcnt, k, n0, n1, n2);
         const uint32_t c0 = (uint32_t)((n0 + Sg - 1) >> ls), c1 = (uint32_t)((n1 + Sg - 1) >> ls), c2 = (uint32_t)((n2 + Sg - 1) >> ls);
-        int base, t0, left, which = 0;
+        int base, t0, left, which = 0, lat = 0;
         if (c < c0) {
             base = so;
             t0 = (int)(c << ls);
@@ -144,10 +259,11 @@
             t0 = (int)((c - c0) << ls);
             left = n1 - t0;
         } else if (c < c0 + c1 + c2) {
-            base = C.ll_base;
+            base = I.ll_base();
             t0 = (int)((c - c0 - c1) << ls);
             left = n2 - t0;
-            which = k == C.Hp ? 2 : 1;
+            lat = (k - 1) * I.ll_stride();
+            which = k == I.Hp() ? 2 : 1;
         } else {
             continue;
         }
@@ -156,14 +272,21 @@
         src.pose(r, parent, pX, pY, cc, ss);
         const size_t abase = ((size_t)m * 3 + (size_t)which) * PDMPC_VMAX;
         d2 pt[PDMPC_VMAX];
+        if (C.areas_in_lds) {
+#pragma unroll
+            for (int i = 0; i < PDMPC_VMAX; ++i) pt[i] = I.l_area()[abase + i];
+        } else {
+#pragma unroll
+            for (int i = 0; i < PDMPC_VMAX; ++i) pt[i] = C.g_area[abase + i];
+        }
 #pragma unroll
         for (int i = 0; i < PDMPC_VMAX; ++i) {
-            const d2 a = C.areas_in_lds ? (d2)C.l_area[abase + i] : C.g_area[abase + i];
+            const d2 a = pt[i];
             pt[i].x = cc * a.x - ss * a.y + pX;
             pt[i].y = ss * a.x + cc * a.y + pY;
         }
-        const lds_d2* q = C.l_soup + base + t0;
         if (CHECKER == PDMPC_CHECK_SAT) {
+            const lds_d2* q = I.l_soup() + base + t0;
             uint32_t fnd = 0;
             if (which == 0) {
                 const int lit = C.l_lit[k - 1];
@@ -188,19 +311,20 @@
             if (fnd) __hip_atomic_fetch_or((lds_u32*)&r_flag[r], fnd, __ATOMIC_RELAXED, __HIP_MEMORY_SCOPE_WORKGROUP);
             continue;
         }
-        d2 q0 = q[0];
-        const int rel0 = (which == 0 && base == so) ? t0 - C.l_lit[k - 1] : -(1 << 20);
+        const lds_u16* lst = rlist + base + lat + t0;
+        const lds_d2* sp = I.l_soup() + base;
+        const int rel0 = (which == 0 && base == so) ? -C.l_lit[k - 1] : -(1 << 20);
         uint32_t found = 0;
         for (int t = 0; t < tn && !(found & 1u); ++t) {
             asm volatile("" : "+v"(pt[0].x), "+v"(pt[0].y), "+v"(pt[1].x), "+v"(pt[1].y), "+v"(pt[2].x), "+v"(pt[2].y), "+v"(pt[3].x), "+v"(pt[3].y), "+v"(pt[4].x), "+v"(pt[4].y),
                          "+v"(pt[5].x), "+v"(pt[5].y), "+v"(pt[6].x), "+v"(pt[6].y), "+v"(pt[7].x), "+v"(pt[7].y));
-            const d2 q1 = q[t + 1];
+            const int j = (int)lst[t];
+            const d2 q0 = sp[j], q1 = sp[j + 1];
             if (interx_segment_n<PDMPC_VMAX>(pt, ncols - 1, q0, q1)) {
-                const int rel = rel0 + t;
+                const int rel = rel0 + j;
                 const bool tent = rel >= 0 && ((pend >> (rel >> 3)) & 1ull) != 0ull;
                 found |= tent ? 2u : 1u;
             }
-            q0 = q1;
         }
         if (found) __hip_atomic_fetch_or((lds_u32*)&r_flag[r], found, __ATOMIC_RELAXED, __HIP_MEMORY_SCOPE_WORKGROUP);
     }
@@ -221,9 +345,10 @@
 __device__ __forceinline__ void bk_recheck_items(const Search& S, const VState& VS, const BkCheck& C, const SpecCtx& P, const uint32_t* vlist, const lds_u32* vcnt, uint32_t cap,
                                                  uint32_t items, unsigned long long arr, const lds_u64s* chg, volatile lds_u32* sh, int tid, int nthreads) {
     for (uint32_t item = (uint32_t)tid; item < items; item += (uint32_t)nthreads) {
+        const BkItemCtx I = bk_item_ctx<CHECKER>(C);
         uint32_t v = item, n_k = 0;
         int ks = 1;
-        for (; ks <= C.Hp; ++ks) {
+        for (; ks <= I.Hp(); ++ks) {
             n_k = vcnt[ks - 1] < cap ? vcnt[ks - 1] : cap;
             const uint32_t m = n_k * (uint32_t)__builtin_popcountll(chg[ks - 1] & arr);
             if (v < m) break;
@@ -243,13 +368,20 @@
         const double cc = pcs.x, ss = pcs.y, pX = pxy.x, pY = pxy.y;
         const size_t abase = (size_t)m * 3 * PDMPC_VMAX;
         d2 pt[PDMPC_VMAX];
+        if (C.areas_in_lds) {
+#pragma unroll
+            for (int i = 0; i < PDMPC_VMAX; ++i) pt[i] = I.l_area()[abase + i];
+        } else {
+#pragma unroll
+            for (int i = 0; i < PDMPC_VMAX; ++i) pt[i] = C.g_area[abase + i];
+        }
 #pragma unroll
         for (int i = 0; i < PDMPC_VMAX; ++i) {
-            const d2 ar = C.areas_in_lds ? (d2)C.l_area[abase + i] : C.g_area[abase + i];
+            const d2 ar = pt[i];
             pt[i].x = cc * ar.x - ss * ar.y + pX;
             pt[i].y = ss * ar.x + cc * ar.y + pY;
         }
-        const lds_d2* poly = P.l_soup + P.l_soff[k - 1] + P.l_lit[k - 1] + p * PDMPC_VMAX;
+        const lds_d2* poly = I.l_soup() + P.l_soff[k - 1] + P.l_lit[k - 1] + p * PDMPC_VMAX;
         d2 q0 = poly[0];
         bool hit = false;
         if (CHECKER == PDMPC_CHECK_SAT) {
@@ -454,7 +586,7 @@
 }
 
 __device__ __forceinline__ void bk_incorporate_body(const pdmpc_vehicle_out* out, const int32_t* pred, lds_d2* l_soup, const lds_i32* l_soff, const lds_i32* l_lit, int Hp, unsigned long long arr, int tid,
-                                                    int nthreads, lds_u64s* chg) {
+                                                    int nthreads, lds_u64s* chg, const lds_f64* rbox) {
     const double qnan = __longlong_as_double(0x7ff8000000000000LL);
     const int per = Hp * PDMPC_VMAX, n_arr = __builtin_popcountll(arr);
     for (int idx = tid; idx < n_arr * per; idx += nthreads) {
@@ -470,15 +602,24 @@
         lds_d2* slot = l_soup + l_soff[k] + l_lit[k] + p * PDMPC_VMAX + v;
         if (chg) {
             const d2 was = *slot;
-            if (__double_as_longlong(was.x) != __double_as_longlong(pt.x) || __double_as_longlong(was.y) != __double_as_longlong(pt.y))
+            const bool differs = __double_as_longlong(was.x) != __double_as_longlong(pt.x) || __double_as_longlong(was.y) != __double_as_longlong(pt.y);
+            if (rbox) {
+                const double nx = __shfl_down(pt.x, 1), ny = __shfl_down(pt.y, 1);
+                const bool in = v + 1 < PDMPC_VMAX && pdmpc_reach_in(pt.x, pt.y, nx, ny, rbox[4 * k], rbox[4 * k + 1], rbox[4 * k + 2], rbox[4 * k + 3]) != 0;
+                const int g = (tid & (PDMPC_WAVE - 1)) & ~(PDMPC_VMAX - 1);
+                const unsigned long long md = __ballot(differs), mi = __ballot(in);
+                if (v == 0 && ((md >> g) & 0xffull) != 0ull && ((mi >> g) & 0xffull) != 0ull)
+                    __hip_atomic_fetch_or(chg + k, 1ull << p, __ATOMIC_RELAXED, __HIP_MEMORY_SCOPE_WORKGROUP);
+            } else if (differs) {
                 __hip_atomic_fetch_or(chg + k, 1ull << p, __ATOMIC_RELAXED, __HIP_MEMORY_SCOPE_WORKGROUP);
+            }
         }
         *slot = pt;
     }
 }
 __device__ __forceinline__ void bk_incorporate(const pdmpc_vehicle_out* out, const int32_t* pred, lds_d2* l_soup, const lds_i32* l_soff, const lds_i32* l_lit, int Hp, unsigned long long arr, int tid,
-                                               int nthreads, lds_u64s* chg) {
-    bk_incorporate_body(out, pred, l_soup, l_soff, l_lit, Hp, arr, tid, nthreads, chg);
+                                               int nthreads, lds_u64s* chg, const lds_f64* rbox) {
+    bk_incorporate_body(out, pred, l_soup, l_soff, l_lit, Hp, arr, tid, nthreads, chg, rbox);
 }
 
 #define WC_DEAD 0x100u
@@ -543,7 +684,9 @@
                                              bool sat, int lane) {
     const lds_u32* pcols = (const lds_u32*)(pshape + Hp * PDMPC_VMAX);
     lds_u64s* chg = (lds_u64s*)(pcols + PDMPC_HP_MAX);
+    LDS_AS unsigned char* reach = (LDS_AS unsigned char*)pshape + (PDMPC_LK_REACH - PDMPC_LK_PSHAPE);
     unsigned long long pend = sh_load64(sh, SH_PEND_LO), fd = sh_load64(sh, BK_FD_LO);
+    const unsigned long long fd_in = fd;
     unsigned long long got = first;
     uint32_t spins = 0, res = 0;
     for (;;) {
@@ -556,7 +699,7 @@
                 __builtin_amdgcn_s_sleep(1);
                 continue;
             }
-            bk_incorporate_body(out, pred, l_soup, l_soff, l_lit, Hp, got, lane, PDMPC_WAVE, chg);
+            bk_incorporate_body(out, pred, l_soup, l_soff, l_lit, Hp, got, lane, PDMPC_WAVE, chg, sat ? (const lds_f64*)nullptr : (const lds_f64*)reach);
             wave_sync();
             pend &= ~got;
             fd |= got;
@@ -610,6 +753,7 @@
         sh[BK_FD_LO] = (uint32_t)fd;
         sh[BK_FD_HI] = (uint32_t)(fd >> 32);
         sh[BK_WAITRES] = res;
+        if (fd != fd_in) *(volatile lds_u32*)(reach + PDMPC_LK_REACH_STALE) = 1u;
         if (res == 2u) sh[BK_PUBLISHED] = 1u;
         sh[BK_IDLE] = sh[BK_IDLE] + spins + 1u;
     }
@@ -794,6 +938,7 @@
     CK.ll_base = X.C.ll_base;
     CK.ll_len = X.C.ll_len;
     CK.Hp = Hp;
+    const lds_u32* rcnt = BK_RCNT(X.lsm);
 
     if (tid == 0) {
         NodeRec r;
@@ -840,19 +985,17 @@
         asm volatile("s_waitcnt vmcnt(0)" ::: "memory");
     }
     if (SW::tentative(A)) bk_tentative_areas(A, P, sh_load64(sh, SH_PEND_LO), tid, (int)blockDim.x);
-    if (tid >= 64 && tid < 72) {
-        const int ls = tid - 64;
-        uint32_t mx = 0;
-        for (int k = 1; k <= Hp; ++k) {
-            const int M_k = CK.l_soff[k] - CK.l_soff[k - 1], Hk = CK.l_hoff[k] - CK.l_hoff[k - 1];
-            int n0, n1, n2;
-            bk_item_counts<CHECKER>(M_k, Hk, CK.ll_len, n0, n1, n2);
-            const int Sg = 1 << ls;
-            const uint32_t ch = (uint32_t)(((n0 + Sg - 1) >> ls) + ((n1 + Sg - 1) >> ls) + ((n2 + Sg - 1) >> ls));
-            mx = ch > mx ? ch : mx;
-        }
-        chm[ls] = mx;
-    }
+    if (CHECKER == PDMPC_CHECK_INTERX) {
+        bk_reach_boxes(A, V, X.lsm, tid);
+        if (tid == 0) {
+            BK_RSTALE(X.lsm)[0] = 0u;
+            bk_reach_scalars(CK, X.lsm, A.lds.reach_shared != 0u);
+        }
+        __syncthreads();
+        bk_reach_build<7>(CK, X.lsm, lane, wave, n_waves);
+        __syncthreads();
+    }
+    bk_chunk_table<CHECKER>(CK, rcnt, chm, tid - 64);
     __syncthreads();
 
     int status = PDMPC_OK;
@@ -1011,6 +1154,19 @@
             rec_valid = false;
             vs_copied = false;
             BK_MARK3
+            if (CHECKER == PDMPC_CHECK_INTERX && BK_RSTALE(X.lsm)[0] != 0u) {
+                BkCheck CL = CK;
+                {
+                    const BkItemCtx I = bk_item_ctx<CHECKER>(CK);
+                    CL.l_soup = I.l_soup();
+                    CL.Hp = I.Hp();
+                }
+                bk_reach_build<1>(CL, X.lsm, lane, wave, n_waves);
+                __syncthreads();
+                bk_chunk_table<CHECKER>(CL, rcnt, chm, tid);
+                if (tid == 0) BK_RSTALE(X.lsm)[0] = 0u;
+                __syncthreads();
+            }
             const BkTreeSrc tsrc{&S, ready};
             const unsigned long long pend_now = SW::tentative(A) ? sh_load64(sh, SH_PEND_LO) : 0ull;
             bool share = A.n_helpers > 0 && Rn >= (uint32_t)A.bk_share_min && P.n_pred <= 64;
@@ -1341,9 +1497,10 @@
             __syncthreads();
             if (sh[SH_STATE] == ST_ARRIVED) {
                 const unsigned long long arr = sh_load64(sh, SH_ARR_LO);
-                bk_incorporate(P.out, P.pred, P.l_soup, P.l_soff, P.l_lit, Hp, arr, tid, bd, chg);
+                bk_incorporate(P.out, P.pred, P.l_soup, P.l_soff, P.l_lit, Hp, arr, tid, bd, chg, CHECKER == PDMPC_CHECK_INTERX ? (const lds_f64*)BK_RBOX(X.lsm) : (const lds_f64*)nullptr);
                 __syncthreads();
                 if (tid == 0) {
+                    BK_RSTALE(X.lsm)[0] = 1u;
                     const unsigned long long pend = sh_load64(sh, SH_PEND_LO) & ~arr, fd = sh_load64(sh, BK_FD_LO) | arr;
                     sh[SH_PEND_LO] = (uint32_t)pend;
                     sh[SH_PEND_HI] = (uint32_t)(pend >> 32);
@@ -2085,6 +2242,7 @@
     CK.ll_base = 0;
     CK.ll_len = 0;
     CK.Hp = Hp;
+    const lds_u32* rcnt = BK_RCNT(lsm);
     if (SW::areas_in_lds(A)) stage16(lsm + A.lds.area, A.man_area, A.n_man * 3 * PDMPC_VMAX, tid);
     if (tid < SH_WORDS) hs[tid] = 0;
     __syncthreads();
@@ -2211,20 +2369,16 @@
             P.n_pred = V->n_pred;
             if (SW::tentative(A)) bk_tentative_areas(A, P, V->n_pred >= 64 ? ~0ull : ((1ull << V->n_pred) - 1ull), tid, bd);
             cur_mask = 0;
-            __syncthreads();
-            if (tid < 8) {
-                const int ls = tid;
-                uint32_t mx = 0;
-                for (int k = 1; k <= Hp; ++k) {
-                    const int M_k = l_soff[k] - l_soff[k - 1], Hk = l_hoff[k] - l_hoff[k - 1];
-                    int n0, n1, n2;
-                    bk_item_counts<CHECKER>(M_k, Hk, CK.ll_len, n0, n1, n2);
-                    const int Sg = 1 << ls;
-                    const uint32_t ch = (uint32_t)(((n0 + Sg - 1) >> ls) + ((n1 + Sg - 1) >> ls) + ((n2 + Sg - 1) >> ls));
-                    mx = ch > mx ? ch : mx;
-                }
-                chm[ls] = mx;
-            }
+            if (CHECKER == PDMPC_CHECK_INTERX) {
+                bk_reach_boxes(A, V, lsm, tid);
+                if (tid == 0) bk_reach_scalars(CK, lsm, A.lds.reach_shared != 0u);
+            }
+            __syncthreads();
+            if (CHECKER == PDMPC_CHECK_INTERX) {
+                bk_reach_build<7>(CK, lsm, lane, wave, bd >> 6);
+                __syncthreads();
+            }
+            bk_chunk_table<CHECKER>(CK, rcnt, chm, tid);
             __syncthreads();
             if (hticking) hk_mark = __builtin_amdgcn_s_memrealtime();
             continue;
@@ -2274,8 +2428,14 @@
         const unsigned long long mask = ((unsigned long long)hs[HS_MASK_HI] << 32) | hs[HS_MASK_LO];
         last_seq = seq;
         if (mask != cur_mask) {
-            bk_incorporate(P.out, P.pred, P.l_soup, P.l_soff, P.l_lit, Hp, mask & ~cur_mask, tid, bd, nullptr);
+            bk_incorporate(P.out, P.pred, P.l_soup, P.l_soff, P.l_lit, Hp, mask & ~cur_mask, tid, bd, nullptr, nullptr);
             cur_mask = mask;
+            if (CHECKER == PDMPC_CHECK_INTERX) {
+                __syncthreads();
+                bk_reach_build<1>(CK, lsm, lane, wave, bd >> 6);
+                __syncthreads();
+                bk_chunk_table<CHECKER>(CK, rcnt, chm, tid);
+            }
         }
         HK_TICK(1)
         {
diff --git a/p-dmpc_amd/csrc/handle.hpp b/p-dmpc_amd/csrc/handle.hpp
--- a/p-dmpc_amd/csrc/handle.hpp
+++ b/p-dmpc_amd/csrc/handle.hpp
@@ -168,6 +168,7 @@
     bool pack_failed = false;
     bool sampled = false;
     int soup_cap = 0;
+    int ll_cap = 0;
     int cand_cap = 0;
     std::vector<int64_t> lit_cols;
     std::vector<int32_t> perm;
diff --git a/p-dmpc_amd/csrc/pack.cpp b/p-dmpc_amd/csrc/pack.cpp
--- a/p-dmpc_amd/csrc/pack.cpp
+++ b/p-dmpc_amd/csrc/pack.cpp
@@ -67,7 +67,7 @@
     size_t veh_bytes = 0, pts_base = 0;
     BlobRegions host;
     size_t n_pred_out = 0, n_pts = 0;
-    int soup_cap = 0, cand_cap = 0;
+    int soup_cap = 0, cand_cap = 0, ll_cap = 0;
 
     BlobRegions regions(unsigned char* blob) const { return {(DevVehicle*)blob, (int32_t*)(blob + veh_bytes), (double*)(blob + pts_base)}; }
     int vehicle_of(int slot) const { return B.perm.empty() ? slot : B.perm[(size_t)slot]; }
@@ -231,6 +231,7 @@
         }
         const int need = (d.lit_off[Hp] - d.lit_off[0]) + Hp * d.n_pred * PDMPC_VMAX + (d.hdv_off[Hp] - d.hdv_off[0]) + d.ll_len;
         soup_cap = std::max(soup_cap, need);
+        ll_cap = std::max(ll_cap, (int)d.ll_len);
         for (int k = 0; k < Hp; ++k) cand_cap = std::max(cand_cap, (d.lit_off[k + 1] - d.lit_off[k]) + d.n_pred * PDMPC_VMAX + (d.hdv_off[k + 1] - d.hdv_off[k]) + d.ll_len);
         return PDMPC_OK;
     }
@@ -240,6 +241,7 @@
         put(qnan, qnan);
         host.pred[n_pred_out++] = 0;
         B.soup_cap = soup_cap + 2;
+        B.ll_cap = ll_cap;
         B.cand_cap = (cand_cap + 4 + 3) & ~3;
         const size_t pts_bytes = (n_pts * 16 + 15) & ~(size_t)15;
         const size_t total = pts_base + pts_bytes;
diff --git a/p-dmpc_amd/csrc/pdmpc_device.h b/p-dmpc_amd/csrc/pdmpc_device.h
--- a/p-dmpc_amd/csrc/pdmpc_device.h
+++ b/p-dmpc_amd/csrc/pdmpc_device.h
@@ -62,6 +62,9 @@
     uint32_t bk_hist;
     uint32_t bk_misc;
     uint32_t bk_pshape;
+    uint32_t reach_shared;
+    uint32_t bk_reach;
+    uint32_t reach;
 };
 
 #define PDMPC_LK_ALIGN16(x) (((x) + 15u) & ~15u)
@@ -86,7 +89,11 @@
 #define PDMPC_LKX_HIST(W, RC, P) (PDMPC_LKX_READY(W, P) + (uint32_t)(RC) * 8u)
 #define PDMPC_LKX_MISC(W, RC, P) (PDMPC_LKX_HIST(W, RC, P) + 3072u * 4u)
 #define PDMPC_LKX_PSHAPE(W, RC, P) (PDMPC_LKX_MISC(W, RC, P) + 2048u)
-#define PDMPC_LKX_FIXED_END(W, RC, P) (PDMPC_LKX_PSHAPE(W, RC, P) + PDMPC_LK_ALIGN16(PDMPC_HP_MAX * PDMPC_VMAX * 16u + PDMPC_HP_MAX * 4u + PDMPC_HP_MAX * 8u + PDMPC_HP_MAX * 4u))
+#define PDMPC_LKX_REACH(W, RC, P) (PDMPC_LKX_PSHAPE(W, RC, P) + PDMPC_LK_ALIGN16(PDMPC_HP_MAX * PDMPC_VMAX * 16u + PDMPC_HP_MAX * 4u + PDMPC_HP_MAX * 8u + PDMPC_HP_MAX * 4u))
+#define PDMPC_LK_REACH_CNT (PDMPC_HP_MAX * 4u * 8u)
+#define PDMPC_LK_REACH_STALE (PDMPC_LK_REACH_CNT + 3u * PDMPC_HP_MAX * 4u)
+#define PDMPC_LK_REACH_SC (PDMPC_LK_REACH_STALE + 16u)
+#define PDMPC_LKX_FIXED_END(W, RC, P) (PDMPC_LKX_REACH(W, RC, P) + PDMPC_LK_REACH_SC + 32u)
 #ifndef PDMPC_BK_PER
 #define PDMPC_BK_PER 4
 #endif
@@ -102,6 +109,7 @@
 #define PDMPC_LK_HIST PDMPC_LKX_HIST(PDMPC_LK_WAVES, PDMPC_LK_READY_CAP, PDMPC_BK_PER)
 #define PDMPC_LK_MISC PDMPC_LKX_MISC(PDMPC_LK_WAVES, PDMPC_LK_READY_CAP, PDMPC_BK_PER)
 #define PDMPC_LK_PSHAPE PDMPC_LKX_PSHAPE(PDMPC_LK_WAVES, PDMPC_LK_READY_CAP, PDMPC_BK_PER)
+#define PDMPC_LK_REACH PDMPC_LKX_REACH(PDMPC_LK_WAVES, PDMPC_LK_READY_CAP, PDMPC_BK_PER)
 #define PDMPC_LK_FIXED_END PDMPC_LKX_FIXED_END(PDMPC_LK_WAVES, PDMPC_LK_READY_CAP, PDMPC_BK_PER)
 
 struct NodeArena {
@@ -132,6 +140,7 @@
     L->bk_hist = PDMPC_LKX_HIST(W, RC, P);
     L->bk_misc = PDMPC_LKX_MISC(W, RC, P);
     L->bk_pshape = PDMPC_LKX_PSHAPE(W, RC, P);
+    L->bk_reach = PDMPC_LKX_REACH(W, RC, P);
     return PDMPC_LKX_FIXED_END(W, RC, P);
 }
 
diff --git a/p-dmpc_amd/pdmpc/prototypes.py b/p-dmpc_amd/pdmpc/prototypes.py
--- a/p-dmpc_amd/pdmpc/prototypes.py
+++ b/p-dmpc_amd/pdmpc/prototypes.py
@@ -26,6 +26,8 @@
     "pdmpc_destroy": (INT, [OBJ]),
     "pdmpc_get_config": (INT, [OBJ, CONFIG, P(I32)]),
     "pdmpc_upload_mpa": (INT, [OBJ, MPA]),
+    "pdmpc_mpa_reach_host": (INT, [MPA, DP, DP]),
+    "pdmpc_reach_lists_host": (INT, [I32, F64, F64, F64, F64, DP, DP, IP, IP, IP, IP]),
     "pdmpc_plan_batch": (INT, [OBJ, I32, VIN, VOUT]),
     "pdmpc_set_arena_limit": (INT, [OBJ, I32]),
     "pdmpc_grow_arena": (INT, [OBJ, I32]),
```

After: 1570, median of 6. 3.8% higher.
